# waczjoan/gaussian-mesh-splatting

Hardware: AMD Instinct MI355X
Metric: train iters/s (fwd+bwd raster) @800×800, 300k Gaussians; HBM GB/s vs roofline (higher is better)
Workload: dtype f32

## Files before the change

### gaussian-mesh-splatting_amd/csrc/gms_common.h

```cpp
#pragma once
#include <hip/hip_runtime.h>
#include <stdint.h>

#include "../../include/gmsplat.h"

namespace gms {

constexpr int TILE = 16;
constexpr int TILE_PIX = TILE * TILE;
constexpr int WAVE = 64;
constexpr int BLOCK = 256;
constexpr float NEAR_Z = 0.2f;
constexpr float DILATE = 0.3f;
constexpr float ALPHA_MIN = 1.0f / 255.0f;
constexpr float ALPHA_MAX = 0.99f;
constexpr float T_MIN = 0.0001f;

__device__ constexpr float SH_C0 = 0.28209479177387814f;
__device__ constexpr float SH_C1 = 0.4886025119029199f;
__device__ constexpr float SH_C2[5] = {1.0925484305920792f, -1.0925484305920792f, 0.31539156525252005f,
                                       -1.0925484305920792f, 0.5462742152960396f};
__device__ constexpr float SH_C3[7] = {-0.5900435899266435f, 2.890611442640554f, -0.4570457994644658f,
                                       0.3731763325901154f, -0.4570457994644658f, 1.445305721320277f,
                                       -0.5900435899266435f};

struct __attribute__((aligned(16))) SplatRec {
    float4 q0, q1, q2;
};

__host__ __device__ inline size_t align_up(size_t v, size_t a) { return (v + a - 1) / a * a; }

struct GeomState {
    SplatRec *rec;
    float *depth;
    uint8_t *clamped;
    ushort4 *rect;
    static __host__ __device__ size_t bytes(size_t P)
    {
        return align_up(P * sizeof(SplatRec), 256) + align_up(P * 4, 256) + align_up(P, 256) + align_up(P * sizeof(ushort4), 256);
    }
    static __host__ __device__ GeomState carve(void *base, size_t P)
    {
        GeomState g;
        char *p = (char *)base;
        g.rec = (SplatRec *)p; p += align_up(P * sizeof(SplatRec), 256);
        g.depth = (float *)p;  p += align_up(P * 4, 256);
        g.clamped = (uint8_t *)p; p += align_up(P, 256);
        g.rect = (ushort4 *)p;
        return g;
    }
};

struct ImageState {
    float *final_T;
    uint32_t *n_contrib;
    uint32_t *tile_count;
    uint32_t *tile_cursor;
    uint32_t *tile_offset;
    uint32_t *unit_first;
    uint32_t *mseg_first;
    uint32_t *class_first;
    uint32_t *tile_dead;
    uint32_t *tile_cmax;
    uint32_t *scan_out;
    static __host__ __device__ size_t bytes(size_t W, size_t H)
    {
        size_t T = ((W + TILE - 1) / TILE) * ((H + TILE - 1) / TILE);
        return 2 * align_up(W * H * 4, 256) + 2 * align_up(T * 4, 256) + 3 * align_up((T + 1) * 4, 256) +
               align_up(8 * (T + 1) * 4, 256) + 2 * align_up(T * 4, 256) + 256;
    }
    static __host__ __device__ ImageState carve(void *base, size_t W, size_t H)
    {
        size_t T = ((W + TILE - 1) / TILE) * ((H + TILE - 1) / TILE);
        ImageState s;
        char *p = (char *)base;
        s.final_T = (float *)p;        p += align_up(W * H * 4, 256);
        s.n_contrib = (uint32_t *)p;   p += align_up(W * H * 4, 256);
        s.tile_count = (uint32_t *)p;  p += align_up(T * 4, 256);
        s.tile_cursor = (uint32_t *)p; p += align_up(T * 4, 256);
        s.tile_offset = (uint32_t *)p; p += align_up((T + 1) * 4, 256);
        s.unit_first = (uint32_t *)p;  p += align_up((T + 1) * 4, 256);
        s.mseg_first = (uint32_t *)p;  p += align_up((T + 1) * 4, 256);
        s.class_first = (uint32_t *)p; p += align_up(8 * (T + 1) * 4, 256);
        s.tile_dead = (uint32_t *)p;   p += align_up(T * 4, 256);
        s.tile_cmax = (uint32_t *)p;   p += align_up(T * 4, 256);
        s.scan_out = (uint32_t *)p;
        return s;
    }
};

struct BinningState {
    uint64_t *keys;
    uint4 *unit_tile;
    float *seg_state;
    uint2 *deep_tab;
    uint32_t *multi_tab;
    uint16_t *mmask;
    static __host__ __device__ size_t n_units(size_t N, size_t T, size_t L) { return T + N / L + 1; }
    static __host__ __device__ size_t n_slots(size_t N, size_t L) { return 2 * (N / L) + 2; }
    static __host__ __device__ size_t n_deep(size_t N, size_t T) { return N / 1024 + T + 2; }
    static __host__ __device__ size_t n_multi(size_t N) { return N / 1024 + 2; }
    static __host__ __device__ size_t bytes(size_t N, size_t T, size_t L, bool micro)
    {
        return align_up((N > 0 ? N : 1) * 8, 256) + align_up(n_units(N, T, L) * 32, 256) +
               align_up(n_slots(N, L) * 7 * TILE_PIX * 4, 256) + align_up(n_deep(N, T) * 8, 256) + align_up(n_multi(N) * 4, 256) +
               (micro ? align_up((N > 0 ? N : 1) * 2, 256) : 0);
    }
    static __host__ __device__ BinningState carve(void *base, size_t N, size_t T, size_t L)
    {
        BinningState b;
        char *p = (char *)base;
        b.keys = (uint64_t *)p;      p += align_up((N > 0 ? N : 1) * 8, 256);
        b.unit_tile = (uint4 *)p;    p += align_up(n_units(N, T, L) * 32, 256);
        b.seg_state = (float *)p;    p += align_up(n_slots(N, L) * 7 * TILE_PIX * 4, 256);
        b.deep_tab = (uint2 *)p;     p += align_up(n_deep(N, T) * 8, 256);
        b.multi_tab = (uint32_t *)p; p += align_up(n_multi(N) * 4, 256);
        b.mmask = (uint16_t *)p;
        return b;
    }
};

template <int CTRL, int ROW_MASK = 0xf>
__device__ __forceinline__ float dpp_add(float v)
{
    int moved = __builtin_amdgcn_update_dpp(0, __builtin_bit_cast(int, v), CTRL, ROW_MASK, 0xf, false);
    return v + __builtin_bit_cast(float, moved);
}

__device__ __forceinline__ float wave_sum_to_lane63(float v)
{
    v = dpp_add<0xB1>(v);
    v = dpp_add<0x4E>(v);
    v = dpp_add<0x141>(v);
    v = dpp_add<0x140>(v);
    v = dpp_add<0x142, 0xa>(v);
    v = dpp_add<0x143, 0xc>(v);
    return v;
}

__device__ __forceinline__ void swap32x5(float &a0, float &a1, float &b0, float &b1, float &c0, float &c1, float &d0,
                                         float &d1, float &e0, float &e1)
{
    asm volatile("s_nop 1\n\tv_permlane32_swap_b32 %0, %1\n\tv_permlane32_swap_b32 %2, %3\n\t"
                 "v_permlane32_swap_b32 %4, %5\n\tv_permlane32_swap_b32 %6, %7\n\tv_permlane32_swap_b32 %8, %9"
                 : "+v"(a0), "+v"(a1), "+v"(b0), "+v"(b1), "+v"(c0), "+v"(c1), "+v"(d0), "+v"(d1), "+v"(e0), "+v"(e1));
}
__device__ __forceinline__ void swap16x3(float &a0, float &a1, float &b0, float &b1, float &c0, float &c1)
{
    asm volatile("s_nop 1\n\tv_permlane16_swap_b32 %0, %1\n\tv_permlane16_swap_b32 %2, %3\n\tv_permlane16_swap_b32 %4, %5"
                 : "+v"(a0), "+v"(a1), "+v"(b0), "+v"(b1), "+v"(c0), "+v"(c1));
}

__device__ __forceinline__ void wave_reduce10(float v0, float v1, float v2, float v3, float v4, float v5, float v6,
                                              float v7, float v8, float v9, float &y0, float &y1)
{
    swap32x5(v0, v1, v2, v3, v4, v5, v6, v7, v8, v9);
    float w0 = v0 + v1, w1 = v2 + v3, w2 = v4 + v5, w3 = v6 + v7, w4 = v8 + v9;
    float z = 0.f;
    swap16x3(w0, w1, w2, w3, w4, z);
    const float x0 = w0 + w1;
    const float x1 = w2 + w3;
    const float x2 = w4 + z;
    const float a = dpp_add<0x128>(x0);
    const float b = dpp_add<0x128>(x1);
    y0 = (threadIdx.x & 8) ? b : a;
    y1 = dpp_add<0x128>(x2);
    y0 = dpp_add<0x141>(y0); y0 = dpp_add<0xB1>(y0); y0 = dpp_add<0x4E>(y0);
    y1 = dpp_add<0x141>(y1); y1 = dpp_add<0xB1>(y1); y1 = dpp_add<0x4E>(y1);
}

__device__ __forceinline__ void wave_reduce10x2(float *a, float *b, float &y0a, float &y1a, float &y0b, float &y1b)
{
    swap32x5(a[0], a[1], a[2], a[3], a[4], a[5], a[6], a[7], a[8], a[9]);
    swap32x5(b[0], b[1], b[2], b[3], b[4], b[5], b[6], b[7], b[8], b[9]);
    float wa0 = a[0] + a[1], wb0 = b[0] + b[1], wa1 = a[2] + a[3], wb1 = b[2] + b[3], wa2 = a[4] + a[5];
    float wb2 = b[4] + b[5], wa3 = a[6] + a[7], wb3 = b[6] + b[7], wa4 = a[8] + a[9], wb4 = b[8] + b[9];
    float za = 0.f, zb = 0.f;
    swap16x3(wa0, wa1, wa2, wa3, wa4, za);
    swap16x3(wb0, wb1, wb2, wb3, wb4, zb);
    const float xa0 = wa0 + wa1, xb0 = wb0 + wb1, xa1 = wa2 + wa3, xb1 = wb2 + wb3, xa2 = wa4 + za, xb2 = wb4 + zb;
    const bool hi8 = (threadIdx.x & 8) != 0;
    const float pa = dpp_add<0x128>(xa0), pb = dpp_add<0x128>(xb0), qa = dpp_add<0x128>(xa1), qb = dpp_add<0x128>(xb1);
    y0a = hi8 ? qa : pa; y0b = hi8 ? qb : pb;
    y1a = dpp_add<0x128>(xa2); y1b = dpp_add<0x128>(xb2);
    y0a = dpp_add<0x141>(y0a); y0b = dpp_add<0x141>(y0b); y1a = dpp_add<0x141>(y1a); y1b = dpp_add<0x141>(y1b);
    y0a = dpp_add<0xB1>(y0a); y0b = dpp_add<0xB1>(y0b); y1a = dpp_add<0xB1>(y1a); y1b = dpp_add<0xB1>(y1b);
    y0a = dpp_add<0x4E>(y0a); y0b = dpp_add<0x4E>(y0b); y1a = dpp_add<0x4E>(y1a); y1b = dpp_add<0x4E>(y1b);
}

__device__ __forceinline__ void wave_sync()
{
    __builtin_amdgcn_fence(__ATOMIC_RELEASE, "wavefront");
    __builtin_amdgcn_wave_barrier();
    __builtin_amdgcn_fence(__ATOMIC_ACQUIRE, "wavefront");
}

__device__ __forceinline__ int lane_id() { return (int)(threadIdx.x & 63); }

__device__ __forceinline__ void tile_rect(float px, float py, float radius, int gx, int gy, int &minx, int &miny,
                                          int &maxx, int &maxy)
{
    const float big = 1048576.0f;
    float q0 = (px - radius) / TILE, q1 = (py - radius) / TILE;
    float q2 = (px + radius + (TILE - 1)) / TILE, q3 = (py + radius + (TILE - 1)) / TILE;
    minx = (int)fminf(big, fmaxf(-big, q0));
    miny = (int)fminf(big, fmaxf(-big, q1));
    maxx = (int)fminf(big, fmaxf(-big, q2));
    maxy = (int)fminf(big, fmaxf(-big, q3));
    minx = min(gx, max(0, minx)); maxx = min(gx, max(0, maxx));
    miny = min(gy, max(0, miny)); maxy = min(gy, max(0, maxy));
}

template <bool RETURNING>
__device__ __forceinline__ uint32_t wave_aggregated_inc(uint32_t *counters, int key, bool active)
{
    const int lane = (int)(threadIdx.x & 63);
    uint32_t rank = 0, cnt = 0;
    int my_leader = lane;
    bool is_leader = false;
    uint64_t todo = __ballot(active);
    while (todo) {
        const int leader = __builtin_ctzll(todo);
        const int k = __builtin_amdgcn_readlane(key, leader);
        const bool mine = active && key == k;
        const uint64_t same = __ballot(mine);
        if (mine) { rank = (uint32_t)__builtin_popcountll(same & ((1ull << lane) - 1ull)); my_leader = leader; }
        if (lane == leader) { is_leader = true; cnt = (uint32_t)__builtin_popcountll(same); }
        todo &= ~same;
    }
    uint32_t base = 0;
    if (is_leader) {
        if (RETURNING) base = atomicAdd(&counters[key], cnt);
        else atomicAdd(&counters[key], cnt);
    }
    if (!RETURNING) return 0;
    base = (uint32_t)__shfl((int)base, my_leader);
    return base + rank;
}

constexpr int TT_SLOTS = 1024;
__device__ __forceinline__ uint32_t tt_hash(int tile) { return ((uint32_t)tile * 2654435761u) >> 22; }
__device__ __forceinline__ int tt_insert(int *key, int tile)
{
    uint32_t h = tt_hash(tile);
    for (int probe = 0; probe < 16; probe++) {
        const int old = atomicCAS(&key[h], -1, tile);
        if (old == -1 || old == tile) return (int)h;
        h = (h + 1) & (TT_SLOTS - 1);
    }
    return -1;
}
__device__ __forceinline__ int tt_find(const int *key, int tile)
{
    uint32_t h = tt_hash(tile);
    for (int probe = 0; probe < 16; probe++) {
        const int k = key[h];
        if (k == tile) return (int)h;
        if (k == -1) return -1;
        h = (h + 1) & (TT_SLOTS - 1);
    }
    return -1;
}

struct AggTicket { uint32_t rank; int leader; uint32_t base; };

__device__ __forceinline__ AggTicket wave_aggregated_issue(uint32_t *counters, int key, bool active)
{
    const int lane = (int)(threadIdx.x & 63);
    AggTicket t{0u, lane, 0u};
    uint32_t cnt = 0;
    bool is_leader = false;
    uint64_t todo = __ballot(active);
    while (todo) {
        const int leader = __builtin_ctzll(todo);
        const int k = __builtin_amdgcn_readlane(key, leader);
        const bool mine = active && key == k;
        const uint64_t same = __ballot(mine);
        if (mine) { t.rank = (uint32_t)__builtin_popcountll(same & ((1ull << lane) - 1ull)); t.leader = leader; }
        if (lane == leader) { is_leader = true; cnt = (uint32_t)__builtin_popcountll(same); }
        todo &= ~same;
    }
    if (is_leader) t.base = atomicAdd(&counters[key], cnt);
    return t;
}

__device__ __forceinline__ uint32_t wave_aggregated_finish(const AggTicket &t)
{
    return (uint32_t)__shfl((int)t.base, t.leader) + t.rank;
}

__device__ __forceinline__ float dot3p(float a, float b, float c, float d, float e, float f, float g)
{
    float t = a * b;
    t = __fmaf_rn(c, d, t);
    t = __fmaf_rn(e, f, t);
    return t + g;
}

int fault_mode();

int det_mode();
int upstream_scale_mod_grad();
void *det_scratch(int slot, size_t bytes, hipStream_t stream);

void set_error(const char *fmt, ...);

struct TraceRange { bool on; explicit TraceRange(const char *name); ~TraceRange(); };

extern bool g_profile_on;
void profile_begin(int kernel_id, hipStream_t stream);
void profile_end(int kernel_id, hipStream_t stream);

}

#define GMS_HIP_CHECK(expr)                                                                    \
    do {                                                                                       \
        hipError_t _e = (expr);                                                                \
        if (_e != hipSuccess) {                                                                \
            gms::set_error("%s failed: %s (%s:%d)", #expr, hipGetErrorString(_e), __FILE__, __LINE__); \
            return GMS_ERR_HIP;                                                                \
        }                                                                                      \
    } while (0)

#define GMS_LAUNCH(kid, stream, ...)                                  \
    do {                                                              \
        if (gms::g_profile_on) gms::profile_begin(kid, stream);       \
        __VA_ARGS__;                                                  \
        if (gms::g_profile_on) gms::profile_end(kid, stream);         \
    } while (0)

#define GMS_KERNEL_CHECK(dbg, stream, name)                                                    \
    do {                                                                                       \
        hipError_t _e = hipGetLastError();                                                     \
        if (_e == hipSuccess && (dbg)) _e = hipStreamSynchronize(stream);                      \
        if (_e != hipSuccess) {                                                                \
            gms::set_error("kernel %s failed: %s", name, hipGetErrorString(_e));               \
            return GMS_ERR_HIP;                                                                \
        }                                                                                      \
    } while (0)
```

### gaussian-mesh-splatting_amd/csrc/gms_project.h

```cpp
#pragma once
#include "gms_common.h"

namespace gms {

struct Cov3 {
    float c[6];
};

__device__ __forceinline__ void cov3d_from_scale_rot(const float s_in[3], float mod, const float q[4], Cov3 &out)
{
#pragma clang fp contract(off)
    float s0 = mod * s_in[0], s1 = mod * s_in[1], s2 = mod * s_in[2];
    float r = q[0], x = q[1], y = q[2], z = q[3];
    float R00 = 1.f - 2.f * (y * y + z * z), R01 = 2.f * (x * y - r * z), R02 = 2.f * (x * z + r * y);
    float R10 = 2.f * (x * y + r * z), R11 = 1.f - 2.f * (x * x + z * z), R12 = 2.f * (y * z - r * x);
    float R20 = 2.f * (x * z - r * y), R21 = 2.f * (y * z + r * x), R22 = 1.f - 2.f * (x * x + y * y);
    float L00 = R00 * s0, L01 = R01 * s1, L02 = R02 * s2;
    float L10 = R10 * s0, L11 = R11 * s1, L12 = R12 * s2;
    float L20 = R20 * s0, L21 = R21 * s1, L22 = R22 * s2;
    out.c[0] = L00 * L00 + L01 * L01 + L02 * L02;
    out.c[1] = L00 * L10 + L01 * L11 + L02 * L12;
    out.c[2] = L00 * L20 + L01 * L21 + L02 * L22;
    out.c[3] = L10 * L10 + L11 * L11 + L12 * L12;
    out.c[4] = L10 * L20 + L11 * L21 + L12 * L22;
    out.c[5] = L20 * L20 + L21 * L21 + L22 * L22;
}

struct Ewa {
    float tx, ty, tz;
    float xmul, ymul;
    float T0[3], T1[3];
    float ST0[3], ST1[3];
    float a0, b, c0;
};

__device__ __forceinline__ void view_transform(const float *V, float px, float py, float pz, float &vx, float &vy,
                                               float &vz)
{
    vx = dot3p(V[0], px, V[4], py, V[8], pz, V[12]);
    vy = dot3p(V[1], px, V[5], py, V[9], pz, V[13]);
    vz = dot3p(V[2], px, V[6], py, V[10], pz, V[14]);
}

__device__ __forceinline__ void ewa_project(const float *V, float vx, float vy, float vz, const Cov3 &cv, float fx,
                                            float fy, float limx, float limy, Ewa &e)
{
#pragma clang fp contract(off)
    float txtz = vx / vz, tytz = vy / vz;
    e.tx = fminf(limx, fmaxf(-limx, txtz)) * vz;
    e.ty = fminf(limy, fmaxf(-limy, tytz)) * vz;
    e.tz = vz;
    e.xmul = (txtz < -limx || txtz > limx) ? 0.f : 1.f;
    e.ymul = (tytz < -limy || tytz > limy) ? 0.f : 1.f;
    float J00 = fx / e.tz, J02 = -(fx * e.tx) / (e.tz * e.tz);
    float J11 = fy / e.tz, J12 = -(fy * e.ty) / (e.tz * e.tz);
#pragma unroll
    for (int c = 0; c < 3; c++) {
        e.T0[c] = J00 * V[4 * c + 0] + J02 * V[4 * c + 2];
        e.T1[c] = J11 * V[4 * c + 1] + J12 * V[4 * c + 2];
    }
    const float S[3][3] = {{cv.c[0], cv.c[1], cv.c[2]}, {cv.c[1], cv.c[3], cv.c[4]}, {cv.c[2], cv.c[4], cv.c[5]}};
#pragma unroll
    for (int r = 0; r < 3; r++) {
        e.ST0[r] = S[r][0] * e.T0[0] + S[r][1] * e.T0[1] + S[r][2] * e.T0[2];
        e.ST1[r] = S[r][0] * e.T1[0] + S[r][1] * e.T1[1] + S[r][2] * e.T1[2];
    }
    e.a0 = e.T0[0] * e.ST0[0] + e.T0[1] * e.ST0[1] + e.T0[2] * e.ST0[2];
    e.b = e.T0[0] * e.ST1[0] + e.T0[1] * e.ST1[1] + e.T0[2] * e.ST1[2];
    e.c0 = e.T1[0] * e.ST1[0] + e.T1[1] * e.ST1[1] + e.T1[2] * e.ST1[2];
}

}
```

### gaussian-mesh-splatting_amd/csrc/raster_backward.hip

```cpp
#include "gms_blend.h"
#include "gms_mesh.h"
#include "gms_common.h"
#include "gms_project.h"

namespace gms {

constexpr int SH_PITCH_B = 52;

struct PreBwdArgs {
    int P, D, M, W, H;
    const float *means3D, *shs, *shs_rest, *colors, *opac, *scales, *rots, *cov3Dp, *view, *proj, *campos;
    float mod, tanx, tany;
    float scale_grad_mod;
    int aa;
    const int *radii;
    const uint8_t *clamped;
    float *accum;
    int rezero;
    float *dL_dmean2D, *dL_dopacity, *dL_dcolors;
    float *dL_dmeans3D, *dL_dcov3D, *dL_dsh, *dL_dsh_rest, *dL_dscales, *dL_drots;
    float *dL_dcolor_sh;
    int campos_row;
    GmsMeshArgs mesh;
    float *mesh_dvertices, *mesh_dalpha, *mesh_dscale, *mesh_dopacity;
};

template <int DEG>
__device__ __forceinline__ void sh_backward_regs(float *r, float x, float y, float z, const float dRGB[3], float gdir[3])
{
#define GMS_SH_TERM(K, BV, BDX, BDY, BDZ)                                          \
    {                                                                              \
        const float bv = (BV), bx = (BDX), by = (BDY), bz = (BDZ);                 \
        _Pragma("unroll") for (int c = 0; c < 3; c++) {                            \
            const float w = r[(K) * 3 + c] * dRGB[c];                              \
            gdir[0] += bx * w; gdir[1] += by * w; gdir[2] += bz * w;               \
            r[(K) * 3 + c] = bv * dRGB[c];                                         \
        }                                                                          \
    }
    GMS_SH_TERM(0, SH_C0, 0.f, 0.f, 0.f)
    if (DEG > 0) {
        GMS_SH_TERM(1, -SH_C1 * y, 0.f, -SH_C1, 0.f)
        GMS_SH_TERM(2, SH_C1 * z, 0.f, 0.f, SH_C1)
        GMS_SH_TERM(3, -SH_C1 * x, -SH_C1, 0.f, 0.f)
    }
    if (DEG > 1) {
        const float xx = x * x, yy = y * y, zz = z * z;
        GMS_SH_TERM(4, SH_C2[0] * x * y, SH_C2[0] * y, SH_C2[0] * x, 0.f)
        GMS_SH_TERM(5, SH_C2[1] * y * z, 0.f, SH_C2[1] * z, SH_C2[1] * y)
        GMS_SH_TERM(6, SH_C2[2] * (2.f * zz - xx - yy), -2.f * SH_C2[2] * x, -2.f * SH_C2[2] * y, 4.f * SH_C2[2] * z)
        GMS_SH_TERM(7, SH_C2[3] * x * z, SH_C2[3] * z, 0.f, SH_C2[3] * x)
        GMS_SH_TERM(8, SH_C2[4] * (xx - yy), 2.f * SH_C2[4] * x, -2.f * SH_C2[4] * y, 0.f)
    }
    if (DEG > 2) {
        const float xx = x * x, yy = y * y, zz = z * z;
        GMS_SH_TERM(9, SH_C3[0] * y * (3.f * xx - yy), SH_C3[0] * 6.f * x * y, SH_C3[0] * (3.f * xx - 3.f * yy), 0.f)
        GMS_SH_TERM(10, SH_C3[1] * x * y * z, SH_C3[1] * y * z, SH_C3[1] * x * z, SH_C3[1] * x * y)
        GMS_SH_TERM(11, SH_C3[2] * y * (4.f * zz - xx - yy), SH_C3[2] * (-2.f * x * y), SH_C3[2] * (4.f * zz - xx - 3.f * yy), SH_C3[2] * 8.f * y * z)
        GMS_SH_TERM(12, SH_C3[3] * z * (2.f * zz - 3.f * xx - 3.f * yy), SH_C3[3] * (-6.f * x * z), SH_C3[3] * (-6.f * y * z), SH_C3[3] * (6.f * zz - 3.f * xx - 3.f * yy))
        GMS_SH_TERM(13, SH_C3[4] * x * (4.f * zz - xx - yy), SH_C3[4] * (4.f * zz - 3.f * xx - yy), SH_C3[4] * (-2.f * x * y), SH_C3[4] * 8.f * x * z)
        GMS_SH_TERM(14, SH_C3[5] * z * (xx - yy), SH_C3[5] * 2.f * x * z, SH_C3[5] * (-2.f * y * z), SH_C3[5] * (xx - yy))
        GMS_SH_TERM(15, SH_C3[6] * x * (xx - 3.f * yy), SH_C3[6] * (3.f * xx - 3.f * yy), SH_C3[6] * (-6.f * x * y), 0.f)
    }
#undef GMS_SH_TERM
}

template <int DEG>
__device__ __forceinline__ void sh_backward(float *row_lds, float x, float y, float z, const float dRGB[3], float gdir[3])
{
    constexpr int NQ = ((DEG + 1) * (DEG + 1) * 3 + 3) / 4;
    float r[NQ * 4];
#pragma unroll
    for (int q = 0; q < NQ; q++) {
        const float4 v = *reinterpret_cast<const float4 *>(row_lds + q * 4);
        r[4 * q] = v.x; r[4 * q + 1] = v.y; r[4 * q + 2] = v.z; r[4 * q + 3] = v.w;
    }
    sh_backward_regs<DEG>(r, x, y, z, dRGB, gdir);
#pragma unroll
    for (int k = (DEG + 1) * (DEG + 1) * 3; k < NQ * 4; k++) r[k] = 0.f;
#pragma unroll
    for (int q = 0; q < NQ; q++)
        *reinterpret_cast<float4 *>(row_lds + q * 4) = make_float4(r[4 * q], r[4 * q + 1], r[4 * q + 2], r[4 * q + 3]);
}

template <int NQ>
__device__ __forceinline__ void stage_sh_rows_b(const float *shs, int g0, int rows, int rowq, float *wl, int lane)
{
    const float4 *src = reinterpret_cast<const float4 *>(shs) + (size_t)g0 * rowq;
    for (int idx = lane; idx < rows * NQ; idx += WAVE) {
        const int r = idx / NQ, c = idx - r * NQ;
        *reinterpret_cast<float4 *>(wl + r * 52 + c * 4) = src[(size_t)r * rowq + c];
    }
}

template <bool MESH>
__global__ void __launch_bounds__(BLOCK) preprocess_bwd_kernel(PreBwdArgs a, int pre_bwd_linear)
{
    __shared__ __attribute__((aligned(16))) float sh_lds[4 * WAVE * SH_PITCH_B];
    const int tid = threadIdx.x, lane = tid & 63, wave = tid >> 6;
    const int i = blockIdx.x * BLOCK + tid;
    const bool valid = i < a.P;
    const bool vis = valid && a.radii[i] > 0;
    float *wl = sh_lds + wave * (WAVE * SH_PITCH_B);
    const int rowf = a.M * 3;
    const bool use_sh = a.shs != nullptr;
    const bool vec_ok = use_sh && (rowf % 4 == 0) && (rowf <= 48);
    const int nb = (a.D + 1) * (a.D + 1);
    const int g0 = blockIdx.x * BLOCK + wave * WAVE;
    const int rows = min(WAVE, a.P - g0);

    const bool split = a.shs_rest != nullptr;
    constexpr int RESTF = 45;
    const bool linear = use_sh && split && a.D == 3 && pre_bwd_linear;
    float *const lin_dc = wl + WAVE * RESTF;
    if (linear) {
        if (__any(vis)) {
            const int rr = max(rows, 0);
            const float *sp = a.shs_rest + (size_t)g0 * RESTF;
            const int nfl = rr * RESTF, nd = rr * 3;
#pragma unroll
            for (int j = 0; j < 12; j++) {
                const int e4 = (lane + WAVE * j) * 4;
                if (e4 + 3 < nfl)
                    __builtin_amdgcn_global_load_lds((const __attribute__((address_space(1))) void *)(sp + e4),
                                                     (__attribute__((address_space(3))) void *)(wl + WAVE * 4 * j), 16, 0, 0);
            }
            if (lane * 4 + 3 < nd)
                __builtin_amdgcn_global_load_lds((const __attribute__((address_space(1))) void *)(a.shs + (size_t)g0 * 3 + lane * 4),
                                                 (__attribute__((address_space(3))) void *)lin_dc, 16, 0, 0);
            if (rr < WAVE) {
                for (int e = (nfl & ~3) + lane; e < nfl; e += WAVE) wl[e] = sp[e];
                for (int e = (nd & ~3) + lane; e < nd; e += WAVE) lin_dc[e] = a.shs[(size_t)g0 * 3 + e];
            }
            __builtin_amdgcn_s_waitcnt(0x0f70);
        }
        wave_sync();
    } else if (use_sh && split) {
        if (__any(vis)) {
            for (int e = lane; e < rows * 3; e += WAVE) wl[(e / 3) * SH_PITCH_B + (e % 3)] = a.shs[(size_t)g0 * 3 + e];
            const int need = nb * 3 - 3;
            if (need == RESTF) {
                const float *sp = a.shs_rest + (size_t)g0 * RESTF;
                const int nfl = rows * RESTF;
                for (int e4 = lane * 4; e4 < nfl; e4 += WAVE * 4) {
                    float v4[4];
                    if (e4 + 3 < nfl) { const float4 v = *reinterpret_cast<const float4 *>(sp + e4); v4[0] = v.x; v4[1] = v.y; v4[2] = v.z; v4[3] = v.w; }
                    else { for (int t = 0; t < 4; t++) v4[t] = e4 + t < nfl ? sp[e4 + t] : 0.f; }
#pragma unroll
                    for (int t = 0; t < 4; t++) {
                        const int e = e4 + t;
                        if (e < nfl) wl[(e / RESTF) * SH_PITCH_B + 3 + (e % RESTF)] = v4[t];
                    }
                }
            } else {
                for (int e = lane; e < rows * need; e += WAVE) {
                    const int r = e / need, c = e - r * need;
                    wl[r * SH_PITCH_B + 3 + c] = a.shs_rest[((size_t)g0 + r) * RESTF + c];
                }
            }
        }
        wave_sync();
    } else if (use_sh) {
        if (vec_ok) {
            if (__any(vis)) {
                const int rowq = rowf / 4;
                switch (a.D) {
                case 0: stage_sh_rows_b<1>(a.shs, g0, rows, rowq, wl, lane); break;
                case 1: stage_sh_rows_b<3>(a.shs, g0, rows, rowq, wl, lane); break;
                case 2: stage_sh_rows_b<7>(a.shs, g0, rows, rowq, wl, lane); break;
                default: stage_sh_rows_b<12>(a.shs, g0, rows, rowq, wl, lane); break;
                }
            }
        } else if (vis) {
            for (int k = 0; k < nb * 3; k++) wl[lane * SH_PITCH_B + k] = a.shs[(size_t)i * rowf + k];
        }
        wave_sync();
    }

    float dmean[3] = {0.f, 0.f, 0.f};
    float dcov[6] = {0.f, 0.f, 0.f, 0.f, 0.f, 0.f};
    float dscale[3] = {0.f, 0.f, 0.f};
    float drot[4] = {0.f, 0.f, 0.f, 0.f};
    float dcol_sh[3] = {0.f, 0.f, 0.f};
    float4 ga = make_float4(0.f, 0.f, 0.f, 0.f), gb = ga, gc4 = ga;
    if (valid) {
        float4 *rec = reinterpret_cast<float4 *>(a.accum + (size_t)i * GRAD_STRIDE);
        ga = rec[0]; gb = rec[1]; gc4 = rec[2];
        if (a.rezero && vis) {
            const float4 z = make_float4(0.f, 0.f, 0.f, 0.f);
            rec[0] = z; rec[1] = z; rec[2] = z;
        }
    }
    const float mom_x = ga.x, mom_y = ga.y, mom_xx = ga.z, mom_xy = ga.w, mom_yy = gb.x, mom_0 = gb.y;
    float acc_mx = 0.f, acc_my = 0.f;
    const float acc_col[3] = {gb.z, gb.w, gc4.x};
    const float acc_id = gc4.y;
    float dop = 0.f;
    float *row = wl + lane * SH_PITCH_B;

    if (vis) {
        const float px = a.means3D[3 * (size_t)i], py = a.means3D[3 * (size_t)i + 1], pz = a.means3D[3 * (size_t)i + 2];
        const float *V = a.view, *Mx = a.proj;
        float vx, vy, vz;
        view_transform(V, px, py, pz, vx, vy, vz);
        Cov3 cv;
        float s_in[3] = {0.f, 0.f, 0.f}, q[4] = {1.f, 0.f, 0.f, 0.f};
        if (a.cov3Dp) {
#pragma unroll
            for (int k = 0; k < 6; k++) cv.c[k] = a.cov3Dp[6 * (size_t)i + k];
        } else {
            s_in[0] = a.scales[3 * (size_t)i]; s_in[1] = a.scales[3 * (size_t)i + 1]; s_in[2] = a.scales[3 * (size_t)i + 2];
            const float4 qv = *reinterpret_cast<const float4 *>(a.rots + 4 * (size_t)i);
            q[0] = qv.x; q[1] = qv.y; q[2] = qv.z; q[3] = qv.w;
            cov3d_from_scale_rot(s_in, a.mod, q, cv);
        }
        const float fx = (float)a.W / (2.f * a.tanx), fy = (float)a.H / (2.f * a.tany);
        Ewa e;
        ewa_project(V, vx, vy, vz, cv, fx, fy, 1.3f * a.tanx, 1.3f * a.tany, e);
        const float b = e.b, aD = e.a0 + DILATE, cD = e.c0 + DILATE;
        const float det = aD * cD - b * b;
        {
            const float dinv = 1.f / det;
            const float cA = cD * dinv, cB = -b * dinv, cC = aD * dinv;
            acc_mx = -(0.5f * (float)a.W) * (cA * mom_x + cB * mom_y);
            acc_my = -(0.5f * (float)a.H) * (cC * mom_y + cB * mom_x);
            float opp = a.opac[i];
            if (a.aa) opp *= sqrtf(fmaxf(0.000025f, (e.a0 * e.c0 - b * b) / det));
            dop = opp > 0.f ? mom_0 / opp : 0.f;
        }
        const float gA = -0.5f * mom_xx, gB = -0.5f * mom_xy, gC = -0.5f * mom_yy;
        const float d2inv = 1.f / (det * det + 0.0000001f);
        float dL_da = d2inv * (-cD * cD * gA + 2.f * b * cD * gB + (det - aD * cD) * gC);
        float dL_dc = d2inv * (-aD * aD * gC + 2.f * aD * b * gB + (det - aD * cD) * gA);
        float dL_db = d2inv * 2.f * (b * cD * gA - (det + 2.f * b * b) * gB + aD * b * gC);
        if (a.aa) {
            const float det0 = e.a0 * e.c0 - b * b;
            const float ratio = det0 / det;
            const float h = sqrtf(fmaxf(0.000025f, ratio));
            const float dL_dh = dop * a.opac[i];
            dop = dop * h;
            const float dL_dr = ratio <= 0.000025f ? 0.f : dL_dh / (2.f * h);
            dL_da += dL_dr * (e.c0 / det - det0 * cD / (det * det));
            dL_dc += dL_dr * (e.a0 / det - det0 * aD / (det * det));
            dL_db += dL_dr * (-2.f * b / det + det0 * 2.f * b / (det * det));
        }
        const float *T0 = e.T0, *T1 = e.T1;
        dcov[0] = T0[0] * T0[0] * dL_da + T0[0] * T1[0] * dL_db + T1[0] * T1[0] * dL_dc;
        dcov[3] = T0[1] * T0[1] * dL_da + T0[1] * T1[1] * dL_db + T1[1] * T1[1] * dL_dc;
        dcov[5] = T0[2] * T0[2] * dL_da + T0[2] * T1[2] * dL_db + T1[2] * T1[2] * dL_dc;
        dcov[1] = 2.f * T0[0] * T0[1] * dL_da + (T0[0] * T1[1] + T0[1] * T1[0]) * dL_db + 2.f * T1[0] * T1[1] * dL_dc;
        dcov[2] = 2.f * T0[0] * T0[2] * dL_da + (T0[0] * T1[2] + T0[2] * T1[0]) * dL_db + 2.f * T1[0] * T1[2] * dL_dc;
        dcov[4] = 2.f * T0[2] * T0[1] * dL_da + (T0[1] * T1[2] + T0[2] * T1[1]) * dL_db + 2.f * T1[1] * T1[2] * dL_dc;
        float dJ00 = 0.f, dJ02 = 0.f, dJ11 = 0.f, dJ12 = 0.f;
#pragma unroll
        for (int c = 0; c < 3; c++) {
            const float dT0 = 2.f * e.ST0[c] * dL_da + e.ST1[c] * dL_db;
            const float dT1 = 2.f * e.ST1[c] * dL_dc + e.ST0[c] * dL_db;
            dJ00 += dT0 * V[4 * c + 0]; dJ02 += dT0 * V[4 * c + 2];
            dJ11 += dT1 * V[4 * c + 1]; dJ12 += dT1 * V[4 * c + 2];
        }
        const float tzi = 1.f / e.tz, tz2 = tzi * tzi, tz3 = tz2 * tzi;
        const float dtx = e.xmul * -fx * tz2 * dJ02;
        const float dty = e.ymul * -fy * tz2 * dJ12;
        float dtz = -fx * tz2 * dJ00 - fy * tz2 * dJ11 + (2.f * fx * e.tx) * tz3 * dJ02 + (2.f * fy * e.ty) * tz3 * dJ12;
        dtz -= acc_id * tz2;
#pragma unroll
        for (int r = 0; r < 3; r++) dmean[r] += V[4 * r + 0] * dtx + V[4 * r + 1] * dty + V[4 * r + 2] * dtz;

        const float hx = dot3p(Mx[0], px, Mx[4], py, Mx[8], pz, Mx[12]);
        const float hy = dot3p(Mx[1], px, Mx[5], py, Mx[9], pz, Mx[13]);
        const float hw = dot3p(Mx[3], px, Mx[7], py, Mx[11], pz, Mx[15]);
        const float mw = 1.f / (hw + 0.0000001f);
        const float gmx = acc_mx, gmy = acc_my;
        const float mul1 = hx * mw * mw, mul2 = hy * mw * mw;
#pragma unroll
        for (int r = 0; r < 3; r++)
            dmean[r] += (Mx[4 * r + 0] * mw - Mx[4 * r + 3] * mul1) * gmx + (Mx[4 * r + 1] * mw - Mx[4 * r + 3] * mul2) * gmy;

        if (use_sh) {
            const float ddx = px - a.campos[0], ddy = py - a.campos[1], ddz = pz - a.campos[2];
            const float inv = 1.f / sqrtf(ddx * ddx + ddy * ddy + ddz * ddz);
            const float x = ddx * inv, y = ddy * inv, z = ddz * inv;
            const unsigned cl = a.clamped[i];
            float dRGB[3];
#pragma unroll
            for (int c = 0; c < 3; c++) { dRGB[c] = ((cl >> c) & 1u) ? 0.f : acc_col[c]; dcol_sh[c] = dRGB[c]; }
            float gdir[3] = {0.f, 0.f, 0.f};
            if (linear) {
                float r[48];
#pragma unroll
                for (int c = 0; c < 3; c++) r[c] = lin_dc[lane * 3 + c];
#pragma unroll
                for (int m = 0; m < RESTF; m++) r[3 + m] = wl[lane * RESTF + m];
                sh_backward_regs<3>(r, x, y, z, dRGB, gdir);
                if (!a.dL_dcolor_sh) {
#pragma unroll
                    for (int c = 0; c < 3; c++) lin_dc[lane * 3 + c] = r[c];
#pragma unroll
                    for (int m = 0; m < RESTF; m++) wl[lane * RESTF + m] = r[3 + m];
                }
            } else
            switch (a.D) {
            case 0: sh_backward<0>(row, x, y, z, dRGB, gdir); break;
            case 1: sh_backward<1>(row, x, y, z, dRGB, gdir); break;
            case 2: sh_backward<2>(row, x, y, z, dRGB, gdir); break;
            default: sh_backward<3>(row, x, y, z, dRGB, gdir); break;
            }
            const float dd = x * gdir[0] + y * gdir[1] + z * gdir[2];
            dmean[0] += (gdir[0] - x * dd) * inv;
            dmean[1] += (gdir[1] - y * dd) * inv;
            dmean[2] += (gdir[2] - z * dd) * inv;
        }

        if (!a.cov3Dp) {
            const float mod = a.mod;
            const float s[3] = {mod * s_in[0], mod * s_in[1], mod * s_in[2]};
            const float r = q[0], x = q[1], y = q[2], z = q[3];
            const float R[3][3] = {
                {1.f - 2.f * (y * y + z * z), 2.f * (x * y - r * z), 2.f * (x * z + r * y)},
                {2.f * (x * y + r * z), 1.f - 2.f * (x * x + z * z), 2.f * (y * z - r * x)},
                {2.f * (x * z - r * y), 2.f * (y * z + r * x), 1.f - 2.f * (x * x + y * y)}};
            const float Gs[3][3] = {{dcov[0], 0.5f * dcov[1], 0.5f * dcov[2]},
                                    {0.5f * dcov[1], dcov[3], 0.5f * dcov[4]},
                                    {0.5f * dcov[2], 0.5f * dcov[4], dcov[5]}};
            float dR[3][3];
#pragma unroll
            for (int j = 0; j < 3; j++) {
                float accs = 0.f;
#pragma unroll
                for (int a1 = 0; a1 < 3; a1++) {
                    float acc = 0.f;
#pragma unroll
                    for (int k2 = 0; k2 < 3; k2++) acc += Gs[a1][k2] * R[k2][j] * s[j];
                    const float dLm = 2.f * acc;
                    accs += R[a1][j] * dLm;
                    dR[a1][j] = dLm * s[j];
                }
                dscale[j] = accs * a.scale_grad_mod;
            }
            drot[0] = 2.f * (-z * dR[0][1] + y * dR[0][2] + z * dR[1][0] - x * dR[1][2] - y * dR[2][0] + x * dR[2][1]);
            drot[1] = 2.f * (y * dR[0][1] + z * dR[0][2] + y * dR[1][0] - 2.f * x * dR[1][1] - r * dR[1][2] + z * dR[2][0] + r * dR[2][1] - 2.f * x * dR[2][2]);
            drot[2] = 2.f * (-2.f * y * dR[0][0] + x * dR[0][1] + r * dR[0][2] + x * dR[1][0] + z * dR[1][2] - r * dR[2][0] + z * dR[2][1] - 2.f * y * dR[2][2]);
            drot[3] = 2.f * (-2.f * z * dR[0][0] - r * dR[0][1] + x * dR[0][2] + r * dR[1][0] - 2.f * z * dR[1][1] + y * dR[1][2] + x * dR[2][0] + y * dR[2][1]);
        }
    }

    if (use_sh && a.dL_dcolor_sh) {
    } else if (linear) {
        if (!vis) {
#pragma unroll
            for (int c = 0; c < 3; c++) lin_dc[lane * 3 + c] = 0.f;
#pragma unroll
            for (int m = 0; m < RESTF; m++) wl[lane * RESTF + m] = 0.f;
        }
        wave_sync();
        if (rows > 0) {
            const int nfl = rows * RESTF, nd = rows * 3;
            float *dp = a.dL_dsh_rest + (size_t)g0 * RESTF, *dd = a.dL_dsh + (size_t)g0 * 3;
#pragma unroll
            for (int j = 0; j < 12; j++) {
                const int e4 = (lane + WAVE * j) * 4;
                if (e4 + 3 < nfl) {
                    typedef float v4f __attribute__((ext_vector_type(4)));
                    __builtin_nontemporal_store(*reinterpret_cast<const v4f *>(wl + e4), reinterpret_cast<v4f *>(dp + e4));
                }
                else for (int t = 0; t < 4; t++) if (e4 + t < nfl) dp[e4 + t] = wl[e4 + t];
            }
            if (lane * 4 + 3 < nd) *reinterpret_cast<float4 *>(dd + lane * 4) = *reinterpret_cast<const float4 *>(lin_dc + lane * 4);
            else for (int t = 0; t < 4; t++) if (lane * 4 + t < nd) dd[lane * 4 + t] = lin_dc[lane * 4 + t];
        }
    } else if (use_sh && split) {
        for (int q = vis ? (nb * 3 + 3) / 4 : 0; q < 12; q++)
            *reinterpret_cast<float4 *>(row + q * 4) = make_float4(0.f, 0.f, 0.f, 0.f);
        wave_sync();
        if (rows > 0) {
            for (int e = lane; e < rows * 3; e += WAVE) a.dL_dsh[(size_t)g0 * 3 + e] = wl[(e / 3) * SH_PITCH_B + (e % 3)];
            float *dp = a.dL_dsh_rest + (size_t)g0 * RESTF;
            const int nfl = rows * RESTF;
            for (int e4 = lane * 4; e4 < nfl; e4 += WAVE * 4) {
                float v4[4];
#pragma unroll
                for (int t = 0; t < 4; t++) {
                    const int e = e4 + t;
                    v4[t] = e < nfl ? wl[(e / RESTF) * SH_PITCH_B + 3 + (e % RESTF)] : 0.f;
                }
                if (e4 + 3 < nfl) *reinterpret_cast<float4 *>(dp + e4) = make_float4(v4[0], v4[1], v4[2], v4[3]);
                else for (int t = 0; t < 4; t++) if (e4 + t < nfl) dp[e4 + t] = v4[t];
            }
        }
    } else if (use_sh) {
        const int used = vis ? nb * 3 : 0;
        if (vec_ok) {
            const int rowq = rowf / 4;
            for (int q = vis ? (nb * 3 + 3) / 4 : 0; q < rowq; q++)
                *reinterpret_cast<float4 *>(row + q * 4) = make_float4(0.f, 0.f, 0.f, 0.f);
            wave_sync();
            if (rows > 0) {
                float4 *dst = reinterpret_cast<float4 *>(a.dL_dsh + (size_t)g0 * rowf);
                for (int idx = lane; idx < rows * rowq; idx += WAVE) {
                    int r = idx / rowq, c = idx - r * rowq;
                    dst[(size_t)r * rowq + c] = *reinterpret_cast<const float4 *>(wl + r * SH_PITCH_B + c * 4);
                }
            }
        } else if (valid) {
            for (int k = 0; k < rowf; k++) a.dL_dsh[(size_t)i * rowf + k] = k < used ? row[k] : 0.f;
        }
    }
    if (!valid) return;
    if (MESH) {
        const float gs[3] = {dscale[0], dscale[1], dscale[2]}, gq[4] = {drot[0], drot[1], drot[2], drot[3]};
        splat_backward_from_registers(a.mesh, (int64_t)i, dmean, gs, gq, dop, a.mesh_dvertices, a.mesh_dalpha, a.mesh_dscale, a.mesh_dopacity);
    } else {
        a.dL_dopacity[i] = dop;
    }
    a.dL_dmean2D[3 * (size_t)i] = acc_mx; a.dL_dmean2D[3 * (size_t)i + 1] = acc_my; a.dL_dmean2D[3 * (size_t)i + 2] = 0.f;
    if (a.dL_dcolors) { a.dL_dcolors[3 * (size_t)i] = acc_col[0]; a.dL_dcolors[3 * (size_t)i + 1] = acc_col[1]; a.dL_dcolors[3 * (size_t)i + 2] = acc_col[2]; }
    if (a.dL_dcolor_sh && a.campos_row && i == 0) {
        a.dL_dcolor_sh[3 * (size_t)a.P] = a.campos[0]; a.dL_dcolor_sh[3 * (size_t)a.P + 1] = a.campos[1]; a.dL_dcolor_sh[3 * (size_t)a.P + 2] = a.campos[2];
    }
    if (a.dL_dcolor_sh) { a.dL_dcolor_sh[3 * (size_t)i] = dcol_sh[0]; a.dL_dcolor_sh[3 * (size_t)i + 1] = dcol_sh[1]; a.dL_dcolor_sh[3 * (size_t)i + 2] = dcol_sh[2]; }
    if (MESH) return;
    a.dL_dmeans3D[3 * (size_t)i] = dmean[0]; a.dL_dmeans3D[3 * (size_t)i + 1] = dmean[1]; a.dL_dmeans3D[3 * (size_t)i + 2] = dmean[2];
    if (a.cov3Dp) {
        if (a.dL_dcov3D)
#pragma unroll
            for (int k = 0; k < 6; k++) a.dL_dcov3D[6 * (size_t)i + k] = dcov[k];
    } else {
        a.dL_dscales[3 * (size_t)i] = dscale[0]; a.dL_dscales[3 * (size_t)i + 1] = dscale[1]; a.dL_dscales[3 * (size_t)i + 2] = dscale[2];
        *reinterpret_cast<float4 *>(a.dL_drots + 4 * (size_t)i) = make_float4(drot[0], drot[1], drot[2], drot[3]);
    }
}


__global__ void fault_scale_kernel(float *base, int rows, int stride, int field, int every, float factor)
{
    const int i = (blockIdx.x * blockDim.x + threadIdx.x) * every;
    if (i < rows) base[(size_t)i * stride + field] *= factor;
}

template <int NSUB>
__global__ void __launch_bounds__(BLOCK) det_reduce_kernel(int P, int gx, int gy, const int *radii, const SplatRec *rec, const float *depth,
                                                           const uint32_t *tile_offset, const uint64_t *keys, uint64_t capacity,
                                                           const float *part, float *accum)
{
    const int i = (int)((blockIdx.x * (unsigned)BLOCK + threadIdx.x) >> 4), f = (int)(threadIdx.x & 15u);
    if (i >= P) return;
    const int r = radii[i];
    if (r <= 0) return;
    const float4 q0 = rec[i].q0;
    int minx, miny, maxx, maxy;
    tile_rect(q0.x, q0.y, (float)r, gx, gy, minx, miny, maxx, maxy);
    const uint64_t key = ((uint64_t)__float_as_uint(depth[i]) << 32) | (uint32_t)i;
    float acc = 0.f;
    for (int ty = miny; ty < maxy; ty++)
        for (int tx = minx; tx < maxx; tx++) {
            const int t = ty * gx + tx;
            uint32_t lo = tile_offset[t], hi = tile_offset[t + 1];
            if ((uint64_t)hi > capacity) return;
            while (lo < hi) {
                const uint32_t mid = lo + ((hi - lo) >> 1);
                if (keys[mid] < key) lo = mid + 1; else hi = mid;
            }
#pragma unroll
            for (int sub = 0; sub < NSUB; sub++) acc += part[((size_t)lo * NSUB + sub) * GRAD_STRIDE + f];
        }
    if (f < 10) accum[(size_t)i * GRAD_STRIDE + f] = acc;
}

struct ShExpandArgs {
    int P, D, M, V;
    const float *means3D;
    const float *campos;
    const float *factors;
    size_t stride;
    float *dL_dsh;
    float *dL_dsh_rest;
    int accumulate;
};

template <int DEG>
__device__ __forceinline__ void sh_basis(float x, float y, float z, float *Y)
{
    Y[0] = SH_C0;
    if (DEG > 0) { Y[1] = -SH_C1 * y; Y[2] = SH_C1 * z; Y[3] = -SH_C1 * x; }
    if (DEG > 1) {
        const float xx = x * x, yy = y * y, zz = z * z;
        Y[4] = SH_C2[0] * x * y; Y[5] = SH_C2[1] * y * z; Y[6] = SH_C2[2] * (2.f * zz - xx - yy);
        Y[7] = SH_C2[3] * x * z; Y[8] = SH_C2[4] * (xx - yy);
    }
    if (DEG > 2) {
        const float xx = x * x, yy = y * y, zz = z * z;
        Y[9] = SH_C3[0] * y * (3.f * xx - yy); Y[10] = SH_C3[1] * x * y * z; Y[11] = SH_C3[2] * y * (4.f * zz - xx - yy);
        Y[12] = SH_C3[3] * z * (2.f * zz - 3.f * xx - 3.f * yy); Y[13] = SH_C3[4] * x * (4.f * zz - xx - yy);
        Y[14] = SH_C3[5] * z * (xx - yy); Y[15] = SH_C3[6] * x * (xx - 3.f * yy);
    }
}

template <int DEG>
__global__ void __launch_bounds__(BLOCK) sh_grad_expand_kernel(ShExpandArgs a)
{
    constexpr int NB = (DEG + 1) * (DEG + 1);
    const int i = blockIdx.x * BLOCK + threadIdx.x;
    if (i >= a.P) return;
    const float px = a.means3D[3 * (size_t)i], py = a.means3D[3 * (size_t)i + 1], pz = a.means3D[3 * (size_t)i + 2];
    float acc[NB * 3];
#pragma unroll
    for (int k = 0; k < NB * 3; k++) acc[k] = 0.f;
    for (int v = 0; v < a.V; v++) {
        const float *gp = a.factors + (size_t)v * a.stride + (size_t)i * 3;
        const float g[3] = {gp[0], gp[1], gp[2]};
        if (g[0] == 0.f && g[1] == 0.f && g[2] == 0.f) continue;
        const float ddx = px - a.campos[3 * v], ddy = py - a.campos[3 * v + 1], ddz = pz - a.campos[3 * v + 2];
        const float inv = 1.f / sqrtf(ddx * ddx + ddy * ddy + ddz * ddz);
        float Y[16];
        sh_basis<DEG>(ddx * inv, ddy * inv, ddz * inv, Y);
#pragma unroll
        for (int k = 0; k < NB; k++)
#pragma unroll
            for (int c = 0; c < 3; c++) acc[k * 3 + c] += Y[k] * g[c];
    }
    float *d0 = a.dL_dsh + (size_t)i * (a.dL_dsh_rest ? 3 : a.M * 3);
    float *d1 = a.dL_dsh_rest ? a.dL_dsh_rest + (size_t)i * ((a.M - 1) * 3) : d0 + 3;
    if (a.accumulate) {
#pragma unroll
        for (int c = 0; c < 3; c++) d0[c] += acc[c];
#pragma unroll
        for (int k = 3; k < NB * 3; k++) d1[k - 3] += acc[k];
    } else {
#pragma unroll
        for (int c = 0; c < 3; c++) d0[c] = acc[c];
#pragma unroll
        for (int k = 3; k < NB * 3; k++) d1[k - 3] = acc[k];
        for (int k = NB * 3; k < a.M * 3; k++) d1[k - 3] = 0.f;
    }
}

}

using namespace gms;

extern "C" int32_t gms_rasterize_backward(const GmsRasterBackwardArgs *A, void *stream_)
{
    gms::TraceRange trace_range("gms_rasterize_backward");
    hipStream_t stream = (hipStream_t)stream_;
    set_error("%s", "");
    if (!A || A->P < 0 || A->width <= 0 || A->height <= 0) {
        set_error("gms_rasterize_backward: invalid sizes");
        return GMS_ERR_INVALID_ARGUMENT;
    }
    const int P = A->P, W = A->width, H = A->height;
    if (P == 0) return GMS_OK;
    const bool sr = A->scales && A->rotations;
    const GmsMeshArgs *mesh = A->mesh;
    if (mesh) {
        const int32_t mrc = check_mesh_args(mesh, false);
        if (mrc != GMS_OK) return mrc;
        if (mesh->P != (int64_t)P || mesh->splats_per_face <= 0 || mesh->splats_per_face > 4 || !mesh->_opacity || !sr || A->cov3D_precomp ||
            !A->mesh_dL_dvertices || !A->mesh_dL_dalpha || !A->mesh_dL_dscale || !A->mesh_dL_d_opacity || det_mode()) {
            set_error("gms_rasterize_backward: the mesh backward inside preprocess_bwd needs a complete GmsMeshArgs (P equal, 1-4 splats per face, "
                      "_opacity), the scales + rotations path, all four mesh_dL_* outputs, and is not available in deterministic mode");
            return GMS_ERR_INVALID_ARGUMENT;
        }
    }
    if (!A->means3D || !A->opacities || !A->radii || !A->geom_buffer || !A->binning_buffer || !A->image_buffer ||
        !A->dL_dout_color || !A->dL_dmeans2D || !A->grad_accum || (!mesh && !A->dL_dopacity) || (A->colors_precomp && !A->dL_dcolors) ||
        (!mesh && !A->dL_dmeans3D) || (A->sh_factor_mode != 0 && A->sh_factor_mode != 1) || (A->sh_factor_mode && (!A->shs || !A->dL_dcolors)) ||
        (A->factor_campos_row && !A->sh_factor_mode) ||
        (A->shs && !A->sh_factor_mode && !A->dL_dsh) || (A->shs_rest && ((!A->sh_factor_mode && !A->dL_dsh_rest) || A->M != 16)) ||
        ((A->shs == nullptr) == (A->colors_precomp == nullptr)) ||
        (sr == (A->cov3D_precomp != nullptr)) || (sr && !mesh && (!A->dL_dscales || !A->dL_drotations)) ||
        (A->cov3D_precomp && !A->dL_dcov3D)) {
        set_error("gms_rasterize_backward: null or inconsistent pointer arguments");
        return GMS_ERR_INVALID_ARGUMENT;
    }
    const int gx = (W + TILE - 1) / TILE, gy = (H + TILE - 1) / TILE;
    GeomState geom = GeomState::carve(const_cast<void *>(A->geom_buffer), (size_t)P);
    ImageState img = ImageState::carve(const_cast<void *>(A->image_buffer), (size_t)W, (size_t)H);
    const int T = gx * gy;
    const uint32_t L = seg_len_min();
    const uint64_t cap = (uint64_t)(A->binning_capacity > 0 ? A->binning_capacity : (A->num_rendered > 0 ? A->num_rendered : 1));
    BinningState bin = BinningState::carve(const_cast<void *>(A->binning_buffer), (size_t)cap, (size_t)T, L);

    if (A->num_rendered > 0) {
        BlendGrid g;
        g.W = W; g.H = H; g.gx = gx; g.gy = gy; g.T = T; g.scan_out = img.scan_out; g.tile_offset = img.tile_offset;
        g.unit_first = img.unit_first; g.mseg_first = img.mseg_first; g.unit_tile = bin.unit_tile; g.keys = bin.keys;
        g.seg_state = bin.seg_state; g.capacity = cap;
        g.max_units = (uint32_t)BinningState::n_units((size_t)cap, (size_t)T, L); g.dbg = 0; g.unit_run = unit_run(); g.dbg_buf = nullptr; g.tile_dead = img.tile_dead; g.tile_cmax = img.tile_cmax;
        g.mmask = bin.mmask;
        BlendBwdArgs b;
        b.rec = geom.rec; b.bg = A->background; b.final_T = img.final_T; b.n_contrib = img.n_contrib;
        b.dL_dpix = A->dL_dout_color; b.dL_dinvd = A->dL_dout_invdepth; b.accum = A->grad_accum;
        b.has_invd = A->dL_dout_invdepth != nullptr;
        b.part = nullptr;
        uint32_t mu = (uint32_t)BinningState::n_units((size_t)cap, (size_t)T, L);
        if (A->num_units > 0 && (uint64_t)A->num_units < mu) mu = (uint32_t)A->num_units;
        const bool micro = use_micro(cap, T);
        const bool det = det_mode() != 0 && fault_mode() == 0;
        if (det) {
            const size_t nsub = micro ? 1 : 4, bytes = (size_t)A->num_rendered * nsub * GRAD_STRIDE * sizeof(float);
            b.part = static_cast<float *>(det_scratch(0, bytes, stream));
            if (!b.part) { set_error("deterministic mode: scratch allocation of %zu bytes failed", bytes); return GMS_ERR_ALLOC; }
            if (!micro) GMS_HIP_CHECK(hipMemsetAsync(b.part, 0, bytes, stream));
        }
        int32_t rc = micro ? launch_micro_backward(g, b, mu, A->debug != 0, stream) : launch_blend_backward(g, b, mu, A->debug != 0, stream);
        if (rc != GMS_OK) return rc;
        if (det) {
            const unsigned rblocks = (unsigned)(((size_t)P * 16 + BLOCK - 1) / BLOCK);
            if (micro) det_reduce_kernel<1><<<rblocks, BLOCK, 0, stream>>>(P, gx, gy, A->radii, geom.rec, geom.depth, img.tile_offset, bin.keys, cap, b.part, A->grad_accum);
            else det_reduce_kernel<4><<<rblocks, BLOCK, 0, stream>>>(P, gx, gy, A->radii, geom.rec, geom.depth, img.tile_offset, bin.keys, cap, b.part, A->grad_accum);
            GMS_KERNEL_CHECK(A->debug, stream, "det_reduce");
        }
        if (fault_mode() == 1)
            fault_scale_kernel<<<(unsigned)((P / 1000 + 256) / 256), 256, 0, stream>>>(A->grad_accum, P, GRAD_STRIDE, GRAD_CA, 1000, 1.002f);
    }
    PreBwdArgs p{};
    p.P = P; p.D = A->D; p.M = A->M; p.W = W; p.H = H;
    p.means3D = A->means3D; p.shs = A->shs; p.shs_rest = A->shs_rest; p.colors = A->colors_precomp; p.opac = A->opacities; p.scales = A->scales;
    p.rots = A->rotations; p.cov3Dp = A->cov3D_precomp; p.view = A->viewmatrix; p.proj = A->projmatrix; p.campos = A->campos;
    p.mod = A->scale_modifier; p.scale_grad_mod = upstream_scale_mod_grad() ? 1.f : A->scale_modifier; p.tanx = A->tan_fovx; p.tany = A->tan_fovy; p.aa = A->antialiasing; p.radii = A->radii;
    p.clamped = geom.clamped; p.accum = A->grad_accum; p.rezero = fault_mode() == 3 ? 0 : A->grad_accum_rezero; p.dL_dmean2D = A->dL_dmeans2D;
    p.dL_dcolors = A->colors_precomp ? A->dL_dcolors : nullptr; p.dL_dcolor_sh = (A->shs && A->sh_factor_mode) ? A->dL_dcolors : nullptr; p.campos_row = A->factor_campos_row; p.dL_dopacity = A->dL_dopacity; p.dL_dmeans3D = A->dL_dmeans3D;
    p.dL_dcov3D = A->dL_dcov3D; p.dL_dsh = A->dL_dsh; p.dL_dsh_rest = A->dL_dsh_rest; p.dL_dscales = A->dL_dscales; p.dL_drots = A->dL_drotations;
    const int lin_ok = A->shs && A->shs_rest && A->D == 3 && (((uintptr_t)A->shs) & 15u) == 0 && (((uintptr_t)A->shs_rest) & 15u) == 0 &&
                       (A->sh_factor_mode || ((((uintptr_t)A->dL_dsh) & 15u) == 0 && (((uintptr_t)A->dL_dsh_rest) & 15u) == 0));
    if (mesh) {
        p.mesh = *mesh; p.mesh_dvertices = A->mesh_dL_dvertices; p.mesh_dalpha = A->mesh_dL_dalpha; p.mesh_dscale = A->mesh_dL_dscale; p.mesh_dopacity = A->mesh_dL_d_opacity;
        GMS_LAUNCH(GMS_K_PREPROCESS_BWD, stream, preprocess_bwd_kernel<true><<<(unsigned)((P + BLOCK - 1) / BLOCK), BLOCK, 0, stream>>>(p, lin_ok));
    } else {
        GMS_LAUNCH(GMS_K_PREPROCESS_BWD, stream, preprocess_bwd_kernel<false><<<(unsigned)((P + BLOCK - 1) / BLOCK), BLOCK, 0, stream>>>(p, lin_ok));
    }
    GMS_KERNEL_CHECK(A->debug, stream, "preprocess_bwd");
    if (fault_mode() == 4 && A->dL_dscales)
        fault_scale_kernel<<<(unsigned)((P / 1000 + 256) / 256), 256, 0, stream>>>(A->dL_dscales, P, 3, 0, 1000, 1.002f);
    if (fault_mode() == 5 && A->dL_dscales)
        for (int f = 0; f < 3; f++)
            fault_scale_kernel<<<(unsigned)((P / 100 + 256) / 256), 256, 0, stream>>>(A->dL_dscales, P, 3, f, 100, 1.0013f);
    return GMS_OK;
}

extern "C" int32_t gms_sh_grad_expand(const GmsShGradExpandArgs *A, void *stream_)
{
    gms::TraceRange trace_range("gms_sh_grad_expand");
    hipStream_t stream = (hipStream_t)stream_;
    set_error("%s", "");
    if (!A || A->P < 0 || A->V < 1 || A->D < 0 || A->D > 3 || A->M < (A->D + 1) * (A->D + 1) || !A->means3D || !A->campos || !A->factors || (A->factor_stride != 0 && A->factor_stride < (int64_t)A->P * 3) ||
        !A->dL_dsh || (A->dL_dsh_rest && A->M < 2)) {
        set_error("gms_sh_grad_expand: invalid sizes or null pointer arguments");
        return GMS_ERR_INVALID_ARGUMENT;
    }
    if (A->P == 0) return GMS_OK;
    ShExpandArgs e;
    e.P = A->P; e.D = A->D; e.M = A->M; e.V = A->V; e.means3D = A->means3D; e.campos = A->campos; e.factors = A->factors;
    e.stride = A->factor_stride > 0 ? (size_t)A->factor_stride : (size_t)A->P * 3;
    e.dL_dsh = A->dL_dsh; e.dL_dsh_rest = A->dL_dsh_rest; e.accumulate = A->accumulate;
    const unsigned blocks = (unsigned)((A->P + BLOCK - 1) / BLOCK);
    switch (A->D) {
    case 0: GMS_LAUNCH(GMS_K_SH_EXPAND, stream, sh_grad_expand_kernel<0><<<blocks, BLOCK, 0, stream>>>(e)); break;
    case 1: GMS_LAUNCH(GMS_K_SH_EXPAND, stream, sh_grad_expand_kernel<1><<<blocks, BLOCK, 0, stream>>>(e)); break;
    case 2: GMS_LAUNCH(GMS_K_SH_EXPAND, stream, sh_grad_expand_kernel<2><<<blocks, BLOCK, 0, stream>>>(e)); break;
    default: GMS_LAUNCH(GMS_K_SH_EXPAND, stream, sh_grad_expand_kernel<3><<<blocks, BLOCK, 0, stream>>>(e)); break;
    }
    GMS_KERNEL_CHECK(A->debug, stream, "sh_grad_expand");
    return GMS_OK;
}
```

### gaussian-mesh-splatting_amd/csrc/raster_forward.hip

```cpp
#include <stdarg.h>
#include <stdio.h>

#include <stdlib.h>
#include <mutex>

#include "gms_blend.h"
#include "gms_mesh.h"
#include "gms_points.h"
#include <atomic>
#include <vector>
#include <chrono>

#include "gms_common.h"
#include "gms_project.h"

namespace gms {

static thread_local char g_err[512] = "";
void set_error(const char *fmt, ...)
{
    va_list ap;
    va_start(ap, fmt);
    vsnprintf(g_err, sizeof(g_err), fmt, ap);
    va_end(ap);
}

constexpr int SMALL_AREA = 64;
constexpr int SH_PITCH = 52;

struct PreArgs {
    int P, D, M, W, H, gx, gy;
    const float *means3D, *shs, *shs_rest, *colors, *opac, *scales, *rots, *cov3Dp, *view, *proj, *campos;
    float mod, tanx, tany;
    int aa;
    int *radii;
    uint8_t *visible;
    GeomState geom;
    uint32_t *tile_count;
    uint32_t *zero_cursor;
    uint32_t *zero_cmax;
    int T;
    GmsMeshArgs mesh;
    float *k0_xyz, *k0_scale, *k0_rot, *k0_opac;
};

template <int DEG>
__device__ __forceinline__ float sh_eval_channel(const float *row, int c, float x, float y, float z)
{
#pragma clang fp contract(off)
    float res = SH_C0 * row[0 * 3 + c];
    if (DEG > 0) {
        res = res - SH_C1 * y * row[1 * 3 + c] + SH_C1 * z * row[2 * 3 + c] - SH_C1 * x * row[3 * 3 + c];
        if (DEG > 1) {
            float xx = x * x, yy = y * y, zz = z * z, xy = x * y, yz = y * z, xz = x * z;
            res = res + SH_C2[0] * xy * row[4 * 3 + c] + SH_C2[1] * yz * row[5 * 3 + c] +
                  SH_C2[2] * (2.f * zz - xx - yy) * row[6 * 3 + c] + SH_C2[3] * xz * row[7 * 3 + c] +
                  SH_C2[4] * (xx - yy) * row[8 * 3 + c];
            if (DEG > 2) {
                res = res + SH_C3[0] * y * (3.f * xx - yy) * row[9 * 3 + c] + SH_C3[1] * xy * z * row[10 * 3 + c] +
                      SH_C3[2] * y * (4.f * zz - xx - yy) * row[11 * 3 + c] +
                      SH_C3[3] * z * (2.f * zz - 3.f * xx - 3.f * yy) * row[12 * 3 + c] +
                      SH_C3[4] * x * (4.f * zz - xx - yy) * row[13 * 3 + c] + SH_C3[5] * z * (xx - yy) * row[14 * 3 + c] +
                      SH_C3[6] * x * (xx - 3.f * yy) * row[15 * 3 + c];
            }
        }
    }
    return res;
}

template <int NQ>
__device__ __forceinline__ void stage_sh_rows(const float *shs, int g0, int rows, int rowq, float *wl, int lane)
{
    const float4 *src = reinterpret_cast<const float4 *>(shs) + (size_t)g0 * rowq;
    for (int idx = lane; idx < rows * NQ; idx += WAVE) {
        const int r = idx / NQ, c = idx - r * NQ;
        *reinterpret_cast<float4 *>(wl + r * SH_PITCH + c * 4) = src[(size_t)r * rowq + c];
    }
}

template <int DEG>
__device__ __forceinline__ void sh_colour(const float *row_lds, float x, float y, float z, float rgb[3], unsigned &clampbits)
{
    constexpr int NQ = ((DEG + 1) * (DEG + 1) * 3 + 3) / 4;
    float r[NQ * 4];
#pragma unroll
    for (int q = 0; q < NQ; q++) {
        const float4 v = *reinterpret_cast<const float4 *>(row_lds + q * 4);
        r[4 * q] = v.x; r[4 * q + 1] = v.y; r[4 * q + 2] = v.z; r[4 * q + 3] = v.w;
    }
#pragma unroll
    for (int c = 0; c < 3; c++) {
        float v = sh_eval_channel<DEG>(r, c, x, y, z) + 0.5f;
        if (v < 0.f) { clampbits |= 1u << c; v = 0.f; }
        rgb[c] = v;
    }
}

template <int SHDEG, bool SPLIT, bool DMA = false, bool K0 = false, bool PTS = false>
__device__ __forceinline__ void preprocess_fwd_body(const PreArgs &a, const GmsPointsArgs &pts = GmsPointsArgs{})
{
#pragma clang fp contract(off)
    static_assert(!DMA || (SHDEG >= 0 && SHDEG <= 3 && SPLIT), "the LDS-DMA staging exists for split degree-3 STORAGE (any active degree: the rows come in whole)");
    static_assert(!K0 || DMA, "the fused mesh input rides on the LDS-DMA instantiation");
    static_assert(!PTS || (DMA && !K0), "the fused points input rides on the LDS-DMA instantiation, without the mesh input");
    static_assert(DMA || !SPLIT || SHDEG != 3, "split degree-3 storage is staged by LDS-DMA (the register-staged rows were measured and removed)");
    constexpr int DMA_HALF_ROWS = WAVE / 2, DMA_HALF_Q = 6;
    constexpr int DMA_REST_FLOATS = DMA_HALF_Q * WAVE * 4;
    constexpr int DMA_WAVE_FLOATS = DMA_REST_FLOATS + WAVE * 3;
    __shared__ __attribute__((aligned(16))) float sh_lds[DMA ? 4 * DMA_WAVE_FLOATS : 4 * WAVE * SH_PITCH];
    const int tid = threadIdx.x, lane = tid & 63, wave = tid >> 6;
    const int i = blockIdx.x * BLOCK + tid;
    const bool valid = i < a.P;
    if (a.zero_cursor)
        for (int q = i; q < a.T; q += (int)gridDim.x * BLOCK) a.zero_cursor[q] = 0u;
    if (a.zero_cmax)
        for (int q = i; q < a.T; q += (int)gridDim.x * BLOCK) a.zero_cmax[q] = 0u;
    if (K0 && a.mesh.prezero)
        for (int64_t q = i; q < a.mesh.prezero_count; q += (int64_t)gridDim.x * BLOCK) a.mesh.prezero[q] = 0.f;

    constexpr int NQ = SHDEG >= 0 ? ((SHDEG + 1) * (SHDEG + 1) * 3 + 3) / 4 : 1;
    constexpr int NB3 = SHDEG >= 0 ? (SHDEG + 1) * (SHDEG + 1) * 3 : 3;
    constexpr int RESTF = 45;
    float4 stg[NQ];
    float dcv[3] = {0.f, 0.f, 0.f};
    float s_in[3] = {0.f, 0.f, 0.f};
    float4 q_in = make_float4(1.f, 0.f, 0.f, 0.f);
    float op_in = 0.f;
    SplatInputs k0in = {};
    if (K0 && valid) splat_inputs_load(a.mesh, (int64_t)i, k0in);
    PointsInputs ptin = {};
    if (PTS && valid) points_inputs_load(pts, (int64_t)i, ptin);
    if (SHDEG >= 0) {
        const int g0 = blockIdx.x * BLOCK + wave * WAVE;
        const int rows = min(WAVE, a.P - g0);
        if (DMA) {
            float *wl = sh_lds + wave * DMA_WAVE_FLOATS;
            const float *sp = a.shs_rest + (size_t)g0 * RESTF;
            const int nfl = max(0, min(rows, DMA_HALF_ROWS)) * RESTF;
#pragma unroll
            for (int j = 0; j < DMA_HALF_Q; j++) {
                const int e4 = (lane + WAVE * j) * 4;
                if (e4 + 3 < nfl)
                    __builtin_amdgcn_global_load_lds((const __attribute__((address_space(1))) void *)(sp + e4),
                                                     (__attribute__((address_space(3))) void *)(wl + WAVE * 4 * j), 16, 0, 0);
            }
            const float *dp = a.shs + (size_t)g0 * 3;
            if (lane * 4 + 3 < rows * 3)
                __builtin_amdgcn_global_load_lds((const __attribute__((address_space(1))) void *)(dp + lane * 4),
                                                 (__attribute__((address_space(3))) void *)(wl + DMA_REST_FLOATS), 16, 0, 0);
        } else if (!SPLIT) {
            const float4 *src = reinterpret_cast<const float4 *>(a.shs) + (size_t)g0 * 12;
#pragma unroll
            for (int j = 0; j < NQ; j++) {
                const int idx = lane + WAVE * j;
                const int r = idx / NQ, c = idx - r * NQ;
                stg[j] = idx < rows * NQ ? src[(size_t)r * 12 + c] : make_float4(0.f, 0.f, 0.f, 0.f);
            }
        } else {
#pragma unroll
            for (int j = 0; j < 3; j++) {
                const int e = lane + WAVE * j;
                dcv[j] = e < rows * 3 ? a.shs[(size_t)g0 * 3 + e] : 0.f;
            }
        }
        if (valid && !K0 && !PTS) {
            op_in = a.opac[i];
            if (!a.cov3Dp) {
                s_in[0] = a.scales[3 * (size_t)i]; s_in[1] = a.scales[3 * (size_t)i + 1]; s_in[2] = a.scales[3 * (size_t)i + 2];
                q_in = *reinterpret_cast<const float4 *>(a.rots + 4 * (size_t)i);
            }
        }
    }

    float px = 0, py = 0, pz = 0, vx = 0, vy = 0, vz = 0;
    bool vis = false;
    float pix = 0, piy = 0, cA = 0, cB = 0, cC = 0, opp = 0, a_d = 0, c_d = 0, rad = 0;
    int minx = 0, miny = 0, maxx = 0, maxy = 0;
    if (K0) {
        if (valid) {
            SplatParams sp;
            splat_from_inputs(a.mesh, k0in, sp);
            px = sp.xyz[0]; py = sp.xyz[1]; pz = sp.xyz[2];
            s_in[0] = sp.scale[0]; s_in[1] = sp.scale[1]; s_in[2] = sp.scale[2];
            q_in = make_float4(sp.q[0], sp.q[1], sp.q[2], sp.q[3]);
            op_in = sp.opacity;
            if (a.k0_xyz) {
                a.k0_xyz[3 * (size_t)i] = px; a.k0_xyz[3 * (size_t)i + 1] = py; a.k0_xyz[3 * (size_t)i + 2] = pz;
                a.k0_scale[3 * (size_t)i] = s_in[0]; a.k0_scale[3 * (size_t)i + 1] = s_in[1]; a.k0_scale[3 * (size_t)i + 2] = s_in[2];
                *reinterpret_cast<float4 *>(a.k0_rot + 4 * (size_t)i) = q_in;
                a.k0_opac[i] = op_in;
            }
            view_transform(a.view, px, py, pz, vx, vy, vz); vis = vz > NEAR_Z;
        }
    } else if (PTS) {
        if (valid) {
            SplatParams sp;
            points_from_inputs(pts, ptin, sp, nullptr);
            px = sp.xyz[0]; py = sp.xyz[1]; pz = sp.xyz[2];
            s_in[0] = sp.scale[0]; s_in[1] = sp.scale[1]; s_in[2] = sp.scale[2];
            q_in = make_float4(sp.q[0], sp.q[1], sp.q[2], sp.q[3]);
            op_in = sp.opacity;
            view_transform(a.view, px, py, pz, vx, vy, vz); vis = vz > NEAR_Z;
        }
    } else if (valid) {
        px = a.means3D[3 * (size_t)i]; py = a.means3D[3 * (size_t)i + 1]; pz = a.means3D[3 * (size_t)i + 2];
        view_transform(a.view, px, py, pz, vx, vy, vz); vis = vz > NEAR_Z;
    }
    if (vis) {
        const float *Mx = a.proj;
        float hx = dot3p(Mx[0], px, Mx[4], py, Mx[8], pz, Mx[12]);
        float hy = dot3p(Mx[1], px, Mx[5], py, Mx[9], pz, Mx[13]);
        float hw = dot3p(Mx[3], px, Mx[7], py, Mx[11], pz, Mx[15]);
        float pw = 1.f / (hw + 0.0000001f);
        float ndcx = hx * pw, ndcy = hy * pw;
        Cov3 cv;
        if (a.cov3Dp) {
#pragma unroll
            for (int k = 0; k < 6; k++) cv.c[k] = a.cov3Dp[6 * (size_t)i + k];
        } else {
            if (SHDEG < 0) {
                s_in[0] = a.scales[3 * (size_t)i]; s_in[1] = a.scales[3 * (size_t)i + 1]; s_in[2] = a.scales[3 * (size_t)i + 2];
                q_in = *reinterpret_cast<const float4 *>(a.rots + 4 * (size_t)i);
            }
            float q[4] = {q_in.x, q_in.y, q_in.z, q_in.w};
            cov3d_from_scale_rot(s_in, a.mod, q, cv);
        }
        const float fx = (float)a.W / (2.f * a.tanx), fy = (float)a.H / (2.f * a.tany);
        Ewa e;
        ewa_project(a.view, vx, vy, vz, cv, fx, fy, 1.3f * a.tanx, 1.3f * a.tany, e);
        float det0 = e.a0 * e.c0 - e.b * e.b;
        a_d = e.a0 + DILATE; c_d = e.c0 + DILATE;
        float det = a_d * c_d - e.b * e.b;
        float hconv = 1.f;
        if (a.aa) hconv = sqrtf(fmaxf(0.000025f, det0 / det));
        if (det == 0.f) vis = false;
        float dinv = 1.f / det;
        cA = c_d * dinv; cB = -e.b * dinv; cC = a_d * dinv;
        float mid = 0.5f * (a_d + c_d);
        float disc = sqrtf(fmaxf(0.1f, mid * mid - det));
        float l1 = mid + disc, l2 = mid - disc;
        rad = ceilf(3.f * sqrtf(fmaxf(l1, l2)));
        pix = ((ndcx + 1.f) * a.W - 1.f) * 0.5f;
        piy = ((ndcy + 1.f) * a.H - 1.f) * 0.5f;
        tile_rect(pix, piy, rad, a.gx, a.gy, minx, miny, maxx, maxy);
        if ((maxx - minx) * (maxy - miny) == 0) vis = false;
        opp = (SHDEG >= 0 ? op_in : a.opac[i]) * hconv;
    }

    float rgb[3] = {0, 0, 0};
    unsigned clampbits = 0;
    if (DMA) {
        float *wl = sh_lds + wave * DMA_WAVE_FLOATS;
        const int g0 = blockIdx.x * BLOCK + wave * WAVE;
        const int rows = max(0, min(WAVE, a.P - g0));
        const float *sp = a.shs_rest + (size_t)g0 * RESTF;
        float dxc = 0.f, dyc = 0.f, dzc = 0.f;
        if (vis) {
            const float dx = px - a.campos[0], dy = py - a.campos[1], dz = pz - a.campos[2];
            const float inv = 1.f / sqrtf(dx * dx + dy * dy + dz * dz);
            dxc = dx * inv; dyc = dy * inv; dzc = dz * inv;
        }
#pragma unroll
        for (int half = 0; half < 2; half++) {
            const int r0 = half * DMA_HALF_ROWS;
            const int hrows = max(0, min(rows - r0, DMA_HALF_ROWS));
            if (half == 1) {
                wave_sync();
                const int nfl = hrows * RESTF;
#pragma unroll
                for (int j = 0; j < DMA_HALF_Q; j++) {
                    const int e4 = (lane + WAVE * j) * 4;
                    if (e4 + 3 < nfl)
                        __builtin_amdgcn_global_load_lds((const __attribute__((address_space(1))) void *)(sp + r0 * RESTF + e4),
                                                         (__attribute__((address_space(3))) void *)(wl + WAVE * 4 * j), 16, 0, 0);
                }
            }
            if (hrows < DMA_HALF_ROWS) {
                const int nfl = hrows * RESTF;
                for (int e = (nfl & ~3) + lane; e < nfl; e += WAVE) wl[e] = sp[r0 * RESTF + e];
            }
            if (half == 0 && rows < WAVE) {
                const int nd = rows * 3;
                for (int e = (nd & ~3) + lane; e < nd; e += WAVE) wl[DMA_REST_FLOATS + e] = a.shs[(size_t)g0 * 3 + e];
            }
            __builtin_amdgcn_s_waitcnt(0x0f70);
            wave_sync();
            if (vis && (lane >> 5) == half) {
                float r[48];
#pragma unroll
                for (int c = 0; c < 3; c++) r[c] = wl[DMA_REST_FLOATS + lane * 3 + c];
#pragma unroll
                for (int m = 0; m < RESTF; m++) r[3 + m] = wl[(lane - r0) * RESTF + m];
#pragma unroll
                for (int c = 0; c < 3; c++) {
                    float v = sh_eval_channel<SHDEG>(r, c, dxc, dyc, dzc) + 0.5f;
                    if (v < 0.f) { clampbits |= 1u << c; v = 0.f; }
                    rgb[c] = v;
                }
            }
        }
    } else if (SHDEG >= 0) {
        float *wl = sh_lds + wave * (WAVE * SH_PITCH);
        if (!SPLIT) {
#pragma unroll
            for (int j = 0; j < NQ; j++) {
                const int idx = lane + WAVE * j;
                const int r = idx / NQ, c = idx - r * NQ;
                *reinterpret_cast<float4 *>(wl + r * SH_PITCH + c * 4) = stg[j];
            }
        } else {
#pragma unroll
            for (int j = 0; j < 3; j++) {
                const int e = lane + WAVE * j;
                wl[(e / 3) * SH_PITCH + (e % 3)] = dcv[j];
            }
            if (SHDEG > 0) {
                const int g0 = blockIdx.x * BLOCK + wave * WAVE;
                const int rows = min(WAVE, a.P - g0);
                constexpr int need = NB3 > 3 ? NB3 - 3 : 1;
                for (int e = lane; e < rows * need; e += WAVE) {
                    const int r = e / need, c = e - r * need;
                    wl[r * SH_PITCH + 3 + c] = a.shs_rest[((size_t)g0 + r) * RESTF + c];
                }
            }
        }
        wave_sync();
        if (vis) {
            float dx = px - a.campos[0], dy = py - a.campos[1], dz = pz - a.campos[2];
            float inv = 1.f / sqrtf(dx * dx + dy * dy + dz * dz);
            sh_colour<(SHDEG >= 0 ? SHDEG : 0)>(wl + lane * SH_PITCH, dx * inv, dy * inv, dz * inv, rgb, clampbits);
        }
    } else if (a.shs) {
        const int nb = (a.D + 1) * (a.D + 1);
        const int rowf = a.M * 3;
        float *wl = sh_lds + wave * (WAVE * SH_PITCH);
        const bool any_vis = __any(vis);
        const bool vec_ok = (rowf % 4 == 0) && (rowf <= 48);
        if (any_vis && vec_ok) {
            const int g0 = blockIdx.x * BLOCK + wave * WAVE;
            const int rows = min(WAVE, a.P - g0);
            const int rowq = rowf / 4;
            switch (a.D) {
            case 0: stage_sh_rows<1>(a.shs, g0, rows, rowq, wl, lane); break;
            case 1: stage_sh_rows<3>(a.shs, g0, rows, rowq, wl, lane); break;
            case 2: stage_sh_rows<7>(a.shs, g0, rows, rowq, wl, lane); break;
            default: stage_sh_rows<12>(a.shs, g0, rows, rowq, wl, lane); break;
            }
        } else if (vis) {
            for (int k = 0; k < nb * 3; k++) wl[lane * SH_PITCH + k] = a.shs[(size_t)i * rowf + k];
        }
        wave_sync();
        if (vis) {
            float dx = px - a.campos[0], dy = py - a.campos[1], dz = pz - a.campos[2];
            float inv = 1.f / sqrtf(dx * dx + dy * dy + dz * dz);
            float x = dx * inv, y = dy * inv, z = dz * inv;
            const float *row = wl + lane * SH_PITCH;
            switch (a.D) {
            case 0: sh_colour<0>(row, x, y, z, rgb, clampbits); break;
            case 1: sh_colour<1>(row, x, y, z, rgb, clampbits); break;
            case 2: sh_colour<2>(row, x, y, z, rgb, clampbits); break;
            default: sh_colour<3>(row, x, y, z, rgb, clampbits); break;
            }
        }
    } else if (vis) {
        rgb[0] = a.colors[3 * (size_t)i]; rgb[1] = a.colors[3 * (size_t)i + 1]; rgb[2] = a.colors[3 * (size_t)i + 2];
    }

    if (valid && !vis) a.radii[i] = 0;
    if (valid) a.geom.rect[i] = vis ? make_ushort4((unsigned short)minx, (unsigned short)miny, (unsigned short)maxx, (unsigned short)maxy)
                                    : make_ushort4(0, 0, 0, 0);
    if (valid && a.visible) a.visible[i] = vis ? 1 : 0;
    if (vis) {
        float ex, ey;
        cull_extents(a_d, c_d, cA, cB, cC, opp, ex, ey);
        SplatRec rec;
        rec.q0 = make_float4(pix, piy, cA, cB);
        rec.q1 = make_float4(cC, opp, rgb[0], rgb[1]);
        rec.q2 = make_float4(rgb[2], 1.f / vz, ex, ey);
        a.geom.rec[i] = rec;
        a.geom.depth[i] = vz;
        a.geom.clamped[i] = (uint8_t)clampbits;
        a.radii[i] = (int)rad;
    }
    const int rw = maxx - minx;
    const int area = vis ? rw * (maxy - miny) : 0;
    const bool small = area <= SMALL_AREA;
    __syncthreads();
    int *tt_key = reinterpret_cast<int *>(sh_lds);
    uint32_t *tt_cnt = reinterpret_cast<uint32_t *>(sh_lds) + TT_SLOTS;
    for (int q = tid; q < TT_SLOTS; q += BLOCK) { tt_key[q] = -1; tt_cnt[q] = 0; }
    __syncthreads();
    if (small) {
        int cx = minx, cy = miny;
        for (int k = 0; k < area; k++) {
            const int t = cy * a.gx + cx;
            const int sl = tt_insert(tt_key, t);
            if (sl >= 0) atomicAdd(&tt_cnt[sl], 1u);
            else atomicAdd(&a.tile_count[t], 1u);
            if (++cx == maxx) { cx = minx; cy++; }
        }
    }
    __syncthreads();
    for (int q = tid; q < TT_SLOTS; q += BLOCK)
        if (tt_key[q] >= 0) atomicAdd(&a.tile_count[tt_key[q]], tt_cnt[q]);
    uint64_t big = __ballot(!small);
    while (big) {
        const int src = __builtin_ctzll(big);
        big &= big - 1;
        const int bminx = __builtin_amdgcn_readlane(minx, src), bminy = __builtin_amdgcn_readlane(miny, src);
        const int brw = __builtin_amdgcn_readlane(rw, src), barea = __builtin_amdgcn_readlane(area, src);
        for (int k = lane; k < barea; k += WAVE) {
            const int ty = k / brw, tx = k - ty * brw;
            atomicAdd(&a.tile_count[(bminy + ty) * a.gx + bminx + tx], 1u);
        }
    }
}

template <int SHDEG, bool SPLIT>
__global__ void __launch_bounds__(BLOCK) preprocess_fwd_kernel(PreArgs a) { preprocess_fwd_body<SHDEG, SPLIT, false, false>(a); }
template <bool K0, int DEG = 3>
__global__ void __launch_bounds__(BLOCK) __attribute__((amdgpu_waves_per_eu(5, 5))) preprocess_fwd_dma_kernel(PreArgs a)
{
    preprocess_fwd_body<DEG, true, true, K0>(a);
}
template <int DEG>
__global__ void __launch_bounds__(BLOCK) __attribute__((amdgpu_waves_per_eu(5, 5))) preprocess_fwd_points_kernel(PreArgs a, GmsPointsArgs pts)
{
    preprocess_fwd_body<DEG, true, true, false, true>(a, pts);
}

constexpr int SORT_RUN = 1024;
constexpr int SORT_RUNS_PER_TILE = 8;
constexpr int SORT_BIG_CHUNK = SORT_RUN * SORT_RUNS_PER_TILE;
constexpr int MP_CHUNK = 1024;

constexpr int NSCAN = 11;
constexpr int NCLASS = 6;
constexpr int SCAN_THREADS = 1024;

__device__ __forceinline__ void tile_terms(uint32_t c, uint32_t L, uint32_t t[NSCAN], int sort_np = 0)
{
    const uint32_t ns = max(1u, (c + L - 1) / L);
    t[0] = c; t[1] = ns; t[2] = ns > 1 ? ns : 0;
    const uint32_t r = c % L;
    t[3] = c / L;
    t[4] = r * 4 >= 3 * L ? 1u : 0u;
    t[5] = (r * 4 < 3 * L && r * 2 >= L) ? 1u : 0u;
    t[6] = (r * 2 < L && r * 4 >= L) ? 1u : 0u;
    t[7] = (r * 4 < L && r != 0) ? 1u : 0u;
    t[8] = c == 0 ? 1u : 0u;
    t[9] = c > 1 ? (c + MP_CHUNK - 1) / MP_CHUNK : 0u;
    t[10] = c > (uint32_t)SORT_RUN ? 1u : 0u;
    (void)sort_np;
}

__device__ __forceinline__ void publish_counts(int32_t *host_slot, int32_t seq, uint32_t n, uint32_t deepest, uint32_t units)
{
    unsigned long long *hs = reinterpret_cast<unsigned long long *>(host_slot);
    const unsigned long long tag = (unsigned long long)(uint32_t)seq << 32;
    __hip_atomic_store(&hs[2], tag | units, __ATOMIC_RELAXED, __HIP_MEMORY_SCOPE_SYSTEM);
    __hip_atomic_store(&hs[1], tag | deepest, __ATOMIC_RELAXED, __HIP_MEMORY_SCOPE_SYSTEM);
    __hip_atomic_store(&hs[0], tag | n, __ATOMIC_RELAXED, __HIP_MEMORY_SCOPE_SYSTEM);
}

__global__ void __launch_bounds__(SCAN_THREADS) tile_scan_kernel(uint32_t *count, uint32_t *offset, uint32_t *cursor,
                                                                 uint32_t *unit_first, uint32_t *mseg_first,
                                                                 uint32_t *class_first, int T, uint32_t L_forced, int32_t *host_slot,
                                                                 int32_t seq, int sort_np, uint32_t *scan_out)
{
    __shared__ uint32_t wave_tot[NSCAN][SCAN_THREADS / WAVE];
    const int tid = threadIdx.x, lane = tid & 63, wave = tid >> 6;
    const int per = (T + SCAN_THREADS - 1) / SCAN_THREADS;
    const int b = tid * per, e = min(T, b + per);
    uint32_t L = L_forced;
    if (L == 0) {
        __shared__ uint32_t wave_n[SCAN_THREADS / WAVE];
        uint32_t n = 0;
        for (int t = b; t < e; t++) n += count[t];
        for (int d = 32; d >= 1; d >>= 1) n += (uint32_t)__shfl_xor((int)n, d);
        if (lane == 0) wave_n[wave] = n;
        __syncthreads();
        uint64_t total = 0;
        for (int w = 0; w < SCAN_THREADS / WAVE; w++) total += wave_n[w];
        L = total > (uint64_t)SEG_VERY_DEEP_PER_TILE * (uint64_t)T ? SEG_LEN_VERY_DEEP
          : total > (uint64_t)SEG_DEEP_PER_TILE * (uint64_t)T ? SEG_LEN_DEEP : SEG_LEN_SHALLOW;
    }
    uint32_t run[NSCAN], own[NSCAN];
    uint32_t deepest = 0;
#pragma unroll
    for (int k = 0; k < NSCAN; k++) run[k] = 0;
    for (int t = b; t < e; t++) {
        uint32_t q[NSCAN];
        tile_terms(count[t], L, q, sort_np);
        deepest = max(deepest, q[0]);
#pragma unroll
        for (int k = 0; k < NSCAN; k++) run[k] += q[k];
    }
    for (int d = 32; d >= 1; d >>= 1) deepest = max(deepest, (uint32_t)__shfl_xor((int)deepest, d));
    __shared__ uint32_t wave_deep[SCAN_THREADS / WAVE];
    if (lane == 0) wave_deep[wave] = deepest;
#pragma unroll
    for (int k = 0; k < NSCAN; k++) {
        own[k] = run[k];
        for (int d = 1; d < WAVE; d <<= 1) {
            const uint32_t x = (uint32_t)__shfl_up((int)run[k], d);
            if (lane >= d) run[k] += x;
        }
        if (lane == WAVE - 1) wave_tot[k][wave] = run[k];
    }
    __syncthreads();
    if (wave == 0) {
#pragma unroll
        for (int k = 0; k < NSCAN; k++) {
            uint32_t v = lane < SCAN_THREADS / WAVE ? wave_tot[k][lane] : 0u;
            for (int d = 1; d < SCAN_THREADS / WAVE; d <<= 1) {
                const uint32_t x = (uint32_t)__shfl_up((int)v, d);
                if (lane >= d) v += x;
            }
            if (lane < SCAN_THREADS / WAVE) wave_tot[k][lane] = v;
        }
    }
    __syncthreads();
    uint32_t tot[NSCAN];
#pragma unroll
    for (int k = 0; k < NSCAN; k++) {
        tot[k] = wave_tot[k][SCAN_THREADS / WAVE - 1];
        run[k] = run[k] - own[k] + (wave > 0 ? wave_tot[k][wave - 1] : 0u);
    }
    if (tid == 0) {
        uint32_t dm = 0;
        for (int w = 0; w < SCAN_THREADS / WAVE; w++) dm = max(dm, wave_deep[w]);
        scan_out[0] = tot[0]; scan_out[1] = dm; scan_out[2] = tot[1]; scan_out[3] = L;
        if (host_slot) publish_counts(host_slot, seq, tot[0], dm, tot[1]);
    }
    for (int t = b; t < e; t++) {
        uint32_t q[NSCAN];
        tile_terms(count[t], L, q, sort_np);
        offset[t] = run[0]; unit_first[t] = run[1]; mseg_first[t] = run[2];
#pragma unroll
        for (int k = 0; k < NCLASS; k++) class_first[k * (T + 1) + t] = run[3 + k];
        class_first[NCLASS * (T + 1) + t] = run[9];
        class_first[(NCLASS + 1) * (T + 1) + t] = run[10];
        cursor[t] = 0;
        count[t] = 0;
#pragma unroll
        for (int k = 0; k < NSCAN; k++) run[k] += q[k];
    }
    if (tid == 0) {
        offset[T] = tot[0]; unit_first[T] = tot[1]; mseg_first[T] = tot[2];
#pragma unroll
        for (int k = 0; k < NCLASS; k++) class_first[k * (T + 1) + T] = tot[3 + k];
        class_first[NCLASS * (T + 1) + T] = tot[9];
        class_first[(NCLASS + 1) * (T + 1) + T] = tot[10];
    }
}

struct FillUnitsArgs {
    const uint32_t *class_first, *offset, *mseg_first;
    uint4 *unit_tile;
    uint2 *deep_tab;
    uint32_t *multi_tab;
    int T, sort_np;
    const uint32_t *scan_out;
    uint32_t max_units, max_deep, max_multi;
};

__device__ __forceinline__ void fill_units_tile(const FillUnitsArgs &f, int t, uint32_t c, uint32_t L, const uint32_t pre[NSCAN], const uint32_t tot[NSCAN])
{
    const uint32_t nfull = c / L;
    uint32_t q[NSCAN];
    tile_terms(c, L, q, f.sort_np);
    const uint32_t nseg = q[1];
    const uint4 tail = make_uint4(pre[0], pre[0] + c, 0u, 0u);
    const uint32_t slot0 = pre[2];
    auto put = [&](uint32_t u, uint32_t seg) {
        if (u < f.max_units) {
            f.unit_tile[2 * (size_t)u] = make_uint4((uint32_t)t, seg, nseg, slot0);
            f.unit_tile[2 * (size_t)u + 1] = tail;
        }
    };
    for (uint32_t j = 0, d = pre[9]; j < q[9]; j++, d++)
        if (d < f.max_deep) f.deep_tab[d] = make_uint2((uint32_t)t, j);
    if (q[10]) { const uint32_t d = pre[10]; if (d < f.max_multi) f.multi_tab[d] = (uint32_t)t; }
    uint32_t u = pre[3];
    for (uint32_t s = 0; s < nfull; s++, u++) put(u, s);
    uint32_t base = tot[3];
    for (int k = 1; k < NCLASS; k++) {
        if (q[3 + k]) put(base + pre[3 + k], k == NCLASS - 1 ? 0u : nfull);
        base += tot[3 + k];
    }
}

__device__ __forceinline__ void fill_units(const FillUnitsArgs &f, int block)
{
    const int T = f.T;
    const int t = block * BLOCK + threadIdx.x;
    if (t >= T) return;
    const uint32_t c = f.offset[t + 1] - f.offset[t];
    uint32_t pre[NSCAN], tot[NSCAN];
    pre[0] = f.offset[t]; pre[1] = 0u; pre[2] = f.mseg_first[t]; tot[0] = tot[1] = tot[2] = 0u;
#pragma unroll
    for (int k = 0; k < NCLASS + 2; k++) { pre[3 + k] = f.class_first[k * (T + 1) + t]; tot[3 + k] = f.class_first[k * (T + 1) + T]; }
    fill_units_tile(f, t, c, f.scan_out[3], pre, tot);
}

constexpr int INLINE_SCAN_MAX_T = 4096;

__device__ __forceinline__ uint32_t wave_incl_scan_u32(uint32_t v, int lane)
{
    for (int d = 1; d < WAVE; d <<= 1) {
        const uint32_t x = (uint32_t)__shfl_up((int)v, d);
        if (lane >= d) v += x;
    }
    return v;
}

__device__ __forceinline__ void inline_offsets(const uint32_t *count, int T, uint32_t *s_off, uint32_t *s_wave )
{
    const int tid = threadIdx.x, lane = tid & 63, wave = tid >> 6;
    const int per = (T + BLOCK - 1) / BLOCK;
    const int b = min(T, tid * per), e = min(T, b + per);
    uint32_t c[16];
    uint32_t sum = 0;
#pragma unroll
    for (int k = 0; k < 16; k++) { c[k] = (k < per && b + k < e) ? count[b + k] : 0u; sum += c[k]; }
    const uint32_t incl = wave_incl_scan_u32(sum, lane);
    if (lane == WAVE - 1) s_wave[wave] = incl;
    __syncthreads();
    uint32_t pre = incl - sum;
    for (int w = 0; w < wave; w++) pre += s_wave[w];
#pragma unroll
    for (int k = 0; k < 16; k++)
        if (k < per && b + k < e) { s_off[b + k] = pre; pre += c[k]; }
    if (tid == BLOCK - 1) s_off[T] = pre;
    __syncthreads();
}

struct InlineScanLds {
    uint32_t chunk[NSCAN][BLOCK];
    uint32_t wave_tot[NSCAN][BLOCK / WAVE];
    uint32_t total[NSCAN];
    uint32_t wave_deep[BLOCK / WAVE];
    uint32_t deepest;
};

__device__ __forceinline__ void inline_scan_build(const uint32_t *count, int T, uint32_t L, int sort_np, InlineScanLds &S)
{
    const int tid = threadIdx.x, lane = tid & 63, wave = tid >> 6;
    const int per = (T + BLOCK - 1) / BLOCK;
    const int b = min(T, tid * per), e = min(T, b + per);
    uint32_t run[NSCAN];
    uint32_t deepest = 0;
#pragma unroll
    for (int k = 0; k < NSCAN; k++) run[k] = 0;
    for (int t = b; t < e; t++) {
        uint32_t q[NSCAN];
        tile_terms(count[t], L, q, sort_np);
        deepest = max(deepest, q[0]);
#pragma unroll
        for (int k = 0; k < NSCAN; k++) run[k] += q[k];
    }
    for (int d = 32; d >= 1; d >>= 1) deepest = max(deepest, (uint32_t)__shfl_xor((int)deepest, d));
    if (lane == 0) S.wave_deep[wave] = deepest;
    uint32_t incl[NSCAN];
#pragma unroll
// ... 988 lines not shown
```

### gaussian-mesh-splatting_amd/csrc/torch_binding.cpp

```cpp
#include <torch/extension.h>

#include <ATen/hip/impl/HIPGuardImplMasqueradingAsCUDA.h>
#include <ATen/hip/impl/HIPStreamMasqueradingAsCUDA.h>

#include <atomic>
#include <map>
#include <mutex>
#include <optional>
#include <tuple>
#include <vector>

#include "../../include/gmsplat.h"

namespace {

using torch::Tensor;
using torch::autograd::AutogradContext;
using torch::autograd::variable_list;

inline void *stream_of(c10::Device d) { return (void *)c10::hip::getCurrentHIPStreamMasqueradingAsCUDA(d.index()).stream(); }
inline void *stream_of(const Tensor &t) { return stream_of(t.device()); }
inline const float *cf(const Tensor &t) { return (t.defined() && t.numel()) ? t.data_ptr<float>() : nullptr; }
inline float *mf(const Tensor &t) { return (t.defined() && t.numel()) ? t.data_ptr<float>() : nullptr; }

inline Tensor f32c(const Tensor &t)
{
    if (!t.defined() || t.numel() == 0) return t;
    Tensor r = t.scalar_type() == torch::kFloat ? t : t.to(torch::kFloat);
    return r.is_contiguous() ? r : r.contiguous();
}

inline void require_gpu(const Tensor &t)
{
    TORCH_CHECK(!t.defined() || t.numel() == 0 || t.is_cuda(),
                "diff_gaussian_rasterization (MI355X/HIP build): tensors must live on a GPU; there is no CPU path in the "
                "product (the CPU oracle lives under oracle/ for tests only)");
}

inline void check_rc(int64_t rc, const char *what)
{
    TORCH_CHECK(rc >= 0, what, " failed (", rc, "): ", gms_last_error());
}

struct Slot { Tensor t; c10::Device dev; bool failed; };
void *alloc_cb(void *ctx, size_t bytes)
{
    Slot *s = static_cast<Slot *>(ctx);
    try {
        s->t = torch::empty({(int64_t)(bytes > 0 ? bytes : 1)}, torch::TensorOptions().dtype(torch::kUInt8).device(s->dev));
        return s->t.data_ptr();
    } catch (...) {
        s->failed = true;
        return nullptr;
    }
}

std::mutex g_mu;
std::map<std::tuple<int, int, int, int64_t>, int64_t> g_capacity;
std::map<std::tuple<int, void *, int64_t>, Tensor> g_accum;

static int64_t quantize_capacity(int64_t x)
{
    if (x < 16) return x;
    const int s = 63 - __builtin_clzll((unsigned long long)x) - 3;
    return ((x + ((int64_t)1 << s) - 1) >> s) << s;
}

struct LastCall { int64_t num_rendered = 0, num_units = 0, hint = 0, P = 0; int W = 0, H = 0; Tensor radii, image, binning, geom; } g_last;
std::atomic<bool> g_keep_buffers{false};

struct Forward {
    int64_t num_rendered = 0, num_units = 0, capacity = 0;
    int64_t ticket[2] = {0, 0}, launched_units = 0;
    Tensor color, radii, invdepth, geom, binning, image;
};
static std::atomic<int> g_defer_counts{-1};
bool deferred_counts()
{
    int v = g_defer_counts.load();
    if (v < 0) { const char *e = getenv("GMS_DEFER_COUNTS"); int expected = -1; g_defer_counts.compare_exchange_strong(expected, (e && atoi(e) != 0) ? 1 : 0); v = g_defer_counts.load(); }
    return v != 0;
}
void set_deferred_counts(bool on) { g_defer_counts.store(on ? 1 : 0); }
static std::atomic<int> g_fused_mesh_bwd{-1};
bool fused_mesh_backward()
{
    int v = g_fused_mesh_bwd.load();
    if (v < 0) { const char *e = getenv("GMS_TRAIN_FUSED_BWD"); int expected = -1; g_fused_mesh_bwd.compare_exchange_strong(expected, (e && atoi(e) == 0) ? 0 : 1); v = g_fused_mesh_bwd.load(); }
    return v != 0;
}
void set_fused_mesh_backward(bool on) { g_fused_mesh_bwd.store(on ? 1 : 0); }
struct MeshOut { Tensor xyz, scaling_act, rotation_unit, opacity_act; };

struct FrameSettings { Tensor bg, view, proj, campos; int64_t H, W; double tanx, tany, mod; int64_t D; bool prefiltered, aa, debug; };
FrameSettings frame_settings(c10::Device dev, const Tensor &bg, const Tensor &view, const Tensor &proj, const Tensor &campos, int64_t H,
                             int64_t W, double tanx, double tany, double mod, int64_t D, bool prefiltered, bool aa, bool debug)
{
    require_gpu(bg); require_gpu(view); require_gpu(proj); require_gpu(campos);
    return {f32c(bg.to(dev)), f32c(view.to(dev)), f32c(proj.to(dev)), f32c(campos.to(dev)), H, W, tanx, tany, mod, D, prefiltered, aa, debug};
}
struct Gaussians { Tensor sh, sh_rest, means3D, colors, opac, scales, rots, cov; };
Gaussians tensor_gaussians(const Tensor &means3D, const Tensor &sh, const Tensor &sh_rest, const Tensor &colors, const Tensor &opac,
                           const Tensor &scales, const Tensor &rots, const Tensor &cov)
{
    require_gpu(means3D);
    TORCH_CHECK(means3D.dim() == 2 && means3D.size(1) == 3, "means3D must have dimensions (num_points, 3)");
    return {f32c(sh), f32c(sh_rest), f32c(means3D), f32c(colors), f32c(opac), f32c(scales), f32c(rots), f32c(cov)};
}

Forward forward_core(const FrameSettings &s, int64_t P, c10::Device dev, const Gaussians &g, const Tensor &visible, bool use_hint,
                     const GmsMeshArgs *mesh = nullptr, const MeshOut *mesh_out = nullptr, bool may_defer = false, const GmsPointsArgs *points = nullptr)
{
    c10::hip::OptionalHIPGuardMasqueradingAsCUDA guard(dev);
    const bool has_sh = g.sh.defined() && g.sh.numel() > 0;
    if (has_sh) TORCH_CHECK(g.sh.dim() == 3 && g.sh.size(0) == P && g.sh.size(2) == 3, "sh must have dimensions (num_points, num_coeffs, 3)");
    int64_t M = has_sh ? g.sh.size(1) : 0;
    const bool split = g.sh_rest.defined() && g.sh_rest.numel() > 0;
    if (split) M = g.sh.size(1) + g.sh_rest.size(1);

    auto fopt = torch::TensorOptions().dtype(torch::kFloat).device(dev);
    Forward f;
    f.color = torch::empty({3, s.H, s.W}, fopt);
    f.invdepth = torch::empty({1, s.H, s.W}, fopt);
    f.radii = torch::empty({P}, fopt.dtype(torch::kInt));

    int64_t hint = 0;
    const auto key = std::make_tuple((int)dev.index(), (int)s.W, (int)s.H, P);
    if (use_hint && !gms_get_deterministic()) {
        std::lock_guard<std::mutex> lk(g_mu);
        auto it = g_capacity.find(key);
        if (it != g_capacity.end()) hint = quantize_capacity(it->second + it->second / 4 + 4096);
    }
    void *stream = stream_of(dev);
    hipStreamCaptureStatus cap_status = hipStreamCaptureStatusNone;
    const bool capturing = hipStreamIsCapturing((hipStream_t)stream, &cap_status) == hipSuccess && cap_status != hipStreamCaptureStatusNone;
    if (capturing)
        TORCH_CHECK(hint > 0 && P > 0, "rasterizing inside a stream capture needs the capacity hint of this shape: render it at least once on the "
                                        "same stream before the capture (not in deterministic mode)");
    Slot geom{Tensor(), dev, false}, binning{Tensor(), dev, false}, image{Tensor(), dev, false};
    int64_t num_units = 0;
    GmsRasterForwardArgs a{};
    a.P = (int32_t)P; a.D = (int32_t)s.D; a.M = (int32_t)M; a.width = (int32_t)s.W; a.height = (int32_t)s.H;
    a.background = cf(s.bg); a.means3D = cf(g.means3D); a.shs = cf(g.sh); a.shs_rest = split ? cf(g.sh_rest) : nullptr;
    a.colors_precomp = cf(g.colors); a.opacities = cf(g.opac); a.scales = cf(g.scales); a.rotations = cf(g.rots);
    a.cov3D_precomp = cf(g.cov); a.viewmatrix = cf(s.view); a.projmatrix = cf(s.proj); a.campos = cf(s.campos);
    a.scale_modifier = (float)s.mod; a.tan_fovx = (float)s.tanx; a.tan_fovy = (float)s.tany;
    a.prefiltered = s.prefiltered; a.antialiasing = s.aa; a.debug = s.debug;
    a.out_color = mf(f.color); a.out_invdepth = mf(f.invdepth); a.radii = P ? f.radii.data_ptr<int32_t>() : nullptr;
    a.geom_alloc = alloc_cb; a.geom_ctx = &geom; a.binning_alloc = alloc_cb; a.binning_ctx = &binning;
    a.image_alloc = alloc_cb; a.image_ctx = &image;
    a.binning_capacity_hint = hint;
    a.visible = (visible.defined() && visible.numel()) ? static_cast<uint8_t *>(visible.data_ptr()) : nullptr;
    a.num_units_out = &num_units;
    a.no_host_wait = capturing ? 1 : 0;
    a.mesh = mesh;
    a.points = points;
    if (mesh && mesh_out) {
        a.mesh_out_xyz = mf(mesh_out->xyz); a.mesh_out_scaling_act = mf(mesh_out->scaling_act);
        a.mesh_out_rotation_unit = mf(mesh_out->rotation_unit); a.mesh_out_opacity_act = mf(mesh_out->opacity_act);
    }
    int64_t ticket[2] = {0, 0};
    const bool defer = may_defer && hint > 0 && !capturing && P > 0 && deferred_counts();
    if (defer) a.count_ticket_out = ticket;
    const int64_t n = gms_rasterize_forward(&a, stream);
    TORCH_CHECK(!(geom.failed || binning.failed || image.failed), "scratch allocation failed (out of device memory?)");
    check_rc(n, "gms_rasterize_forward");
    f.num_rendered = n; f.num_units = num_units;
    f.capacity = (hint > 0 && n <= hint) ? hint : (n > 0 ? n : 1);
    f.geom = geom.t; f.binning = binning.t; f.image = image.t;
    if (defer) { f.ticket[0] = ticket[0]; f.ticket[1] = ticket[1]; f.launched_units = gms_last_launched_units(); f.num_rendered = -1; f.capacity = hint; }
    {
        std::lock_guard<std::mutex> lk(g_mu);
        int64_t &c = g_capacity[key];
        if (!capturing && !defer) c = std::max(n, (int64_t)(0.97 * (double)c));
        g_last.num_rendered = n; g_last.num_units = num_units; g_last.hint = hint; g_last.P = P; g_last.W = (int)s.W; g_last.H = (int)s.H;
        if (g_keep_buffers.load()) { g_last.radii = f.radii; g_last.image = f.image; g_last.binning = f.binning; g_last.geom = f.geom; }
    }
    return f;
}

struct Backward { Tensor dmeans2D, dcolors, dopacity, dmeans3D, dcov3D, dsh, dsh_rest, dscales, drots; };
struct MeshGrads { Tensor d_vertices, d_alpha, d_scale, d_opacity; };

static std::atomic<bool> g_sh_factor{false};
static std::map<int, std::vector<Tensor>> g_factors;
constexpr size_t MAX_QUEUED_FACTORS = 256;

Backward alloc_backward(const Gaussians &g)
{
    const int64_t P = g.means3D.size(0);
    auto fopt = torch::TensorOptions().dtype(torch::kFloat).device(g.means3D.device());
    const bool has_sh = g.sh.defined() && g.sh.numel() > 0, split = g.sh_rest.defined() && g.sh_rest.numel() > 0;
    const bool has_cov = g.cov.defined() && g.cov.numel() > 0;
    Backward b;
    b.dmeans2D = torch::empty({P, 3}, fopt);
    b.dopacity = torch::empty(g.opac.sizes(), fopt);
    b.dmeans3D = torch::empty({P, 3}, fopt);
    const bool factor = has_sh && g_sh_factor.load();
    if (!has_sh) b.dcolors = torch::empty({P, 3}, fopt);
    if (factor) b.dcolors = torch::empty({P + 1, 3}, fopt);
    if (has_sh && !factor) b.dsh = torch::empty(g.sh.sizes(), fopt);
    if (split && !factor) b.dsh_rest = torch::empty(g.sh_rest.sizes(), fopt);
    if (has_cov) b.dcov3D = torch::empty({P, 6}, fopt);
    else { b.dscales = torch::empty({P, 3}, fopt); b.drots = torch::empty({P, 4}, fopt); }
    return b;
}

Backward backward_core(const FrameSettings &s, const Gaussians &g, const Forward &f, const Tensor &dL_dcolor_, const Tensor &dL_dinvd_,
                       const Backward *prealloc = nullptr, const GmsMeshArgs *mesh = nullptr, const MeshGrads *mesh_grads = nullptr)
{
    const auto dev = g.means3D.device();
    c10::hip::OptionalHIPGuardMasqueradingAsCUDA guard(dev);
    const int64_t P = g.means3D.size(0);
    const bool has_sh = g.sh.defined() && g.sh.numel() > 0, split = g.sh_rest.defined() && g.sh_rest.numel() > 0;
    int64_t M = has_sh ? g.sh.size(1) : 0;
    if (split) M = g.sh.size(1) + g.sh_rest.size(1);
    auto fopt = torch::TensorOptions().dtype(torch::kFloat).device(dev);
    Tensor gcol = f32c(dL_dcolor_), ginv = f32c(dL_dinvd_);
    void *stream = stream_of(dev);
    Tensor accum;
    const auto akey = std::make_tuple((int)dev.index(), stream, P);
    {
        std::lock_guard<std::mutex> lk(g_mu);
        auto it = g_accum.find(akey);
        if (it != g_accum.end()) { accum = it->second; g_accum.erase(it); }
    }
    if (!accum.defined()) accum = torch::zeros({std::max<int64_t>(P, 1), 16}, fopt);
    Backward b = prealloc ? *prealloc : alloc_backward(g);
    GmsRasterBackwardArgs a{};
    a.P = (int32_t)P; a.D = (int32_t)s.D; a.M = (int32_t)M; a.width = (int32_t)s.W; a.height = (int32_t)s.H;
    a.num_rendered = f.num_rendered; a.binning_capacity = f.capacity;
    a.background = cf(s.bg); a.means3D = cf(g.means3D); a.shs = cf(g.sh); a.shs_rest = split ? cf(g.sh_rest) : nullptr;
    a.colors_precomp = cf(g.colors); a.opacities = cf(g.opac); a.scales = cf(g.scales); a.rotations = cf(g.rots); a.cov3D_precomp = cf(g.cov);
    a.viewmatrix = cf(s.view); a.projmatrix = cf(s.proj); a.campos = cf(s.campos);
    a.scale_modifier = (float)s.mod; a.tan_fovx = (float)s.tanx; a.tan_fovy = (float)s.tany; a.antialiasing = s.aa; a.debug = s.debug;
    a.radii = P ? f.radii.data_ptr<int32_t>() : nullptr;
    a.geom_buffer = f.geom.numel() ? f.geom.data_ptr() : nullptr;
    a.binning_buffer = f.binning.numel() ? f.binning.data_ptr() : nullptr;
    a.image_buffer = f.image.numel() ? f.image.data_ptr() : nullptr;
    a.dL_dout_color = cf(gcol); a.dL_dout_invdepth = cf(ginv);
    a.grad_accum = mf(accum); a.dL_dmeans2D = mf(b.dmeans2D); a.dL_dopacity = mf(b.dopacity); a.dL_dcolors = mf(b.dcolors);
    a.dL_dmeans3D = mf(b.dmeans3D); a.dL_dcov3D = mf(b.dcov3D); a.dL_dsh = mf(b.dsh); a.dL_dsh_rest = mf(b.dsh_rest);
    a.dL_dscales = mf(b.dscales); a.dL_drotations = mf(b.drots);
    a.grad_accum_rezero = 1; a.num_units = f.num_units;
    if (mesh && mesh_grads) {
        a.mesh = mesh; a.mesh_dL_dvertices = mf(mesh_grads->d_vertices); a.mesh_dL_dalpha = mf(mesh_grads->d_alpha);
        a.mesh_dL_dscale = mf(mesh_grads->d_scale); a.mesh_dL_d_opacity = mf(mesh_grads->d_opacity);
    }
    a.sh_factor_mode = (has_sh && b.dcolors.defined()) ? 1 : 0;
    a.factor_campos_row = (a.sh_factor_mode && b.dcolors.size(0) == P + 1) ? 1 : 0;
    if (a.sh_factor_mode) {
        std::lock_guard<std::mutex> lk(g_mu);
        TORCH_CHECK(g_factors[(int)dev.index()].size() < MAX_QUEUED_FACTORS, "factorised SH mode: ", MAX_QUEUED_FACTORS,
                    " factors queued on this device and never taken (call take_sh_factors() every step, or set_sh_factor_mode(False))");
    }
    if (P > 0) check_rc(gms_rasterize_backward(&a, stream), "gms_rasterize_backward");
    if (a.sh_factor_mode) {
        std::lock_guard<std::mutex> lk(g_mu);
        g_factors[(int)dev.index()].push_back(b.dcolors);
    }
    {
        std::lock_guard<std::mutex> lk(g_mu);
        if (g_accum.size() >= 8) g_accum.clear();
        g_accum[akey] = accum;
    }
    return b;
}

std::tuple<int64_t, Tensor, Tensor, Tensor, Tensor, Tensor, Tensor>
rasterize_gaussians(const Tensor &background, const Tensor &means3D, const Tensor &colors, const Tensor &opacity, const Tensor &scales,
                    const Tensor &rotations, double scale_modifier, const Tensor &cov3D_precomp, const Tensor &viewmatrix,
                    const Tensor &projmatrix, double tan_fovx, double tan_fovy, int64_t image_height, int64_t image_width,
                    const Tensor &sh, int64_t degree, const Tensor &campos, bool prefiltered, bool antialiasing, bool debug)
{
    const Gaussians g = tensor_gaussians(means3D, sh, Tensor(), colors, opacity, scales, rotations, cov3D_precomp);
    const FrameSettings s = frame_settings(means3D.device(), background, viewmatrix, projmatrix, campos, image_height, image_width, tan_fovx,
                                           tan_fovy, scale_modifier, degree, prefiltered, antialiasing, debug);
    Forward f = forward_core(s, means3D.size(0), means3D.device(), g, Tensor(), false);
    return std::make_tuple(f.num_rendered, f.color, f.radii, f.geom, f.binning, f.image, f.invdepth);
}

std::tuple<Tensor, Tensor, Tensor, Tensor, Tensor, Tensor, Tensor, Tensor>
rasterize_gaussians_backward(const Tensor &background, const Tensor &means3D, const Tensor &radii, const Tensor &colors,
                             const Tensor &opacities, const Tensor &scales, const Tensor &rotations, double scale_modifier,
                             const Tensor &cov3D_precomp, const Tensor &viewmatrix, const Tensor &projmatrix, double tan_fovx,
                             double tan_fovy, const Tensor &dL_dout_color, const Tensor &dL_dout_invdepth, const Tensor &sh,
                             int64_t degree, const Tensor &campos, const Tensor &geomBuffer, int64_t R, const Tensor &binningBuffer,
                             const Tensor &imageBuffer, bool antialiasing, bool debug)
{
    const Gaussians g = tensor_gaussians(means3D, sh, Tensor(), colors, opacities, scales, rotations, cov3D_precomp);
    const int64_t H = dL_dout_color.defined() ? dL_dout_color.size(-2) : 0, W = dL_dout_color.defined() ? dL_dout_color.size(-1) : 0;
    const FrameSettings s = frame_settings(means3D.device(), background, viewmatrix, projmatrix, campos, H, W, tan_fovx, tan_fovy,
                                           scale_modifier, degree, false, antialiasing, debug);
    Forward f;
    f.radii = radii; f.geom = geomBuffer; f.binning = binningBuffer; f.image = imageBuffer; f.num_rendered = R; f.capacity = R > 0 ? R : 1;
    Backward b = backward_core(s, g, f, dL_dout_color, dL_dout_invdepth);
    return std::make_tuple(b.dmeans2D, b.dcolors, b.dopacity, b.dmeans3D, b.dcov3D, b.dsh, b.dscales, b.drots);
}

Tensor mark_visible(const Tensor &means3D, const Tensor &viewmatrix, const Tensor &projmatrix)
{
    require_gpu(means3D);
    c10::hip::OptionalHIPGuardMasqueradingAsCUDA guard(means3D.device());
    Tensor pos = f32c(means3D.detach()), view = f32c(viewmatrix.to(means3D.device())), proj = f32c(projmatrix.to(means3D.device()));
    Tensor present = torch::empty({pos.size(0)}, torch::TensorOptions().dtype(torch::kUInt8).device(pos.device()));
    check_rc(gms_mark_visible((int32_t)pos.size(0), cf(pos), cf(view), cf(proj), pos.size(0) ? present.data_ptr<uint8_t>() : nullptr,
                              stream_of(pos)), "gms_mark_visible");
    return present.to(torch::kBool);
}

void save_frame(AutogradContext *ctx, std::vector<Tensor> tensors, const FrameSettings &s, const Forward &f)
{
    tensors.insert(tensors.end(), {f.radii, f.geom, f.binning, f.image, s.bg, s.view, s.proj, s.campos});
    ctx->save_for_backward(tensors);
    auto &d = ctx->saved_data;
    d["H"] = s.H; d["W"] = s.W; d["tanx"] = s.tanx; d["tany"] = s.tany; d["mod"] = s.mod; d["D"] = s.D; d["aa"] = s.aa; d["debug"] = s.debug;
    d["R"] = f.num_rendered; d["units"] = f.num_units; d["cap"] = f.capacity;
    d["ticket0"] = f.ticket[0]; d["ticket1"] = f.ticket[1]; d["launched"] = f.launched_units;
}
std::pair<FrameSettings, Forward> load_frame(AutogradContext *ctx, const variable_list &saved)
{
    auto &d = ctx->saved_data;
    const size_t k = saved.size() - 8;
    FrameSettings s{saved[k + 4], saved[k + 5], saved[k + 6], saved[k + 7], d["H"].toInt(), d["W"].toInt(), d["tanx"].toDouble(),
                    d["tany"].toDouble(), d["mod"].toDouble(), d["D"].toInt(), false, d["aa"].toBool(), d["debug"].toBool()};
    Forward f;
    f.radii = saved[k]; f.geom = saved[k + 1]; f.binning = saved[k + 2]; f.image = saved[k + 3];
    f.num_rendered = d["R"].toInt(); f.num_units = d["units"].toInt(); f.capacity = d["cap"].toInt();
    f.ticket[0] = d["ticket0"].toInt(); f.ticket[1] = d["ticket1"].toInt(); f.launched_units = d["launched"].toInt();
    return {s, f};
}

void redeem_counts(AutogradContext *ctx, const FrameSettings &s, Forward &f, const Tensor &means3D)
{
    if (f.ticket[0] == 0) return;
    const auto dev = means3D.device();
    const int64_t P = means3D.size(0);
    c10::hip::OptionalHIPGuardMasqueradingAsCUDA guard(dev);
    int64_t units = 0, deepest = 0;
    const int64_t n = gms_rasterize_forward_counts(f.ticket, (int32_t)s.W, (int32_t)s.H, (int32_t)P, &units, &deepest, stream_of(dev));
    check_rc(n, "gms_rasterize_forward_counts");
    {
        std::lock_guard<std::mutex> lk(g_mu);
        int64_t &c = g_capacity[std::make_tuple((int)dev.index(), (int)s.W, (int)s.H, P)];
        c = std::max(n, (int64_t)(0.97 * (double)c));
        g_last.num_rendered = n; g_last.num_units = units;
    }
    TORCH_CHECK(n <= f.capacity && units <= f.launched_units,
                "GMS_DEFERRED_OVERFLOW: the frame held ", n, " instances / ", units, " work units but was launched for ", f.capacity, " / ", f.launched_units,
                " (deferred read-back of the instance count: diff_gaussian_rasterization.set_deferred_counts): its image is incomplete -- "
                "redo this step (the capacity hint has been raised; or render it with set_deferred_counts(False))");
    f.ticket[0] = 0; f.num_rendered = n; f.num_units = units;
// ... 575 lines not shown
    const auto dev = in.tables[0].device();
    const int64_t V = in.tables[0].size(0), J = (int64_t)in.parents.size(), L = in.tables[1].size(0);
    TORCH_CHECK(J >= 2 && J <= GMS_FLAME_MAX_JOINTS, "flame: ", J, " joints (2 .. ", GMS_FLAME_MAX_JOINTS, " are supported)");
    TORCH_CHECK(V <= INT32_MAX / 3 && in.tables[0].numel() == V * 3 && in.tables[1].numel() == L * V * 3 && in.tables[2].numel() == (J - 1) * 9 * V * 3 &&
                in.tables[3].numel() == V * J && in.tables[4].numel() == J * 3 && in.tables[5].numel() == L * J * 3, "flame: model table sizes do not fit together");
    m = GmsFlameModel{};
    m.V = (int32_t)V; m.J = (int32_t)J; m.L = (int32_t)L;
    for (int64_t j = 0; j < J; j++) m.parents[j] = (int32_t)in.parents[j];
    m.v_template = cf(in.tables[0]); m.shapedirs = cf(in.tables[1]); m.posedirs = cf(in.tables[2]);
    m.lbs_weights = cf(in.tables[3]); m.joints_template = cf(in.tables[4]); m.joints_shapedirs = cf(in.tables[5]);
    auto param = [&](Tensor &t, int64_t n, const char *name) {
        if (!t.defined()) return;
        require_gpu(t);
        TORCH_CHECK(t.scalar_type() == torch::kFloat, "flame: ", name, " must be a float32 tensor (the kernels and their gradients are float32), got ",
                    t.scalar_type());
        t = f32c(t);
        TORCH_CHECK(t.numel() == n && (n == 0 || t.device() == dev), "flame: ", name, " must hold ", n, " values on the model's device (batch 1 only)");
    };
    TORCH_CHECK(in.shape.defined() && in.expression.defined(), "flame: shape and expression parameters are required");
    TORCH_CHECK(in.shape.numel() + in.expression.numel() == L, "flame: the model is packed for ", L, " shape + expression columns, got ",
                in.shape.numel(), " + ", in.expression.numel(), " (batch 1 only)");
    param(in.shape, in.shape.numel(), "shape_params");
    param(in.expression, in.expression.numel(), "expression_params");
    param(in.transl, 3, "transl");
    param(in.enlargement, V * 3, "enlargement");
    p = GmsFlameParams{};
    p.shape = cf(in.shape); p.expression = cf(in.expression);
    p.n_shape = (int32_t)in.shape.numel(); p.n_expression = (int32_t)in.expression.numel();
    size_t k = 0;
    for (Tensor &r : in.rots) {
        TORCH_CHECK(r.defined() && r.numel() % 3 == 0, "flame: a rotation tensor holds 3 values per joint");
        param(r, r.numel(), "pose");
        for (int64_t q = 0; q < r.numel() / 3; q++, k++) {
            TORCH_CHECK(k < in.rot_joints.size() && in.rot_joints[k] >= 0 && in.rot_joints[k] < J && !p.joint_rot[in.rot_joints[k]],
                        "flame: every rotation triple needs one joint of its own in [0, J)");
            p.joint_rot[in.rot_joints[k]] = cf(r) + 3 * q;
        }
    }
    TORCH_CHECK(k == in.rot_joints.size(), "flame: ", in.rot_joints.size(), " joints named for ", k, " rotation triples");
    p.transl = cf(in.transl);
    p.enlargement = cf(in.enlargement);
    p.enlargement_scalar = (float)in.enlargement_scalar;
    p.swap = in.swap ? 1 : 0;
}

Tensor flame_run_forward(FlameInputs &in, Tensor *saved)
{
    GmsFlameModel m;
    GmsFlameParams p;
    flame_fill(in, m, p);
    const auto dev = in.tables[0].device();
    c10::hip::OptionalHIPGuardMasqueradingAsCUDA guard(dev);
    auto fopt = torch::TensorOptions().dtype(torch::kFloat).device(dev);
    Tensor out = torch::empty({(int64_t)m.V, 3}, fopt);
    if (saved) *saved = torch::empty({(int64_t)GMS_FLAME_SAVED_FLOATS(m.V)}, fopt);
    check_rc(gms_flame_forward(&m, &p, mf(out), saved ? mf(*saved) : nullptr, stream_of(dev)), "gms_flame_forward");
    return out;
}

class FlameFn : public torch::autograd::Function<FlameFn> {
public:
    static Tensor forward(AutogradContext *ctx, at::TensorList rots, Tensor shape, Tensor expression, std::optional<Tensor> transl,
                          std::optional<Tensor> enlargement, const FlameInputs *st)
    {
        ctx->set_materialize_grads(false);
        FlameInputs in = *st;
        in.rots.assign(rots.begin(), rots.end());
        in.shape = shape; in.expression = expression;
        in.transl = transl ? *transl : Tensor(); in.enlargement = enlargement ? *enlargement : Tensor();
        Tensor saved;
        Tensor out = flame_run_forward(in, &saved);
        variable_list keep(in.rots.begin(), in.rots.end());
        auto fopt = out.options();
        keep.push_back(in.shape); keep.push_back(in.expression);
        keep.push_back(in.transl.defined() ? in.transl : torch::empty({0}, fopt));
        keep.push_back(in.enlargement.defined() ? in.enlargement : torch::empty({0}, fopt));
        keep.push_back(saved);
        for (const Tensor &t : in.tables) keep.push_back(t);
        ctx->save_for_backward(keep);
        ctx->saved_data["n_rots"] = (int64_t)in.rots.size();
        ctx->saved_data["parents"] = in.parents;
        ctx->saved_data["rot_joints"] = in.rot_joints;
        ctx->saved_data["enlargement_scalar"] = in.enlargement_scalar;
        ctx->saved_data["swap"] = in.swap;
        return out;
    }

    static variable_list backward(AutogradContext *ctx, variable_list g)
    {
        auto s = ctx->get_saved_variables();
        const size_t nr = (size_t)ctx->saved_data["n_rots"].toInt();
        variable_list grads(nr + 5);
        if (!g[0].defined()) return grads;
        FlameInputs in;
        in.rots.assign(s.begin(), s.begin() + nr);
        in.shape = s[nr]; in.expression = s[nr + 1];
        if (s[nr + 2].numel()) in.transl = s[nr + 2];
        if (s[nr + 3].numel()) in.enlargement = s[nr + 3];
        const Tensor &saved = s[nr + 4];
        in.tables.assign(s.begin() + nr + 5, s.end());
        in.parents = ctx->saved_data["parents"].toIntVector();
        in.rot_joints = ctx->saved_data["rot_joints"].toIntVector();
        in.enlargement_scalar = ctx->saved_data["enlargement_scalar"].toDouble();
        in.swap = ctx->saved_data["swap"].toBool();
        GmsFlameModel m;
        GmsFlameParams p;
        flame_fill(in, m, p);
        const auto dev = in.tables[0].device();
        c10::hip::OptionalHIPGuardMasqueradingAsCUDA guard(dev);
        Tensor gv = f32c(g[0]);
        TORCH_CHECK(gv.numel() == (int64_t)m.V * 3 && gv.device() == dev, "flame backward: gradient of the vertices must be [V,3] on the model's device");
        GmsFlameGrads gr{};
        size_t k = 0;
        for (size_t i = 0; i < nr; i++) {
            const int64_t n = in.rots[i].numel() / 3;
            if (ctx->needs_input_grad(i)) {
                grads[i] = torch::empty_like(in.rots[i]);
                for (int64_t q = 0; q < n; q++) gr.d_joint_rot[in.rot_joints[k + q]] = mf(grads[i]) + 3 * q;
            }
            k += (size_t)n;
        }
        if (ctx->needs_input_grad(nr) && in.shape.numel()) { grads[nr] = torch::empty_like(in.shape); gr.d_shape = mf(grads[nr]); }
        if (ctx->needs_input_grad(nr + 1) && in.expression.numel()) { grads[nr + 1] = torch::empty_like(in.expression); gr.d_expression = mf(grads[nr + 1]); }
        size_t edge = nr + 2;
        if (in.transl.defined() && ctx->needs_input_grad(edge++)) { grads[nr + 2] = torch::empty_like(in.transl); gr.d_transl = mf(grads[nr + 2]); }
        if (in.enlargement.defined() && ctx->needs_input_grad(edge++)) { grads[nr + 3] = torch::empty_like(in.enlargement); gr.d_enlargement = mf(grads[nr + 3]); }
        const size_t bytes = gms_flame_workspace_bytes(m.V, m.J, m.L);
        Tensor work = torch::empty({(int64_t)bytes}, torch::TensorOptions().dtype(torch::kUInt8).device(dev));
        check_rc(gms_flame_backward(&m, &p, cf(saved), cf(gv), &gr, work.data_ptr(), bytes, stream_of(dev)), "gms_flame_backward");
        return grads;
    }
};

FlameInputs flame_inputs(const std::vector<Tensor> &tables, const std::vector<int64_t> &parents, const std::vector<Tensor> &rots,
                         const std::vector<std::vector<int64_t>> &rot_joints, const Tensor &shape, const Tensor &expression,
                         const std::optional<Tensor> &transl, const std::optional<Tensor> &enlargement, double enlargement_scalar, bool swap)
{
    TORCH_CHECK(rots.size() == rot_joints.size(), "flame: one list of joints per rotation tensor");
    FlameInputs in;
    in.tables = tables; in.parents = parents; in.rots = rots;
    for (size_t i = 0; i < rots.size(); i++) {
        TORCH_CHECK(rots[i].defined() && (int64_t)rot_joints[i].size() * 3 == rots[i].numel(), "flame: a rotation tensor holds 3 values for each of its joints (batch 1 only)");
        in.rot_joints.insert(in.rot_joints.end(), rot_joints[i].begin(), rot_joints[i].end());
    }
    in.shape = shape; in.expression = expression;
    if (transl) in.transl = *transl;
    if (enlargement) in.enlargement = *enlargement;
    in.enlargement_scalar = enlargement_scalar; in.swap = swap;
    return in;
}

Tensor flame_vertices(const std::vector<Tensor> &tables, const std::vector<int64_t> &parents, const std::vector<Tensor> &rots,
                      const std::vector<std::vector<int64_t>> &rot_joints, const Tensor &shape, const Tensor &expression,
                      const std::optional<Tensor> &transl, const std::optional<Tensor> &enlargement, double enlargement_scalar, bool swap)
{
    FlameInputs in = flame_inputs(tables, parents, rots, rot_joints, shape, expression, transl, enlargement, enlargement_scalar, swap);
    auto opt = [](const Tensor &t) { return t.defined() ? std::optional<Tensor>(t) : std::nullopt; };
    return FlameFn::apply(at::TensorList(in.rots), in.shape, in.expression, opt(in.transl), opt(in.enlargement), (const FlameInputs *)&in);
}

Tensor flame_forward(const std::vector<Tensor> &tables, const std::vector<int64_t> &parents, const std::vector<Tensor> &rots,
                     const std::vector<std::vector<int64_t>> &rot_joints, const Tensor &shape, const Tensor &expression,
                     const std::optional<Tensor> &transl, const std::optional<Tensor> &enlargement, double enlargement_scalar, bool swap)
{
    FlameInputs in = flame_inputs(tables, parents, rots, rot_joints, shape, expression, transl, enlargement, enlargement_scalar, swap);
    return flame_run_forward(in, nullptr);
}

const float *densify_f32(const Tensor &t, int64_t numel, c10::Device dev, const char *what)
{
    TORCH_CHECK(t.defined() && t.scalar_type() == torch::kFloat && t.is_contiguous() && t.numel() == numel && (numel == 0 || t.device() == dev),
                "densify: ", what, " must be a contiguous float32 tensor of ", numel, " values on the model's device");
    return numel ? t.data_ptr<float>() : nullptr;
}

void densify_stats(const Tensor &radii, const Tensor &viewspace_grad, const std::optional<Tensor> &max_radii2D, Tensor xyz_gradient_accum, Tensor denom)
{
    require_gpu(radii);
    const int64_t P = radii.numel();
    const c10::Device dev = radii.device();
    TORCH_CHECK(radii.scalar_type() == torch::kInt && radii.is_contiguous(), "densify_stats: radii must be a contiguous int32 tensor");
    TORCH_CHECK(viewspace_grad.dim() == 2 && viewspace_grad.size(1) == 3, "densify_stats: the screen-space gradient must have dimensions (P, 3)");
    const float *g = densify_f32(viewspace_grad, 3 * P, dev, "viewspace_grad");
    float *mr = max_radii2D.has_value() && max_radii2D->defined() ? const_cast<float *>(densify_f32(*max_radii2D, P, dev, "max_radii2D")) : nullptr;
    float *ac = const_cast<float *>(densify_f32(xyz_gradient_accum, P, dev, "xyz_gradient_accum"));
    float *dn = const_cast<float *>(densify_f32(denom, P, dev, "denom"));
    if (P == 0) return;
    c10::hip::OptionalHIPGuardMasqueradingAsCUDA guard(dev);
    check_rc(gms_densify_stats(P, radii.data_ptr<int32_t>(), g, mr, ac, dn, stream_of(dev)), "gms_densify_stats");
}

std::tuple<Tensor, Tensor, std::vector<int64_t>> densify_plan(const Tensor &xyz_gradient_accum, const Tensor &denom, const Tensor &opacity,
                                                              const Tensor &scaling, double grad_threshold, double dense_threshold,
                                                              double min_opacity, bool prune_world, double world_threshold, double eps_s0)
{
    require_gpu(scaling);
    TORCH_CHECK(scaling.dim() == 2, "densify_plan: scaling must have dimensions (P, 2) or (P, 3)");
    const int64_t P = scaling.size(0), S = scaling.size(1);
    const c10::Device dev = scaling.device();
    const float *sc = densify_f32(scaling, P * S, dev, "scaling"), *ac = densify_f32(xyz_gradient_accum, P, dev, "xyz_gradient_accum");
    const float *dn = densify_f32(denom, P, dev, "denom"), *op = densify_f32(opacity, P, dev, "opacity");
    c10::hip::OptionalHIPGuardMasqueradingAsCUDA guard(dev);
    auto iopt = torch::TensorOptions().dtype(torch::kInt).device(dev);
    Tensor src = torch::empty({2 * P}, iopt), kind = torch::empty({2 * P}, iopt);
    const size_t bytes = gms_densify_plan_workspace_bytes(P);
    Tensor work = torch::empty({(int64_t)bytes}, torch::TensorOptions().dtype(torch::kUInt8).device(dev));
    std::vector<int64_t> counts(5, 0);
    check_rc(gms_densify_plan(P, (int32_t)S, ac, dn, op, sc, (float)grad_threshold, (float)dense_threshold, (float)min_opacity, prune_world ? 1 : 0,
                              (float)world_threshold, (float)eps_s0, P ? src.data_ptr<int32_t>() : nullptr, P ? kind.data_ptr<int32_t>() : nullptr,
                              counts.data(), work.data_ptr(), bytes, P ? stream_of(dev) : nullptr),
             "gms_densify_plan");
    return {src.narrow(0, 0, counts[0]), kind.narrow(0, 0, counts[0]), counts};
}

std::tuple<std::vector<Tensor>, std::vector<Tensor>, std::vector<Tensor>> densify_apply(const Tensor &src, const Tensor &kind, const std::vector<Tensor> &params,
                                                                                        const std::vector<Tensor> &exp_avg, const std::vector<Tensor> &exp_avg_sq,
                                                                                        const Tensor &noise, double eps_s0)
{
    TORCH_CHECK(params.size() == 6, "densify_apply: six parameter tensors expected (xyz, f_dc, f_rest, opacity, scaling, rotation)");
    const bool moments = !exp_avg.empty() || !exp_avg_sq.empty();
    TORCH_CHECK(!moments || (exp_avg.size() == 6 && exp_avg_sq.size() == 6), "densify_apply: six tensors of each Adam moment, or none");
    require_gpu(params[0]); require_gpu(src);
    const int64_t P = params[0].size(0), P_new = src.numel();
    const c10::Device dev = params[0].device();
    TORCH_CHECK(src.scalar_type() == torch::kInt && kind.scalar_type() == torch::kInt && src.is_contiguous() && kind.is_contiguous() && kind.numel() == P_new &&
                (P_new == 0 || (src.device() == dev && kind.device() == dev)), "densify_apply: src and kind must be contiguous int32 [P'] on the model's device");
    const float *z = densify_f32(noise, 6 * P, dev, "noise [2,P,3]");
    c10::hip::OptionalHIPGuardMasqueradingAsCUDA guard(dev);
    GmsDensifyTensor t[6];
    std::vector<Tensor> po(6), mo, vo;
    for (int g = 0; g < 6; g++) {
        const Tensor &p = params[g];
        TORCH_CHECK(p.defined() && p.dim() >= 1 && p.size(0) == P, "densify_apply: parameter ", g, " does not have P rows");
        const int64_t width = P ? p.numel() / P : 0;
        std::vector<int64_t> shape = p.sizes().vec();
        shape[0] = P_new;
        po[g] = torch::empty(shape, p.options());
        t[g] = GmsDensifyTensor{densify_f32(p, P * width, dev, "a parameter"), nullptr, nullptr, P_new * width ? po[g].data_ptr<float>() : nullptr,
                                nullptr, nullptr, (int32_t)width};
        if (moments) {
            mo.push_back(torch::empty(shape, p.options())); vo.push_back(torch::empty(shape, p.options()));
            t[g].exp_avg = densify_f32(exp_avg[g], P * width, dev, "exp_avg");
            t[g].exp_avg_sq = densify_f32(exp_avg_sq[g], P * width, dev, "exp_avg_sq");
            if (P_new * width) { t[g].exp_avg_out = mo[g].data_ptr<float>(); t[g].exp_avg_sq_out = vo[g].data_ptr<float>(); }
        }
    }
    if (P_new == 0 || P == 0) return {po, mo, vo};
    check_rc(gms_densify_apply(P, P_new, src.data_ptr<int32_t>(), kind.data_ptr<int32_t>(), t, z, (float)eps_s0, stream_of(dev)), "gms_densify_apply");
    return {po, mo, vo};
}

void adam_step(const std::vector<Tensor> &params, const std::vector<Tensor> &grads, const std::vector<Tensor> &exp_avg,
               const std::vector<Tensor> &exp_avg_sq, const std::vector<double> &lrs, const std::vector<int64_t> &steps, double beta1,
               double beta2, double eps)
{
    const size_t n = params.size();
    TORCH_CHECK(grads.size() == n && exp_avg.size() == n && exp_avg_sq.size() == n && lrs.size() == n && steps.size() == n, "adam_step: list sizes differ");
    if (n == 0) return;
    std::vector<GmsAdamTensor> t(n);
    std::vector<Tensor> keep;
    for (size_t i = 0; i < n; i++) {
        require_gpu(params[i]);
        TORCH_CHECK(params[i].scalar_type() == torch::kFloat && params[i].is_contiguous(), "FusedAdam needs contiguous float32 parameters");
        TORCH_CHECK(exp_avg[i].is_contiguous() && exp_avg_sq[i].is_contiguous(), "FusedAdam needs contiguous optimizer state");
        Tensor g = f32c(grads[i]);
        keep.push_back(g);
        t[i] = GmsAdamTensor{params[i].data_ptr<float>(), g.data_ptr<float>(), exp_avg[i].data_ptr<float>(), exp_avg_sq[i].data_ptr<float>(),
                             params[i].numel(), (float)lrs[i], (int32_t)steps[i]};
    }
    c10::hip::OptionalHIPGuardMasqueradingAsCUDA guard(params[0].device());
    check_rc(gms_adam_step(t.data(), (int32_t)n, beta1, beta2, eps, stream_of(params[0])), "gms_adam_step");
}

}

PYBIND11_MODULE(TORCH_EXTENSION_NAME, m)
{
    m.doc() = "MI355X-native diff_gaussian_rasterization._C (PyTorch-ROCm binding of libgmsplat.so)";
    using nogil = py::call_guard<py::gil_scoped_release>;
    m.def("rasterize_gaussians", &rasterize_gaussians, nogil());
    m.def("rasterize_gaussians_backward", &rasterize_gaussians_backward, nogil());
    m.def("mark_visible", &mark_visible, nogil());
    m.def("rasterize", &rasterize, "differentiable rasterization (autograd node in C++)", nogil());
    m.def("mesh_to_gaussians", &mesh_to_gaussians, "differentiable mesh-face -> Gaussian parameterization", nogil());
    m.def("render_mesh_forward", &render_mesh_forward, "forward-only frame straight from a mesh (K0 inside the preprocess thread)", nogil());
    m.def("points_to_gaussians", &points_to_gaussians, "differentiable pseudo-triangle -> Gaussian: [xyz, scaling_raw, rotation_raw, scaling_act, rotation_unit(, opacity_act)]", nogil());
    m.def("points_prepare_vertices", &points_prepare_vertices, "Gaussian -> pseudo-triangle [P,3,3] (prepare_vertices)", nogil());
    m.def("render_points_forward", &render_points_forward, "forward-only frame straight from pseudo-triangles (the points op inside the preprocess thread)", nogil());
    m.def("bind_pseudomesh", &bind_pseudomesh, "bind pseudo-triangles [P,3,3] to the nearest faces of a guide mesh: (face_idx int32 [P], alpha [P,3,3], n_degenerate)", nogil());
    m.def("bind_apply", &bind_apply, "pseudo-triangles [P,3,3] of a binding on (edited) guide vertices; launches only", py::arg("face_idx"), py::arg("alpha"),
          py::arg("guide_vertices"), py::arg("guide_faces"), py::arg("out") = py::none(), nogil());
    m.def("densify_stats", &densify_stats, "per-iteration densification statistics, in place on (max_radii2D, xyz_gradient_accum, denom); one launch", nogil());
    m.def("densify_plan", &densify_plan, "clone / split / prune decisions as a source map: (src int32 [P'], kind int32 [P'], counts)", nogil());
    m.def("densify_apply", &densify_apply, "gather the six parameters and their Adam moments through a plan: (params, exp_avg, exp_avg_sq)", nogil());
    m.def("flame_vertices", &flame_vertices, "differentiable FLAME layer (+ axis swap and enlargement): vertices [V,3], one autograd node", py::arg("tables"),
          py::arg("parents"), py::arg("rots"), py::arg("rot_joints"), py::arg("shape"), py::arg("expression"), py::arg("transl") = py::none(),
          py::arg("enlargement") = py::none(), py::arg("enlargement_scalar") = 1.0, py::arg("swap") = false, nogil());
    m.def("flame_forward", &flame_forward, "the FLAME layer without a graph: one launch", py::arg("tables"), py::arg("parents"), py::arg("rots"),
          py::arg("rot_joints"), py::arg("shape"), py::arg("expression"), py::arg("transl") = py::none(), py::arg("enlargement") = py::none(),
          py::arg("enlargement_scalar") = 1.0, py::arg("swap") = false, nogil());
    m.def("render_mesh", &render_mesh, "differentiable frame straight from a mesh: [image, radii, invdepth, xyz, scaling_act, rotation_unit, opacity_act]", nogil());
    m.def("l1_ssim", &l1_ssim, "differentiable w_l1 * L1 + w_ssim * SSIM + bias; returns (value [0-dim], [l1, ssim])", nogil());
    m.def("adam_step", &adam_step, nogil());
    m.def("set_keep_buffers", &set_keep_buffers, "keep references to the last forward's scratch tensors (diagnostics only)");
    m.def("clear_accum", &clear_accum);
    m.def("set_sh_factor_mode", &set_sh_factor_mode, "factorised SH gradient: backward calls queue [P+1,3] factors instead of writing dL/dsh");
    m.def("sh_factor_mode", &sh_factor_mode);
    m.def("take_sh_factors", &take_sh_factors, py::arg("device") = -1);
    m.def("sh_grad_expand", &sh_grad_expand, "dsh (+)= sum_v Y(dir_v) (x) factor_v over the [V,P+1,3] factors", nogil());
    m.def("last_stats", &last_stats);
    m.def("set_deferred_counts", &set_deferred_counts, "read the frame's instance count back at the start of the backward instead of inside the forward (opt-in)");
    m.def("deferred_counts", &deferred_counts);
    m.def("set_fused_mesh_backward", &set_fused_mesh_backward, "frames rendered straight from a mesh: run the mesh backward inside preprocess_bwd (default on)");
    m.def("fused_mesh_backward", &fused_mesh_backward);
    m.def("set_capacity", &set_capacity);
    m.def("clear_capacity", &clear_capacity);
    m.def("abi_version", []() { return (int64_t)gms_abi_version(); });
    m.def("image_counts_offset", [](int64_t w, int64_t h) { return (int64_t)gms_image_counts_offset((int32_t)w, (int32_t)h); });
    m.def("last_launched_units", []() { return (int64_t)gms_last_launched_units(); });
}
```

### gaussian-mesh-splatting_amd/diff_gaussian_rasterization/__init__.py

```python
from __future__ import annotations

import ctypes as C
import os
from typing import NamedTuple, Optional

import torch
import torch.nn as nn

from . import _lib

_BINDING = os.environ.get("GMS_BINDING", "auto")
try:
    if _BINDING == "ctypes":
        raise ImportError("GMS_BINDING=ctypes")
    from . import _C
except ImportError as _e:
    if _BINDING == "torch":
        raise
    _C = None

__all__ = ["GaussianRasterizationSettings", "GaussianRasterizer", "rasterize_gaussians", "last_stats", "SplitSH", "keep_buffers",
           "set_capacity_hint", "clear_capacity_hints"]


class SplitSH:

    def __init__(self, dc: torch.Tensor, rest: torch.Tensor):
        self.dc, self.rest = dc, rest
        self._full = None

    def full(self) -> torch.Tensor:
        if self._full is None:
            self._full = torch.cat((self.dc, self.rest), dim=1)
        return self._full

    @property
    def shape(self):
        return torch.Size((self.dc.shape[0], self.dc.shape[1] + self.rest.shape[1], self.dc.shape[2]))

    def __getattr__(self, name):
        return getattr(self.full(), name)


class GaussianRasterizationSettings(NamedTuple):
    image_height: int
    image_width: int
    tanfovx: float
    tanfovy: float
    bg: torch.Tensor
    scale_modifier: float
    viewmatrix: torch.Tensor
    projmatrix: torch.Tensor
    sh_degree: int
    campos: torch.Tensor
    prefiltered: bool
    debug: bool
    antialiasing: bool


_capacity_cache = {}
_last_stats = {}


def _quantize_capacity(x: int) -> int:
    if x < 16:
        return x
    s = x.bit_length() - 1 - 3
    return ((x + (1 << s) - 1) >> s) << s


def set_capacity_hint(device_index: int, width: int, height: int, P: int, value: int) -> None:
    if _C is not None:
        _C.set_capacity(int(device_index), int(width), int(height), int(P), int(value))
    elif value < 0:
        _capacity_cache.pop((device_index, width, height, P), None)
    else:
        _capacity_cache[(device_index, width, height, P)] = int(value)


def clear_capacity_hints() -> None:
    if _C is not None:
        _C.clear_capacity()
    _capacity_cache.clear()


def set_upstream_scale_mod_grad(on: bool) -> None:
    _lib.load().gms_set_upstream_scale_mod_grad(1 if on else 0)


def set_deterministic(on: bool) -> None:
    _lib.load().gms_set_deterministic(1 if on else 0)


def deterministic() -> bool:
    return bool(_lib.load().gms_get_deterministic())


DEFERRED_OVERFLOW = "GMS_DEFERRED_OVERFLOW"


def set_deferred_counts(on: bool) -> None:
    if _C is None:
        raise NotImplementedError("the deferred read-back needs the _C extension module (GMS_BINDING=ctypes drives the blocking form)")
    _C.set_deferred_counts(bool(on))


def deferred_counts() -> bool:
    return bool(_C is not None and _C.deferred_counts())


def set_sh_factor_mode(on: bool) -> None:
    if _C is None:
        raise NotImplementedError("the factorised SH gradient needs the _C extension module (GMS_BINDING=ctypes has no such path)")
    _C.set_sh_factor_mode(bool(on))


def sh_factor_mode() -> bool:
    return _C is not None and bool(_C.sh_factor_mode())


def take_sh_factors(device=None) -> list:
    if _C is None:
        return []
    idx = -1 if device is None else (device if isinstance(device, int) else (torch.device(device).index if torch.device(device).index is not None else -1))
    return list(_C.take_sh_factors(int(idx)))


def sh_grad_expand(factors: torch.Tensor, means3D: torch.Tensor, sh_degree: int, dL_dsh: torch.Tensor,
                   dL_dsh_rest: Optional[torch.Tensor] = None, accumulate: bool = False) -> None:
    if _C is None:
        raise NotImplementedError("sh_grad_expand needs the _C extension module")
    _C.sh_grad_expand(factors, means3D, int(sh_degree), dL_dsh, dL_dsh_rest if dL_dsh_rest is not None else torch.Tensor(), bool(accumulate))


_keep_buffers = False


def keep_buffers(on: bool = True) -> None:
    global _keep_buffers
    _keep_buffers = bool(on)
    if _C is not None:
        _C.set_keep_buffers(bool(on))
    if not on:
        for k in ("radii", "image", "binning", "geom"):
            _last_stats.pop(k, None)


def raw_buffers() -> dict:
    d = _C.last_stats() if _C is not None else _last_stats
    return {k: d.get(k) for k in ("geom", "binning", "image")}


def last_stats() -> dict:
    d = dict(_C.last_stats()) if _C is not None else dict(_last_stats)
    radii = d.pop("radii", None)
    if radii is not None:
        d["visible"] = int((radii > 0).sum())
    d.pop("binning", None)
    d.pop("geom", None)
    image = d.pop("image", None)
    if image is not None and image.numel():
        off = int(_lib.load().gms_image_n_contrib_offset(d["width"], d["height"]))
        d["interactions"] = int(image[off:off + 4 * d["width"] * d["height"]].view(torch.int32).sum(dtype=torch.int64))
        micro = bool(d.get("used_micro", int(_lib.load().gms_last_used_micro())))
        d["interactions_kind"] = "micro_tile_block_list_positions" if micro else "tile_list_positions"
    return d


def _f32c(t: Optional[torch.Tensor]) -> Optional[torch.Tensor]:
    if t is None:
        return None
    if t.dtype != torch.float32:
        t = t.float()
    return t if t.is_contiguous() else t.contiguous()


class _Scratch:

    def __init__(self, device):
        self.device = device
        self.tensors = {}
        self.error = None

        def make(name):
            def cb(_ctx, nbytes):
                try:
                    t = torch.empty(max(int(nbytes), 1), dtype=torch.uint8, device=self.device)
                    self.tensors[name] = t
                    return t.data_ptr()
                except Exception as e:
                    self.error = e
                    return None
            return _lib.ALLOC_FN(cb)

        self.geom_cb, self.binning_cb, self.image_cb = make("geom"), make("binning"), make("image")


_empties = {}


def _empty(device):
    e = _empties.get(device)
    if e is None:
        e = _empties[device] = torch.empty(0, device=device)
    return e


def _cpu_copy(x):
    if torch.is_tensor(x):
        return x.detach().cpu().clone()
    if isinstance(x, SplitSH):
        return (_cpu_copy(x.dc), _cpu_copy(x.rest))
    if isinstance(x, tuple):
        return tuple(_cpu_copy(v) for v in x)
    return x


def rasterize_gaussians(means3D, means2D, sh, colors_precomp, opacities, scales, rotations, cov3Ds_precomp,
                        raster_settings, visible_out=None):
    if raster_settings.debug:
        snapshot = _cpu_copy((means3D, means2D, sh, colors_precomp, opacities, scales, rotations, cov3Ds_precomp,
                              tuple(raster_settings)))
        try:
            return _rasterize_gaussians(means3D, means2D, sh, colors_precomp, opacities, scales, rotations, cov3Ds_precomp,
                                        raster_settings, visible_out)
        except Exception:
            torch.save(snapshot, "snapshot_fw.dump")
            print("\nAn error occured in forward. Please forward snapshot_fw.dump for debugging.")
            raise
    return _rasterize_gaussians(means3D, means2D, sh, colors_precomp, opacities, scales, rotations, cov3Ds_precomp,
                                raster_settings, visible_out)


def _rasterize_gaussians(means3D, means2D, sh, colors_precomp, opacities, scales, rotations, cov3Ds_precomp,
                         raster_settings, visible_out=None):
    if _C is not None:
        rs = raster_settings
        e = _empty(means3D.device)
        rest = e
        if isinstance(sh, SplitSH):
            if sh.dc.shape[1] == 1 and sh.rest.shape[1] == 15 and sh.dc.is_cuda:
                sh, rest = sh.dc, sh.rest
            else:
                sh = sh.full()
        return _C.rasterize(means3D, means2D, sh, rest, colors_precomp, opacities, scales, rotations, cov3Ds_precomp, rs.bg,
                            rs.viewmatrix, rs.projmatrix, rs.campos, int(rs.image_height), int(rs.image_width), float(rs.tanfovx),
                            float(rs.tanfovy), float(rs.scale_modifier), int(rs.sh_degree), bool(rs.prefiltered),
                            bool(rs.antialiasing), bool(rs.debug), visible_out if visible_out is not None else e,
                            os.environ.get("GMS_SYNC_BINNING", "0") != "1")
    if isinstance(sh, SplitSH):
        if sh.dc.shape[1] == 1 and sh.rest.shape[1] == 15 and sh.dc.is_cuda:
            return _RasterizeGaussians.apply(means3D, means2D, sh.dc, colors_precomp, opacities, scales, rotations,
                                             cov3Ds_precomp, raster_settings, sh.rest, visible_out)
        sh = sh.full()
    return _RasterizeGaussians.apply(means3D, means2D, sh, colors_precomp, opacities, scales, rotations,
                                     cov3Ds_precomp, raster_settings, None, visible_out)


_accum_cache = {}


class _RasterizeGaussians(torch.autograd.Function):
    @staticmethod
    def forward(ctx, means3D, means2D, sh, colors_precomp, opacities, scales, rotations, cov3Ds_precomp,
                raster_settings, sh_rest=None, visible_out=None):
        rs = raster_settings
        lib = _lib.load()
        _lib.require_gpu(means3D, rs.bg, rs.viewmatrix, rs.projmatrix, rs.campos)
        device = means3D.device
        ctx.set_materialize_grads(False)
        if means3D.dim() != 2 or means3D.shape[1] != 3:
            raise RuntimeError("means3D must have dimensions (num_points, 3)")
        P = int(means3D.shape[0])
        H, W = int(rs.image_height), int(rs.image_width)

        means3D = _f32c(means3D)
        sh = _f32c(sh) if sh.numel() else sh
        colors_precomp = _f32c(colors_precomp) if colors_precomp.numel() else colors_precomp
        opacities = _f32c(opacities)
        scales = _f32c(scales) if scales.numel() else scales
        rotations = _f32c(rotations) if rotations.numel() else rotations
        cov3Ds_precomp = _f32c(cov3Ds_precomp) if cov3Ds_precomp.numel() else cov3Ds_precomp
        bg, view, proj, campos = (_f32c(t.to(device)) for t in (rs.bg, rs.viewmatrix, rs.projmatrix, rs.campos))
        if sh.numel() and (sh.dim() != 3 or sh.shape[0] != P or sh.shape[2] != 3):
            raise RuntimeError("sh must have dimensions (num_points, num_coeffs, 3)")
        M = int(sh.shape[1]) if sh.numel() else 0
        if sh_rest is not None:
            sh_rest = _f32c(sh_rest)
            M = int(sh.shape[1] + sh_rest.shape[1])

        color = torch.empty((3, H, W), dtype=torch.float32, device=device)
        invdepth = torch.empty((1, H, W), dtype=torch.float32, device=device)
        radii = torch.empty((P,), dtype=torch.int32, device=device)

        scratch = _Scratch(device)
        key = (device.index, W, H, P)
        hint = 0
        if os.environ.get("GMS_SYNC_BINNING", "0") != "1" and not lib.gms_get_deterministic():
            prev = _capacity_cache.get(key)
            if prev is not None:
                hint = _quantize_capacity(int(prev * 1.25) + 4096)
        num_units = C.c_int64(0)
        a = _lib.RasterForwardArgs(
            P=P, D=int(rs.sh_degree), M=M, width=W, height=H,
            background=_lib.ptr(bg), means3D=_lib.ptr(means3D), shs=_lib.ptr(sh), shs_rest=_lib.ptr(sh_rest),
            colors_precomp=_lib.ptr(colors_precomp), opacities=_lib.ptr(opacities), scales=_lib.ptr(scales),
            rotations=_lib.ptr(rotations), cov3D_precomp=_lib.ptr(cov3Ds_precomp), viewmatrix=_lib.ptr(view),
            projmatrix=_lib.ptr(proj), campos=_lib.ptr(campos), scale_modifier=float(rs.scale_modifier),
            tan_fovx=float(rs.tanfovx), tan_fovy=float(rs.tanfovy), prefiltered=int(bool(rs.prefiltered)),
            antialiasing=int(bool(rs.antialiasing)), debug=int(bool(rs.debug)),
            out_color=_lib.ptr(color), out_invdepth=_lib.ptr(invdepth), radii=_lib.ptr(radii),
            visible=_lib.ptr(visible_out) if visible_out is not None else None,
            num_units_out=C.addressof(num_units),
            geom_alloc=scratch.geom_cb, geom_ctx=None, binning_alloc=scratch.binning_cb, binning_ctx=None,
            image_alloc=scratch.image_cb, image_ctx=None, binning_capacity_hint=hint)
        with _lib.on_device(device):
            stream = _lib.stream_ptr(device)
            num_rendered = lib.gms_rasterize_forward(C.byref(a), C.c_void_p(stream))
        if num_rendered < 0:
            if scratch.error is not None:
                raise scratch.error
            _lib.check(num_rendered, "gms_rasterize_forward")
        _capacity_cache[key] = max(int(num_rendered), int(0.97 * _capacity_cache.get(key, 0)))
        _last_stats.update(num_rendered=int(num_rendered), num_units=int(num_units.value), capacity_hint=hint, P=P, width=W, height=H,
                           deepest_tile=int(lib.gms_last_deepest_tile()), used_micro=int(lib.gms_last_used_micro()))
        if _keep_buffers:
            _last_stats.update(radii=radii, image=scratch.tensors.get("image"), binning=scratch.tensors.get("binning"),
                               geom=scratch.tensors.get("geom"))

        ctx.raster_settings = rs
        ctx.num_rendered = int(num_rendered)
        ctx.num_units = int(num_units.value)
        ctx.binning_capacity = hint if (hint > 0 and num_rendered <= hint) else max(int(num_rendered), 1)
        ctx.M = M
        empty = torch.empty(0, device=device)
        ctx.split = sh_rest is not None
        ctx.save_for_backward(means3D, sh, sh_rest if sh_rest is not None else empty, colors_precomp, opacities, scales,
                              rotations, cov3Ds_precomp, radii,
                              scratch.tensors.get("geom", empty), scratch.tensors.get("binning", empty),
                              scratch.tensors.get("image", empty), bg, view, proj, campos)
        ctx.mark_non_differentiable(radii)
        return color, radii, invdepth

    @staticmethod
    def backward(ctx, grad_color, _grad_radii, grad_invdepth):
        lib = _lib.load()
        rs = ctx.raster_settings
        (means3D, sh, sh_rest, colors_precomp, opacities, scales, rotations, cov3Ds_precomp, radii, geom, binning, image,
         bg, view, proj, campos) = ctx.saved_tensors
        device = means3D.device
        P = int(means3D.shape[0])
        H, W = int(rs.image_height), int(rs.image_width)
        M = ctx.M
        use_sh, use_cov = sh.numel() > 0, cov3Ds_precomp.numel() > 0

        grad_color = _f32c(grad_color) if grad_color is not None else torch.zeros((3, H, W), device=device)
        grad_invdepth = _f32c(grad_invdepth) if grad_invdepth is not None else None

        stream = _lib.stream_ptr(device)
        accum_key = (device.index, stream, P)
        grad_accum = _accum_cache.pop(accum_key, None)
        if grad_accum is None:
            grad_accum = torch.zeros((max(P, 1), 16), dtype=torch.float32, device=device)
        dL_dmeans2D = torch.empty((P, 3), dtype=torch.float32, device=device)
        dL_dopacity = torch.empty(opacities.shape, dtype=torch.float32, device=device)
        dL_dcolors = torch.empty((P, 3), dtype=torch.float32, device=device) if not use_sh else None
        dL_dmeans3D = torch.empty((P, 3), dtype=torch.float32, device=device)
        dL_dsh = torch.empty(sh.shape, dtype=torch.float32, device=device) if use_sh else None
        dL_dsh_rest = torch.empty(sh_rest.shape, dtype=torch.float32, device=device) if ctx.split else None
        dL_dscales = torch.empty((P, 3), dtype=torch.float32, device=device) if not use_cov else None
        dL_drot = torch.empty((P, 4), dtype=torch.float32, device=device) if not use_cov else None
        dL_dcov3D = torch.empty((P, 6), dtype=torch.float32, device=device) if use_cov else None

        a = _lib.RasterBackwardArgs(
            P=P, D=int(rs.sh_degree), M=M, width=W, height=H, num_rendered=ctx.num_rendered,
            binning_capacity=ctx.binning_capacity,
            background=_lib.ptr(bg), means3D=_lib.ptr(means3D), shs=_lib.ptr(sh),
            shs_rest=_lib.ptr(sh_rest) if ctx.split else None, colors_precomp=_lib.ptr(colors_precomp),
            opacities=_lib.ptr(opacities), scales=_lib.ptr(scales), rotations=_lib.ptr(rotations),
            cov3D_precomp=_lib.ptr(cov3Ds_precomp), viewmatrix=_lib.ptr(view), projmatrix=_lib.ptr(proj),
            campos=_lib.ptr(campos), scale_modifier=float(rs.scale_modifier), tan_fovx=float(rs.tanfovx),
            tan_fovy=float(rs.tanfovy), antialiasing=int(bool(rs.antialiasing)), debug=int(bool(rs.debug)),
            radii=_lib.ptr(radii), geom_buffer=_lib.ptr(geom), binning_buffer=_lib.ptr(binning),
            image_buffer=_lib.ptr(image), dL_dout_color=_lib.ptr(grad_color), dL_dout_invdepth=_lib.ptr(grad_invdepth),
            grad_accum=_lib.ptr(grad_accum), dL_dmeans2D=_lib.ptr(dL_dmeans2D), dL_dopacity=_lib.ptr(dL_dopacity),
            dL_dcolors=_lib.ptr(dL_dcolors), dL_dmeans3D=_lib.ptr(dL_dmeans3D),
            dL_dcov3D=_lib.ptr(dL_dcov3D), dL_dsh=_lib.ptr(dL_dsh), dL_dsh_rest=_lib.ptr(dL_dsh_rest),
            dL_dscales=_lib.ptr(dL_dscales),
            dL_drotations=_lib.ptr(dL_drot), grad_accum_rezero=1, num_units=ctx.num_units)
        if P > 0:
            try:
                with _lib.on_device(device):
                    _lib.check(lib.gms_rasterize_backward(C.byref(a), C.c_void_p(stream)), "gms_rasterize_backward")
            except Exception:
                if rs.debug:
                    torch.save(_cpu_copy((means3D, sh, colors_precomp, opacities, scales, rotations, cov3Ds_precomp, radii,
                                          grad_color, tuple(rs))), "snapshot_bw.dump")
                    print("\nAn error occured in backward. Writing snapshot_bw.dump for debugging.\n")
                raise
        if len(_accum_cache) >= 8:
            _accum_cache.clear()
        _accum_cache[accum_key] = grad_accum
        return (dL_dmeans3D, dL_dmeans2D, dL_dsh, dL_dcolors, dL_dopacity, dL_dscales, dL_drot,
                dL_dcov3D, None, dL_dsh_rest, None)


class GaussianRasterizer(nn.Module):
    def __init__(self, raster_settings: GaussianRasterizationSettings):
        super().__init__()
        self.raster_settings = raster_settings

    def markVisible(self, positions: torch.Tensor) -> torch.Tensor:
        rs = self.raster_settings
        if _C is not None:
            with torch.no_grad():
                return _C.mark_visible(positions, rs.viewmatrix, rs.projmatrix)
        lib = _lib.load()
        _lib.require_gpu(positions)
        with torch.no_grad():
            pos = _f32c(positions)
            present = torch.empty((pos.shape[0],), dtype=torch.uint8, device=pos.device)
            view, proj = _f32c(rs.viewmatrix.to(pos.device)), _f32c(rs.projmatrix.to(pos.device))
            with _lib.on_device(pos.device):
                stream = _lib.stream_ptr(pos.device)
                _lib.check(lib.gms_mark_visible(int(pos.shape[0]), _lib.ptr(pos), _lib.ptr(view), _lib.ptr(proj),
                                                _lib.ptr(present), C.c_void_p(stream)), "gms_mark_visible")
        return present.bool()

    def forward(self, means3D, means2D, opacities, shs=None, colors_precomp=None, scales=None, rotations=None,
                cov3D_precomp=None):
        rs = self.raster_settings
        if (shs is None and colors_precomp is None) or (shs is not None and colors_precomp is not None):
            raise Exception("Please provide excatly one of either SHs or precomputed colors!")
        if ((scales is None or rotations is None) and cov3D_precomp is None) or \
                ((scales is not None or rotations is not None) and cov3D_precomp is not None):
            raise Exception("Please provide exactly one of either scale/rotation pair or precomputed 3D covariance!")
        e = torch.Tensor([]).to(means3D.device)
        shs = e if shs is None else shs
        colors_precomp = e if colors_precomp is None else colors_precomp
        scales = e if scales is None else scales
        rotations = e if rotations is None else rotations
        cov3D_precomp = e if cov3D_precomp is None else cov3D_precomp
        vis = torch.empty((means3D.shape[0],), dtype=torch.bool, device=means3D.device) if means3D.is_cuda and means3D.shape[0] else None
        out = rasterize_gaussians(means3D, means2D, shs, colors_precomp, opacities, scales, rotations, cov3D_precomp, rs, vis)
        self.visibility_filter = vis
        return out
```

Baseline: 3000.

## Cache SH direction Jacobian in forward pass and drop SH staging in backward

The forward preprocess now computes the 3x3 Jacobian of the SH colour with respect to view direction while evaluating colour, and stores 9 floats per Gaussian in geometry scratch. The backward preprocess no longer stages the full SH coefficient rows (up to 48 floats per Gaussian) into LDS. It reads the cached Jacobian to get the direction gradient, and writes dL/dsh from the SH basis times dRGB. This trades a large SH read in backward for a small extra write in forward and a small read in backward, with more scratch memory per Gaussian. A diagnostic scratch-fill option is also added.

```diff
diff --git a/gaussian-mesh-splatting_amd/csrc/gms_common.h b/gaussian-mesh-splatting_amd/csrc/gms_common.h
--- a/gaussian-mesh-splatting_amd/csrc/gms_common.h
+++ b/gaussian-mesh-splatting_amd/csrc/gms_common.h
@@ -35,9 +35,12 @@
     float *depth;
     uint8_t *clamped;
     ushort4 *rect;
+    float *sh_ddir;
+    static constexpr size_t SH_DDIR = 9;
     static __host__ __device__ size_t bytes(size_t P)
     {
-        return align_up(P * sizeof(SplatRec), 256) + align_up(P * 4, 256) + align_up(P, 256) + align_up(P * sizeof(ushort4), 256);
+        return align_up(P * sizeof(SplatRec), 256) + align_up(P * 4, 256) + align_up(P, 256) + align_up(P * sizeof(ushort4), 256) +
+               align_up(P * SH_DDIR * 4, 256);
     }
     static __host__ __device__ GeomState carve(void *base, size_t P)
     {
@@ -46,7 +49,8 @@
         g.rec = (SplatRec *)p; p += align_up(P * sizeof(SplatRec), 256);
         g.depth = (float *)p;  p += align_up(P * 4, 256);
         g.clamped = (uint8_t *)p; p += align_up(P, 256);
-        g.rect = (ushort4 *)p;
+        g.rect = (ushort4 *)p; p += align_up(P * sizeof(ushort4), 256);
+        g.sh_ddir = (float *)p;
         return g;
     }
 };
diff --git a/gaussian-mesh-splatting_amd/csrc/gms_project.h b/gaussian-mesh-splatting_amd/csrc/gms_project.h
--- a/gaussian-mesh-splatting_amd/csrc/gms_project.h
+++ b/gaussian-mesh-splatting_amd/csrc/gms_project.h
@@ -70,4 +70,76 @@
     e.c0 = e.T1[0] * e.ST1[0] + e.T1[1] * e.ST1[1] + e.T1[2] * e.ST1[2];
 }
 
+template <int DEG, typename SH>
+__device__ __forceinline__ void sh_eval_with_dir_jacobian(SH sh, float x, float y, float z, float res[3], float D[9])
+{
+#pragma clang fp contract(off)
+#pragma unroll
+    for (int j = 0; j < 9; j++) D[j] = 0.f;
+#define GMS_SH_K(K, BV, AXES)                                                      \
+    {                                                                              \
+        const float s[3] = {sh((K), 0), sh((K), 1), sh((K), 2)};                   \
+        const float bv = (BV);                                                     \
+        _Pragma("unroll") for (int c = 0; c < 3; c++) res[c] = res[c] + bv * s[c]; \
+        AXES                                                                       \
+    }
+#define GMS_DDIR_AXIS(A, BD)                                                       \
+    {                                                                              \
+        const float bd = (BD);                                                     \
+        _Pragma("unroll") for (int c = 0; c < 3; c++) D[(A) * 3 + c] = __fmaf_rn(bd, s[c], D[(A) * 3 + c]); \
+    }
+#define GMS_SH_FENCE()                                                             \
+    __asm__ volatile("" : "+v"(x), "+v"(y), "+v"(z), "+v"(xx), "+v"(yy), "+v"(zz), "+v"(xy), "+v"(yz), "+v"(xz),       \
+                          "+v"(res[0]), "+v"(res[1]), "+v"(res[2]), "+v"(D[0]), "+v"(D[1]), "+v"(D[2]), "+v"(D[3]), "+v"(D[4]), \
+                          "+v"(D[5]), "+v"(D[6]), "+v"(D[7]), "+v"(D[8]));
+#define GMS_DDIR_X(BD) GMS_DDIR_AXIS(0, BD)
+#define GMS_DDIR_Y(BD) GMS_DDIR_AXIS(1, BD)
+#define GMS_DDIR_Z(BD) GMS_DDIR_AXIS(2, BD)
+#pragma unroll
+    for (int c = 0; c < 3; c++) res[c] = SH_C0 * sh(0, c);
+    if (DEG > 0) {
+        GMS_SH_K(1, -(SH_C1 * y), GMS_DDIR_Y(-SH_C1))
+        GMS_SH_K(2, SH_C1 * z, GMS_DDIR_Z(SH_C1))
+        GMS_SH_K(3, -(SH_C1 * x), GMS_DDIR_X(-SH_C1))
+    }
+    if (DEG > 1) {
+        float xx = x * x, yy = y * y, zz = z * z, xy = x * y, yz = y * z, xz = x * z;
+        GMS_SH_FENCE()
+        GMS_SH_K(4, SH_C2[0] * xy, GMS_DDIR_X(SH_C2[0] * y) GMS_DDIR_Y(SH_C2[0] * x))
+        GMS_SH_K(5, SH_C2[1] * yz, GMS_DDIR_Y(SH_C2[1] * z) GMS_DDIR_Z(SH_C2[1] * y))
+        GMS_SH_K(6, SH_C2[2] * (2.f * zz - xx - yy), GMS_DDIR_X(-2.f * SH_C2[2] * x) GMS_DDIR_Y(-2.f * SH_C2[2] * y) GMS_DDIR_Z(4.f * SH_C2[2] * z))
+        GMS_SH_FENCE()
+        GMS_SH_K(7, SH_C2[3] * xz, GMS_DDIR_X(SH_C2[3] * z) GMS_DDIR_Z(SH_C2[3] * x))
+        GMS_SH_K(8, SH_C2[4] * (xx - yy), GMS_DDIR_X(2.f * SH_C2[4] * x) GMS_DDIR_Y(-2.f * SH_C2[4] * y))
+        if (DEG > 2) {
+            GMS_SH_FENCE()
+            GMS_SH_K(9, SH_C3[0] * y * (3.f * xx - yy), GMS_DDIR_X(SH_C3[0] * 6.f * xy) GMS_DDIR_Y(SH_C3[0] * (3.f * xx - 3.f * yy)))
+            GMS_SH_K(10, SH_C3[1] * xy * z, GMS_DDIR_X(SH_C3[1] * yz) GMS_DDIR_Y(SH_C3[1] * xz) GMS_DDIR_Z(SH_C3[1] * xy))
+            GMS_SH_K(11, SH_C3[2] * y * (4.f * zz - xx - yy),
+                     GMS_DDIR_X(SH_C3[2] * (-2.f * xy)) GMS_DDIR_Y(SH_C3[2] * (4.f * zz - xx - 3.f * yy)) GMS_DDIR_Z(SH_C3[2] * 8.f * yz))
+            GMS_SH_FENCE()
+            GMS_SH_K(12, SH_C3[3] * z * (2.f * zz - 3.f * xx - 3.f * yy),
+                     GMS_DDIR_X(SH_C3[3] * (-6.f * xz)) GMS_DDIR_Y(SH_C3[3] * (-6.f * yz)) GMS_DDIR_Z(SH_C3[3] * (6.f * zz - 3.f * xx - 3.f * yy)))
+            GMS_SH_K(13, SH_C3[4] * x * (4.f * zz - xx - yy),
+                     GMS_DDIR_X(SH_C3[4] * (4.f * zz - 3.f * xx - yy)) GMS_DDIR_Y(SH_C3[4] * (-2.f * xy)) GMS_DDIR_Z(SH_C3[4] * 8.f * xz))
+            GMS_SH_FENCE()
+            GMS_SH_K(14, SH_C3[5] * z * (xx - yy), GMS_DDIR_X(SH_C3[5] * 2.f * xz) GMS_DDIR_Y(SH_C3[5] * (-2.f * yz)) GMS_DDIR_Z(SH_C3[5] * (xx - yy)))
+            GMS_SH_K(15, SH_C3[6] * x * (xx - 3.f * yy), GMS_DDIR_X(SH_C3[6] * (3.f * xx - 3.f * yy)) GMS_DDIR_Y(SH_C3[6] * (-6.f * xy)))
+        }
+    }
+#undef GMS_SH_K
+#undef GMS_SH_FENCE
+#undef GMS_DDIR_X
+#undef GMS_DDIR_Y
+#undef GMS_DDIR_Z
+#undef GMS_DDIR_AXIS
 }
+
+__device__ __forceinline__ void sh_dir_grad(const float D[9], const float dRGB[3], float gdir[3])
+{
+#pragma clang fp contract(off)
+#pragma unroll
+    for (int a = 0; a < 3; a++) gdir[a] = D[a * 3] * dRGB[0] + D[a * 3 + 1] * dRGB[1] + D[a * 3 + 2] * dRGB[2];
+}
+
+}
diff --git a/gaussian-mesh-splatting_amd/csrc/raster_backward.hip b/gaussian-mesh-splatting_amd/csrc/raster_backward.hip
--- a/gaussian-mesh-splatting_amd/csrc/raster_backward.hip
+++ b/gaussian-mesh-splatting_amd/csrc/raster_backward.hip
@@ -15,6 +15,7 @@
     int aa;
     const int *radii;
     const uint8_t *clamped;
+    const float *sh_ddir;
     float *accum;
     int rezero;
     float *dL_dmean2D, *dL_dopacity, *dL_dcolors;
@@ -26,155 +27,57 @@
 };
 
 template <int DEG>
-__device__ __forceinline__ void sh_backward_regs(float *r, float x, float y, float z, const float dRGB[3], float gdir[3])
-{
-#define GMS_SH_TERM(K, BV, BDX, BDY, BDZ)                                          \
-    {                                                                              \
-        const float bv = (BV), bx = (BDX), by = (BDY), bz = (BDZ);                 \
-        _Pragma("unroll") for (int c = 0; c < 3; c++) {                            \
-            const float w = r[(K) * 3 + c] * dRGB[c];                              \
-            gdir[0] += bx * w; gdir[1] += by * w; gdir[2] += bz * w;               \
-            r[(K) * 3 + c] = bv * dRGB[c];                                         \
-        }                                                                          \
-    }
-    GMS_SH_TERM(0, SH_C0, 0.f, 0.f, 0.f)
-    if (DEG > 0) {
-        GMS_SH_TERM(1, -SH_C1 * y, 0.f, -SH_C1, 0.f)
-        GMS_SH_TERM(2, SH_C1 * z, 0.f, 0.f, SH_C1)
-        GMS_SH_TERM(3, -SH_C1 * x, -SH_C1, 0.f, 0.f)
-    }
+__device__ __forceinline__ void sh_basis(float x, float y, float z, float *Y)
+{
+#pragma clang fp contract(on)
+    Y[0] = SH_C0;
+    if (DEG > 0) { Y[1] = -SH_C1 * y; Y[2] = SH_C1 * z; Y[3] = -SH_C1 * x; }
     if (DEG > 1) {
         const float xx = x * x, yy = y * y, zz = z * z;
-        GMS_SH_TERM(4, SH_C2[0] * x * y, SH_C2[0] * y, SH_C2[0] * x, 0.f)
-        GMS_SH_TERM(5, SH_C2[1] * y * z, 0.f, SH_C2[1] * z, SH_C2[1] * y)
-        GMS_SH_TERM(6, SH_C2[2] * (2.f * zz - xx - yy), -2.f * SH_C2[2] * x, -2.f * SH_C2[2] * y, 4.f * SH_C2[2] * z)
-        GMS_SH_TERM(7, SH_C2[3] * x * z, SH_C2[3] * z, 0.f, SH_C2[3] * x)
-        GMS_SH_TERM(8, SH_C2[4] * (xx - yy), 2.f * SH_C2[4] * x, -2.f * SH_C2[4] * y, 0.f)
+        Y[4] = SH_C2[0] * x * y; Y[5] = SH_C2[1] * y * z; Y[6] = SH_C2[2] * (2.f * zz - xx - yy);
+        Y[7] = SH_C2[3] * x * z; Y[8] = SH_C2[4] * (xx - yy);
     }
     if (DEG > 2) {
         const float xx = x * x, yy = y * y, zz = z * z;
-        GMS_SH_TERM(9, SH_C3[0] * y * (3.f * xx - yy), SH_C3[0] * 6.f * x * y, SH_C3[0] * (3.f * xx - 3.f * yy), 0.f)
-        GMS_SH_TERM(10, SH_C3[1] * x * y * z, SH_C3[1] * y * z, SH_C3[1] * x * z, SH_C3[1] * x * y)
-        GMS_SH_TERM(11, SH_C3[2] * y * (4.f * zz - xx - yy), SH_C3[2] * (-2.f * x * y), SH_C3[2] * (4.f * zz - xx - 3.f * yy), SH_C3[2] * 8.f * y * z)
-        GMS_SH_TERM(12, SH_C3[3] * z * (2.f * zz - 3.f * xx - 3.f * yy), SH_C3[3] * (-6.f * x * z), SH_C3[3] * (-6.f * y * z), SH_C3[3] * (6.f * zz - 3.f * xx - 3.f * yy))
-        GMS_SH_TERM(13, SH_C3[4] * x * (4.f * zz - xx - yy), SH_C3[4] * (4.f * zz - 3.f * xx - yy), SH_C3[4] * (-2.f * x * y), SH_C3[4] * 8.f * x * z)
-        GMS_SH_TERM(14, SH_C3[5] * z * (xx - yy), SH_C3[5] * 2.f * x * z, SH_C3[5] * (-2.f * y * z), SH_C3[5] * (xx - yy))
-        GMS_SH_TERM(15, SH_C3[6] * x * (xx - 3.f * yy), SH_C3[6] * (3.f * xx - 3.f * yy), SH_C3[6] * (-6.f * x * y), 0.f)
-    }
-#undef GMS_SH_TERM
-}
-
-template <int DEG>
-__device__ __forceinline__ void sh_backward(float *row_lds, float x, float y, float z, const float dRGB[3], float gdir[3])
-{
-    constexpr int NQ = ((DEG + 1) * (DEG + 1) * 3 + 3) / 4;
-    float r[NQ * 4];
-#pragma unroll
-    for (int q = 0; q < NQ; q++) {
-        const float4 v = *reinterpret_cast<const float4 *>(row_lds + q * 4);
-        r[4 * q] = v.x; r[4 * q + 1] = v.y; r[4 * q + 2] = v.z; r[4 * q + 3] = v.w;
-    }
-    sh_backward_regs<DEG>(r, x, y, z, dRGB, gdir);
-#pragma unroll
-    for (int k = (DEG + 1) * (DEG + 1) * 3; k < NQ * 4; k++) r[k] = 0.f;
-#pragma unroll
-    for (int q = 0; q < NQ; q++)
-        *reinterpret_cast<float4 *>(row_lds + q * 4) = make_float4(r[4 * q], r[4 * q + 1], r[4 * q + 2], r[4 * q + 3]);
-}
-
-template <int NQ>
-__device__ __forceinline__ void stage_sh_rows_b(const float *shs, int g0, int rows, int rowq, float *wl, int lane)
-{
-    const float4 *src = reinterpret_cast<const float4 *>(shs) + (size_t)g0 * rowq;
-    for (int idx = lane; idx < rows * NQ; idx += WAVE) {
-        const int r = idx / NQ, c = idx - r * NQ;
-        *reinterpret_cast<float4 *>(wl + r * 52 + c * 4) = src[(size_t)r * rowq + c];
-    }
-}
+        Y[9] = SH_C3[0] * y * (3.f * xx - yy); Y[10] = SH_C3[1] * x * y * z; Y[11] = SH_C3[2] * y * (4.f * zz - xx - yy);
+        Y[12] = SH_C3[3] * z * (2.f * zz - 3.f * xx - 3.f * yy); Y[13] = SH_C3[4] * x * (4.f * zz - xx - yy);
+        Y[14] = SH_C3[5] * z * (xx - yy); Y[15] = SH_C3[6] * x * (xx - 3.f * yy);
+    }
+}
+
+template <int DEG, typename PUT>
+__device__ __forceinline__ void sh_grad_row(bool vis, float x, float y, float z, const float dRGB[3], PUT put)
+{
+    constexpr int NB = (DEG + 1) * (DEG + 1);
+    float Y[16];
+    sh_basis<DEG>(x, y, z, Y);
+#pragma unroll
+    for (int k = 0; k < NB; k++) Y[k] = vis ? Y[k] : 0.f;
+#pragma unroll
+    for (int k = 0; k < 16; k++)
+#pragma unroll
+        for (int c = 0; c < 3; c++) put(k * 3 + c, k < NB ? Y[k < NB ? k : 0] * dRGB[c] : 0.f);
+}
+
+constexpr int BWD_RESTF = 45;
+constexpr int BWD_WAVE_FLOATS = WAVE * SH_PITCH_B;
+static_assert(BWD_WAVE_FLOATS >= WAVE * BWD_RESTF + WAVE * 3, "the split image fits the wave's LDS");
 
 template <bool MESH>
-__global__ void __launch_bounds__(BLOCK) preprocess_bwd_kernel(PreBwdArgs a, int pre_bwd_linear)
-{
-    __shared__ __attribute__((aligned(16))) float sh_lds[4 * WAVE * SH_PITCH_B];
+__global__ void __launch_bounds__(BLOCK) preprocess_bwd_kernel(PreBwdArgs a, int dst_vec)
+{
+#pragma clang fp contract(on)
+    __shared__ __attribute__((aligned(16))) float sh_lds[4 * BWD_WAVE_FLOATS];
     const int tid = threadIdx.x, lane = tid & 63, wave = tid >> 6;
     const int i = blockIdx.x * BLOCK + tid;
     const bool valid = i < a.P;
     const bool vis = valid && a.radii[i] > 0;
-    float *wl = sh_lds + wave * (WAVE * SH_PITCH_B);
+    float *wl = sh_lds + wave * BWD_WAVE_FLOATS;
     const int rowf = a.M * 3;
     const bool use_sh = a.shs != nullptr;
-    const bool vec_ok = use_sh && (rowf % 4 == 0) && (rowf <= 48);
-    const int nb = (a.D + 1) * (a.D + 1);
     const int g0 = blockIdx.x * BLOCK + wave * WAVE;
     const int rows = min(WAVE, a.P - g0);
-
     const bool split = a.shs_rest != nullptr;
-    constexpr int RESTF = 45;
-    const bool linear = use_sh && split && a.D == 3 && pre_bwd_linear;
-    float *const lin_dc = wl + WAVE * RESTF;
-    if (linear) {
-        if (__any(vis)) {
-            const int rr = max(rows, 0);
-            const float *sp = a.shs_rest + (size_t)g0 * RESTF;
-            const int nfl = rr * RESTF, nd = rr * 3;
-#pragma unroll
-            for (int j = 0; j < 12; j++) {
-                const int e4 = (lane + WAVE * j) * 4;
-                if (e4 + 3 < nfl)
-                    __builtin_amdgcn_global_load_lds((const __attribute__((address_space(1))) void *)(sp + e4),
-                                                     (__attribute__((address_space(3))) void *)(wl + WAVE * 4 * j), 16, 0, 0);
-            }
-            if (lane * 4 + 3 < nd)
-                __builtin_amdgcn_global_load_lds((const __attribute__((address_space(1))) void *)(a.shs + (size_t)g0 * 3 + lane * 4),
-                                                 (__attribute__((address_space(3))) void *)lin_dc, 16, 0, 0);
-            if (rr < WAVE) {
-                for (int e = (nfl & ~3) + lane; e < nfl; e += WAVE) wl[e] = sp[e];
-                for (int e = (nd & ~3) + lane; e < nd; e += WAVE) lin_dc[e] = a.shs[(size_t)g0 * 3 + e];
-            }
-            __builtin_amdgcn_s_waitcnt(0x0f70);
-        }
-        wave_sync();
-    } else if (use_sh && split) {
-        if (__any(vis)) {
-            for (int e = lane; e < rows * 3; e += WAVE) wl[(e / 3) * SH_PITCH_B + (e % 3)] = a.shs[(size_t)g0 * 3 + e];
-            const int need = nb * 3 - 3;
-            if (need == RESTF) {
-                const float *sp = a.shs_rest + (size_t)g0 * RESTF;
-                const int nfl = rows * RESTF;
-                for (int e4 = lane * 4; e4 < nfl; e4 += WAVE * 4) {
-                    float v4[4];
-                    if (e4 + 3 < nfl) { const float4 v = *reinterpret_cast<const float4 *>(sp + e4); v4[0] = v.x; v4[1] = v.y; v4[2] = v.z; v4[3] = v.w; }
-                    else { for (int t = 0; t < 4; t++) v4[t] = e4 + t < nfl ? sp[e4 + t] : 0.f; }
-#pragma unroll
-                    for (int t = 0; t < 4; t++) {
-                        const int e = e4 + t;
-                        if (e < nfl) wl[(e / RESTF) * SH_PITCH_B + 3 + (e % RESTF)] = v4[t];
-                    }
-                }
-            } else {
-                for (int e = lane; e < rows * need; e += WAVE) {
-                    const int r = e / need, c = e - r * need;
-                    wl[r * SH_PITCH_B + 3 + c] = a.shs_rest[((size_t)g0 + r) * RESTF + c];
-                }
-            }
-        }
-        wave_sync();
-    } else if (use_sh) {
-        if (vec_ok) {
-            if (__any(vis)) {
-                const int rowq = rowf / 4;
-                switch (a.D) {
-                case 0: stage_sh_rows_b<1>(a.shs, g0, rows, rowq, wl, lane); break;
-                case 1: stage_sh_rows_b<3>(a.shs, g0, rows, rowq, wl, lane); break;
-                case 2: stage_sh_rows_b<7>(a.shs, g0, rows, rowq, wl, lane); break;
-                default: stage_sh_rows_b<12>(a.shs, g0, rows, rowq, wl, lane); break;
-                }
-            }
-        } else if (vis) {
-            for (int k = 0; k < nb * 3; k++) wl[lane * SH_PITCH_B + k] = a.shs[(size_t)i * rowf + k];
-        }
-        wave_sync();
-    }
 
     float dmean[3] = {0.f, 0.f, 0.f};
     float dcov[6] = {0.f, 0.f, 0.f, 0.f, 0.f, 0.f};
@@ -195,10 +98,18 @@
     const float acc_col[3] = {gb.z, gb.w, gc4.x};
     const float acc_id = gc4.y;
     float dop = 0.f;
-    float *row = wl + lane * SH_PITCH_B;
-
+    float px = 0.f, py = 0.f, pz = 0.f;
+    float dirx = 0.f, diry = 0.f, dirz = 0.f, dir_inv = 0.f;
     if (vis) {
-        const float px = a.means3D[3 * (size_t)i], py = a.means3D[3 * (size_t)i + 1], pz = a.means3D[3 * (size_t)i + 2];
+        px = a.means3D[3 * (size_t)i]; py = a.means3D[3 * (size_t)i + 1]; pz = a.means3D[3 * (size_t)i + 2];
+        if (use_sh) {
+            const float ddx = px - a.campos[0], ddy = py - a.campos[1], ddz = pz - a.campos[2];
+            dir_inv = 1.f / sqrtf(ddx * ddx + ddy * ddy + ddz * ddz);
+            dirx = ddx * dir_inv; diry = ddy * dir_inv; dirz = ddz * dir_inv;
+            const unsigned cl = a.clamped[i];
+#pragma unroll
+            for (int c = 0; c < 3; c++) dcol_sh[c] = ((cl >> c) & 1u) ? 0.f : acc_col[c];
+        }
         const float *V = a.view, *Mx = a.proj;
         float vx, vy, vz;
         view_transform(V, px, py, pz, vx, vy, vz);
@@ -277,34 +188,11 @@
             dmean[r] += (Mx[4 * r + 0] * mw - Mx[4 * r + 3] * mul1) * gmx + (Mx[4 * r + 1] * mw - Mx[4 * r + 3] * mul2) * gmy;
 
         if (use_sh) {
-            const float ddx = px - a.campos[0], ddy = py - a.campos[1], ddz = pz - a.campos[2];
-            const float inv = 1.f / sqrtf(ddx * ddx + ddy * ddy + ddz * ddz);
-            const float x = ddx * inv, y = ddy * inv, z = ddz * inv;
-            const unsigned cl = a.clamped[i];
-            float dRGB[3];
-#pragma unroll
-            for (int c = 0; c < 3; c++) { dRGB[c] = ((cl >> c) & 1u) ? 0.f : acc_col[c]; dcol_sh[c] = dRGB[c]; }
-            float gdir[3] = {0.f, 0.f, 0.f};
-            if (linear) {
-                float r[48];
-#pragma unroll
-                for (int c = 0; c < 3; c++) r[c] = lin_dc[lane * 3 + c];
-#pragma unroll
-                for (int m = 0; m < RESTF; m++) r[3 + m] = wl[lane * RESTF + m];
-                sh_backward_regs<3>(r, x, y, z, dRGB, gdir);
-                if (!a.dL_dcolor_sh) {
-#pragma unroll
-                    for (int c = 0; c < 3; c++) lin_dc[lane * 3 + c] = r[c];
-#pragma unroll
-                    for (int m = 0; m < RESTF; m++) wl[lane * RESTF + m] = r[3 + m];
-                }
-            } else
-            switch (a.D) {
-            case 0: sh_backward<0>(row, x, y, z, dRGB, gdir); break;
-            case 1: sh_backward<1>(row, x, y, z, dRGB, gdir); break;
-            case 2: sh_backward<2>(row, x, y, z, dRGB, gdir); break;
-            default: sh_backward<3>(row, x, y, z, dRGB, gdir); break;
-            }
+            const float x = dirx, y = diry, z = dirz, inv = dir_inv;
+            float D[9], gdir[3];
+#pragma unroll
+            for (int j = 0; j < 9; j++) D[j] = a.sh_ddir[(size_t)i * GeomState::SH_DDIR + j];
+            sh_dir_grad(D, dcol_sh, gdir);
             const float dd = x * gdir[0] + y * gdir[1] + z * gdir[2];
             dmean[0] += (gdir[0] - x * dd) * inv;
             dmean[1] += (gdir[1] - y * dd) * inv;
@@ -344,68 +232,7 @@
         }
     }
 
-    if (use_sh && a.dL_dcolor_sh) {
-    } else if (linear) {
-        if (!vis) {
-#pragma unroll
-            for (int c = 0; c < 3; c++) lin_dc[lane * 3 + c] = 0.f;
-#pragma unroll
-            for (int m = 0; m < RESTF; m++) wl[lane * RESTF + m] = 0.f;
-        }
-        wave_sync();
-        if (rows > 0) {
-            const int nfl = rows * RESTF, nd = rows * 3;
-            float *dp = a.dL_dsh_rest + (size_t)g0 * RESTF, *dd = a.dL_dsh + (size_t)g0 * 3;
-#pragma unroll
-            for (int j = 0; j < 12; j++) {
-                const int e4 = (lane + WAVE * j) * 4;
-                if (e4 + 3 < nfl) {
-                    typedef float v4f __attribute__((ext_vector_type(4)));
-                    __builtin_nontemporal_store(*reinterpret_cast<const v4f *>(wl + e4), reinterpret_cast<v4f *>(dp + e4));
-                }
-                else for (int t = 0; t < 4; t++) if (e4 + t < nfl) dp[e4 + t] = wl[e4 + t];
-            }
-            if (lane * 4 + 3 < nd) *reinterpret_cast<float4 *>(dd + lane * 4) = *reinterpret_cast<const float4 *>(lin_dc + lane * 4);
-            else for (int t = 0; t < 4; t++) if (lane * 4 + t < nd) dd[lane * 4 + t] = lin_dc[lane * 4 + t];
-        }
-    } else if (use_sh && split) {
-        for (int q = vis ? (nb * 3 + 3) / 4 : 0; q < 12; q++)
-            *reinterpret_cast<float4 *>(row + q * 4) = make_float4(0.f, 0.f, 0.f, 0.f);
-        wave_sync();
-        if (rows > 0) {
-            for (int e = lane; e < rows * 3; e += WAVE) a.dL_dsh[(size_t)g0 * 3 + e] = wl[(e / 3) * SH_PITCH_B + (e % 3)];
-            float *dp = a.dL_dsh_rest + (size_t)g0 * RESTF;
-            const int nfl = rows * RESTF;
-            for (int e4 = lane * 4; e4 < nfl; e4 += WAVE * 4) {
-                float v4[4];
-#pragma unroll
-                for (int t = 0; t < 4; t++) {
-                    const int e = e4 + t;
-                    v4[t] = e < nfl ? wl[(e / RESTF) * SH_PITCH_B + 3 + (e % RESTF)] : 0.f;
-                }
-                if (e4 + 3 < nfl) *reinterpret_cast<float4 *>(dp + e4) = make_float4(v4[0], v4[1], v4[2], v4[3]);
-                else for (int t = 0; t < 4; t++) if (e4 + t < nfl) dp[e4 + t] = v4[t];
-            }
-        }
-    } else if (use_sh) {
-        const int used = vis ? nb * 3 : 0;
-        if (vec_ok) {
-            const int rowq = rowf / 4;
-            for (int q = vis ? (nb * 3 + 3) / 4 : 0; q < rowq; q++)
-                *reinterpret_cast<float4 *>(row + q * 4) = make_float4(0.f, 0.f, 0.f, 0.f);
-            wave_sync();
-            if (rows > 0) {
-                float4 *dst = reinterpret_cast<float4 *>(a.dL_dsh + (size_t)g0 * rowf);
-                for (int idx = lane; idx < rows * rowq; idx += WAVE) {
-                    int r = idx / rowq, c = idx - r * rowq;
-                    dst[(size_t)r * rowq + c] = *reinterpret_cast<const float4 *>(wl + r * SH_PITCH_B + c * 4);
-                }
-            }
-        } else if (valid) {
-            for (int k = 0; k < rowf; k++) a.dL_dsh[(size_t)i * rowf + k] = k < used ? row[k] : 0.f;
-        }
-    }
-    if (!valid) return;
+    if (valid) {
     if (MESH) {
         const float gs[3] = {dscale[0], dscale[1], dscale[2]}, gq[4] = {drot[0], drot[1], drot[2], drot[3]};
         splat_backward_from_registers(a.mesh, (int64_t)i, dmean, gs, gq, dop, a.mesh_dvertices, a.mesh_dalpha, a.mesh_dscale, a.mesh_dopacity);
@@ -418,7 +245,7 @@
         a.dL_dcolor_sh[3 * (size_t)a.P] = a.campos[0]; a.dL_dcolor_sh[3 * (size_t)a.P + 1] = a.campos[1]; a.dL_dcolor_sh[3 * (size_t)a.P + 2] = a.campos[2];
     }
     if (a.dL_dcolor_sh) { a.dL_dcolor_sh[3 * (size_t)i] = dcol_sh[0]; a.dL_dcolor_sh[3 * (size_t)i + 1] = dcol_sh[1]; a.dL_dcolor_sh[3 * (size_t)i + 2] = dcol_sh[2]; }
-    if (MESH) return;
+    if (!MESH) {
     a.dL_dmeans3D[3 * (size_t)i] = dmean[0]; a.dL_dmeans3D[3 * (size_t)i + 1] = dmean[1]; a.dL_dmeans3D[3 * (size_t)i + 2] = dmean[2];
     if (a.cov3Dp) {
         if (a.dL_dcov3D)
@@ -427,6 +254,63 @@
     } else {
         a.dL_dscales[3 * (size_t)i] = dscale[0]; a.dL_dscales[3 * (size_t)i + 1] = dscale[1]; a.dL_dscales[3 * (size_t)i + 2] = dscale[2];
         *reinterpret_cast<float4 *>(a.dL_drots + 4 * (size_t)i) = make_float4(drot[0], drot[1], drot[2], drot[3]);
+    }
+    }
+    }
+    if (use_sh && !a.dL_dcolor_sh && rows > 0) {
+        float rdx = 0.f, rdy = 0.f, rdz = 0.f;
+        if (vis) {
+            const float ddx = a.means3D[3 * (size_t)i] - a.campos[0], ddy = a.means3D[3 * (size_t)i + 1] - a.campos[1], ddz = a.means3D[3 * (size_t)i + 2] - a.campos[2];
+            const float dinv = 1.f / sqrtf(ddx * ddx + ddy * ddy + ddz * ddz);
+            rdx = ddx * dinv; rdy = ddy * dinv; rdz = ddz * dinv;
+        }
+        float *const dcw = wl + WAVE * BWD_RESTF;
+        auto write_row = [&](auto put) {
+            switch (a.D) {
+            case 0: sh_grad_row<0>(vis, rdx, rdy, rdz, dcol_sh, put); break;
+            case 1: sh_grad_row<1>(vis, rdx, rdy, rdz, dcol_sh, put); break;
+            case 2: sh_grad_row<2>(vis, rdx, rdy, rdz, dcol_sh, put); break;
+            default: sh_grad_row<3>(vis, rdx, rdy, rdz, dcol_sh, put); break;
+            }
+        };
+        if (split) {
+            float *const d0 = dcw + lane * 3, *const d1 = wl + lane * BWD_RESTF - 3;
+            write_row([&](int e, float v) { (e < 3 ? d0 : d1)[e] = v; });
+        } else {
+            float *const d0 = wl + lane * SH_PITCH_B;
+            const int lim = min(rowf, 48);
+            write_row([&](int e, float v) { if (e < lim) d0[e] = v; });
+        }
+        wave_sync();
+        if (split) {
+            const int nfl = rows * BWD_RESTF, nd = rows * 3;
+            float *dp = a.dL_dsh_rest + (size_t)g0 * BWD_RESTF, *dd = a.dL_dsh + (size_t)g0 * 3;
+            if (dst_vec) {
+                typedef float v4f __attribute__((ext_vector_type(4)));
+#pragma unroll
+                for (int j = 0; j < 12; j++) {
+                    const int e4 = (lane + WAVE * j) * 4;
+                    if (e4 + 3 < nfl) __builtin_nontemporal_store(*reinterpret_cast<const v4f *>(wl + e4), reinterpret_cast<v4f *>(dp + e4));
+                }
+                const int e = (nfl & ~3) + lane;
+                if (e < nfl) dp[e] = wl[e];
+                if (lane * 4 + 3 < nd) *reinterpret_cast<float4 *>(dd + lane * 4) = *reinterpret_cast<const float4 *>(dcw + lane * 4);
+                const int ed = (nd & ~3) + lane;
+                if (ed < nd) dd[ed] = dcw[ed];
+            } else {
+                for (int e = lane; e < nfl; e += WAVE) dp[e] = wl[e];
+                for (int e = lane; e < nd; e += WAVE) dd[e] = dcw[e];
+            }
+        } else if (rowf == 48) {
+            float4 *dst = reinterpret_cast<float4 *>(a.dL_dsh + (size_t)g0 * 48);
+            for (int idx = lane; idx < rows * 12; idx += WAVE) {
+                const int r = idx / 12, c = idx - r * 12;
+                dst[idx] = *reinterpret_cast<const float4 *>(wl + r * SH_PITCH_B + c * 4);
+            }
+        } else if (valid) {
+            const float *row = wl + lane * SH_PITCH_B;
+            for (int k = 0; k < rowf; k++) a.dL_dsh[(size_t)i * rowf + k] = k < 48 ? row[k] : 0.f;
+        }
     }
 }
 
@@ -476,24 +360,6 @@
     float *dL_dsh_rest;
     int accumulate;
 };
-
-template <int DEG>
-__device__ __forceinline__ void sh_basis(float x, float y, float z, float *Y)
-{
-    Y[0] = SH_C0;
-    if (DEG > 0) { Y[1] = -SH_C1 * y; Y[2] = SH_C1 * z; Y[3] = -SH_C1 * x; }
-    if (DEG > 1) {
-        const float xx = x * x, yy = y * y, zz = z * z;
-        Y[4] = SH_C2[0] * x * y; Y[5] = SH_C2[1] * y * z; Y[6] = SH_C2[2] * (2.f * zz - xx - yy);
-        Y[7] = SH_C2[3] * x * z; Y[8] = SH_C2[4] * (xx - yy);
-    }
-    if (DEG > 2) {
-        const float xx = x * x, yy = y * y, zz = z * z;
-        Y[9] = SH_C3[0] * y * (3.f * xx - yy); Y[10] = SH_C3[1] * x * y * z; Y[11] = SH_C3[2] * y * (4.f * zz - xx - yy);
-        Y[12] = SH_C3[3] * z * (2.f * zz - 3.f * xx - 3.f * yy); Y[13] = SH_C3[4] * x * (4.f * zz - xx - yy);
-        Y[14] = SH_C3[5] * z * (xx - yy); Y[15] = SH_C3[6] * x * (xx - 3.f * yy);
-    }
-}
 
 template <int DEG>
 __global__ void __launch_bounds__(BLOCK) sh_grad_expand_kernel(ShExpandArgs a)
@@ -618,16 +484,15 @@
     p.means3D = A->means3D; p.shs = A->shs; p.shs_rest = A->shs_rest; p.colors = A->colors_precomp; p.opac = A->opacities; p.scales = A->scales;
     p.rots = A->rotations; p.cov3Dp = A->cov3D_precomp; p.view = A->viewmatrix; p.proj = A->projmatrix; p.campos = A->campos;
     p.mod = A->scale_modifier; p.scale_grad_mod = upstream_scale_mod_grad() ? 1.f : A->scale_modifier; p.tanx = A->tan_fovx; p.tany = A->tan_fovy; p.aa = A->antialiasing; p.radii = A->radii;
-    p.clamped = geom.clamped; p.accum = A->grad_accum; p.rezero = fault_mode() == 3 ? 0 : A->grad_accum_rezero; p.dL_dmean2D = A->dL_dmeans2D;
+    p.clamped = geom.clamped; p.sh_ddir = geom.sh_ddir; p.accum = A->grad_accum; p.rezero = fault_mode() == 3 ? 0 : A->grad_accum_rezero; p.dL_dmean2D = A->dL_dmeans2D;
     p.dL_dcolors = A->colors_precomp ? A->dL_dcolors : nullptr; p.dL_dcolor_sh = (A->shs && A->sh_factor_mode) ? A->dL_dcolors : nullptr; p.campos_row = A->factor_campos_row; p.dL_dopacity = A->dL_dopacity; p.dL_dmeans3D = A->dL_dmeans3D;
     p.dL_dcov3D = A->dL_dcov3D; p.dL_dsh = A->dL_dsh; p.dL_dsh_rest = A->dL_dsh_rest; p.dL_dscales = A->dL_dscales; p.dL_drots = A->dL_drotations;
-    const int lin_ok = A->shs && A->shs_rest && A->D == 3 && (((uintptr_t)A->shs) & 15u) == 0 && (((uintptr_t)A->shs_rest) & 15u) == 0 &&
-                       (A->sh_factor_mode || ((((uintptr_t)A->dL_dsh) & 15u) == 0 && (((uintptr_t)A->dL_dsh_rest) & 15u) == 0));
+    const int dst_vec = A->shs_rest && !A->sh_factor_mode && (((uintptr_t)A->dL_dsh) & 15u) == 0 && (((uintptr_t)A->dL_dsh_rest) & 15u) == 0;
     if (mesh) {
         p.mesh = *mesh; p.mesh_dvertices = A->mesh_dL_dvertices; p.mesh_dalpha = A->mesh_dL_dalpha; p.mesh_dscale = A->mesh_dL_dscale; p.mesh_dopacity = A->mesh_dL_d_opacity;
-        GMS_LAUNCH(GMS_K_PREPROCESS_BWD, stream, preprocess_bwd_kernel<true><<<(unsigned)((P + BLOCK - 1) / BLOCK), BLOCK, 0, stream>>>(p, lin_ok));
+        GMS_LAUNCH(GMS_K_PREPROCESS_BWD, stream, preprocess_bwd_kernel<true><<<(unsigned)((P + BLOCK - 1) / BLOCK), BLOCK, 0, stream>>>(p, dst_vec));
     } else {
-        GMS_LAUNCH(GMS_K_PREPROCESS_BWD, stream, preprocess_bwd_kernel<false><<<(unsigned)((P + BLOCK - 1) / BLOCK), BLOCK, 0, stream>>>(p, lin_ok));
+        GMS_LAUNCH(GMS_K_PREPROCESS_BWD, stream, preprocess_bwd_kernel<false><<<(unsigned)((P + BLOCK - 1) / BLOCK), BLOCK, 0, stream>>>(p, dst_vec));
     }
     GMS_KERNEL_CHECK(A->debug, stream, "preprocess_bwd");
     if (fault_mode() == 4 && A->dL_dscales)
diff --git a/gaussian-mesh-splatting_amd/csrc/raster_forward.hip b/gaussian-mesh-splatting_amd/csrc/raster_forward.hip
--- a/gaussian-mesh-splatting_amd/csrc/raster_forward.hip
+++ b/gaussian-mesh-splatting_amd/csrc/raster_forward.hip
@@ -44,30 +44,6 @@
     float *k0_xyz, *k0_scale, *k0_rot, *k0_opac;
 };
 
-template <int DEG>
-__device__ __forceinline__ float sh_eval_channel(const float *row, int c, float x, float y, float z)
-{
-#pragma clang fp contract(off)
-    float res = SH_C0 * row[0 * 3 + c];
-    if (DEG > 0) {
-        res = res - SH_C1 * y * row[1 * 3 + c] + SH_C1 * z * row[2 * 3 + c] - SH_C1 * x * row[3 * 3 + c];
-        if (DEG > 1) {
-            float xx = x * x, yy = y * y, zz = z * z, xy = x * y, yz = y * z, xz = x * z;
-            res = res + SH_C2[0] * xy * row[4 * 3 + c] + SH_C2[1] * yz * row[5 * 3 + c] +
-                  SH_C2[2] * (2.f * zz - xx - yy) * row[6 * 3 + c] + SH_C2[3] * xz * row[7 * 3 + c] +
-                  SH_C2[4] * (xx - yy) * row[8 * 3 + c];
-            if (DEG > 2) {
-                res = res + SH_C3[0] * y * (3.f * xx - yy) * row[9 * 3 + c] + SH_C3[1] * xy * z * row[10 * 3 + c] +
-                      SH_C3[2] * y * (4.f * zz - xx - yy) * row[11 * 3 + c] +
-                      SH_C3[3] * z * (2.f * zz - 3.f * xx - 3.f * yy) * row[12 * 3 + c] +
-                      SH_C3[4] * x * (4.f * zz - xx - yy) * row[13 * 3 + c] + SH_C3[5] * z * (xx - yy) * row[14 * 3 + c] +
-                      SH_C3[6] * x * (xx - 3.f * yy) * row[15 * 3 + c];
-            }
-        }
-    }
-    return res;
-}
-
 template <int NQ>
 __device__ __forceinline__ void stage_sh_rows(const float *shs, int g0, int rows, int rowq, float *wl, int lane)
 {
@@ -79,7 +55,7 @@
 }
 
 template <int DEG>
-__device__ __forceinline__ void sh_colour(const float *row_lds, float x, float y, float z, float rgb[3], unsigned &clampbits)
+__device__ __forceinline__ void sh_colour(const float *row_lds, float x, float y, float z, float rgb[3], unsigned &clampbits, float ddir[9])
 {
     constexpr int NQ = ((DEG + 1) * (DEG + 1) * 3 + 3) / 4;
     float r[NQ * 4];
@@ -88,12 +64,21 @@
         const float4 v = *reinterpret_cast<const float4 *>(row_lds + q * 4);
         r[4 * q] = v.x; r[4 * q + 1] = v.y; r[4 * q + 2] = v.z; r[4 * q + 3] = v.w;
     }
+    float res[3];
+    sh_eval_with_dir_jacobian<DEG>([&](int k, int c) { return r[k * 3 + c]; }, x, y, z, res, ddir);
 #pragma unroll
     for (int c = 0; c < 3; c++) {
-        float v = sh_eval_channel<DEG>(r, c, x, y, z) + 0.5f;
+        float v = res[c] + 0.5f;
         if (v < 0.f) { clampbits |= 1u << c; v = 0.f; }
         rgb[c] = v;
     }
+}
+
+__device__ __forceinline__ void store_sh_ddir(float *sh_ddir, int i, const float ddir[9])
+{
+    float *d = sh_ddir + (size_t)i * GeomState::SH_DDIR;
+#pragma unroll
+    for (int j = 0; j < 9; j++) d[j] = ddir[j];
 }
 
 template <int SHDEG, bool SPLIT, bool DMA = false, bool K0 = false, bool PTS = false>
@@ -286,17 +271,17 @@
             __builtin_amdgcn_s_waitcnt(0x0f70);
             wave_sync();
             if (vis && (lane >> 5) == half) {
-                float r[48];
-#pragma unroll
-                for (int c = 0; c < 3; c++) r[c] = wl[DMA_REST_FLOATS + lane * 3 + c];
-#pragma unroll
-                for (int m = 0; m < RESTF; m++) r[3 + m] = wl[(lane - r0) * RESTF + m];
+                const float *dcrow = wl + DMA_REST_FLOATS + lane * 3;
+                const float *rrow = wl + (lane - r0) * RESTF - 3;
+                float res[3], ddir[9];
+                sh_eval_with_dir_jacobian<SHDEG>([&](int k, int c) { return k == 0 ? dcrow[c] : rrow[k * 3 + c]; }, dxc, dyc, dzc, res, ddir);
 #pragma unroll
                 for (int c = 0; c < 3; c++) {
-                    float v = sh_eval_channel<SHDEG>(r, c, dxc, dyc, dzc) + 0.5f;
+                    float v = res[c] + 0.5f;
                     if (v < 0.f) { clampbits |= 1u << c; v = 0.f; }
                     rgb[c] = v;
                 }
+                store_sh_ddir(a.geom.sh_ddir, i, ddir);
             }
         }
     } else if (SHDEG >= 0) {
@@ -328,7 +313,9 @@
         if (vis) {
             float dx = px - a.campos[0], dy = py - a.campos[1], dz = pz - a.campos[2];
             float inv = 1.f / sqrtf(dx * dx + dy * dy + dz * dz);
-            sh_colour<(SHDEG >= 0 ? SHDEG : 0)>(wl + lane * SH_PITCH, dx * inv, dy * inv, dz * inv, rgb, clampbits);
+            float ddir[9];
+            sh_colour<(SHDEG >= 0 ? SHDEG : 0)>(wl + lane * SH_PITCH, dx * inv, dy * inv, dz * inv, rgb, clampbits, ddir);
+            store_sh_ddir(a.geom.sh_ddir, i, ddir);
         }
     } else if (a.shs) {
         const int nb = (a.D + 1) * (a.D + 1);
@@ -355,12 +342,14 @@
             float inv = 1.f / sqrtf(dx * dx + dy * dy + dz * dz);
             float x = dx * inv, y = dy * inv, z = dz * inv;
             const float *row = wl + lane * SH_PITCH;
+            float ddir[9];
             switch (a.D) {
-            case 0: sh_colour<0>(row, x, y, z, rgb, clampbits); break;
-            case 1: sh_colour<1>(row, x, y, z, rgb, clampbits); break;
-            case 2: sh_colour<2>(row, x, y, z, rgb, clampbits); break;
-            default: sh_colour<3>(row, x, y, z, rgb, clampbits); break;
-            }
+            case 0: sh_colour<0>(row, x, y, z, rgb, clampbits, ddir); break;
+            case 1: sh_colour<1>(row, x, y, z, rgb, clampbits, ddir); break;
+            case 2: sh_colour<2>(row, x, y, z, rgb, clampbits, ddir); break;
+            default: sh_colour<3>(row, x, y, z, rgb, clampbits, ddir); break;
+            }
+            store_sh_ddir(a.geom.sh_ddir, i, ddir);
         }
     } else if (vis) {
         rgb[0] = a.colors[3 * (size_t)i]; rgb[1] = a.colors[3 * (size_t)i + 1]; rgb[2] = a.colors[3 * (size_t)i + 2];
diff --git a/gaussian-mesh-splatting_amd/csrc/torch_binding.cpp b/gaussian-mesh-splatting_amd/csrc/torch_binding.cpp
--- a/gaussian-mesh-splatting_amd/csrc/torch_binding.cpp
+++ b/gaussian-mesh-splatting_amd/csrc/torch_binding.cpp
@@ -43,11 +43,15 @@
 }
 
 struct Slot { Tensor t; c10::Device dev; bool failed; };
+std::atomic<int> g_scratch_fill{-1};
+void set_scratch_fill(int64_t byte) { g_scratch_fill = (byte >= 0 && byte <= 255) ? (int)byte : -1; }
 void *alloc_cb(void *ctx, size_t bytes)
 {
     Slot *s = static_cast<Slot *>(ctx);
     try {
         s->t = torch::empty({(int64_t)(bytes > 0 ? bytes : 1)}, torch::TensorOptions().dtype(torch::kUInt8).device(s->dev));
+        const int fill = g_scratch_fill.load();
+        if (fill >= 0) s->t.fill_(fill);
         return s->t.data_ptr();
     } catch (...) {
         s->failed = true;
@@ -1229,6 +1233,7 @@
     m.def("render_mesh", &render_mesh, "differentiable frame straight from a mesh: [image, radii, invdepth, xyz, scaling_act, rotation_unit, opacity_act]", nogil());
     m.def("l1_ssim", &l1_ssim, "differentiable w_l1 * L1 + w_ssim * SSIM + bias; returns (value [0-dim], [l1, ssim])", nogil());
     m.def("adam_step", &adam_step, nogil());
+    m.def("set_scratch_fill", &set_scratch_fill, "fill every scratch buffer with this byte before the library writes into it; -1: off (diagnostics only)");
     m.def("set_keep_buffers", &set_keep_buffers, "keep references to the last forward's scratch tensors (diagnostics only)");
     m.def("clear_accum", &clear_accum);
     m.def("set_sh_factor_mode", &set_sh_factor_mode, "factorised SH gradient: backward calls queue [P+1,3] factors instead of writing dL/dsh");
diff --git a/gaussian-mesh-splatting_amd/diff_gaussian_rasterization/__init__.py b/gaussian-mesh-splatting_amd/diff_gaussian_rasterization/__init__.py
--- a/gaussian-mesh-splatting_amd/diff_gaussian_rasterization/__init__.py
+++ b/gaussian-mesh-splatting_amd/diff_gaussian_rasterization/__init__.py
@@ -146,6 +146,16 @@
             _last_stats.pop(k, None)
 
 
+_scratch_fill = None
+
+
+def set_scratch_fill(byte: Optional[int]) -> None:
+    global _scratch_fill
+    _scratch_fill = None if byte is None else int(byte) & 0xFF
+    if _C is not None:
+        _C.set_scratch_fill(-1 if _scratch_fill is None else _scratch_fill)
+
+
 def raw_buffers() -> dict:
     d = _C.last_stats() if _C is not None else _last_stats
     return {k: d.get(k) for k in ("geom", "binning", "image")}
@@ -186,6 +196,8 @@
             def cb(_ctx, nbytes):
                 try:
                     t = torch.empty(max(int(nbytes), 1), dtype=torch.uint8, device=self.device)
+                    if _scratch_fill is not None:
+                        t.fill_(_scratch_fill)
                     self.tensors[name] = t
                     return t.data_ptr()
                 except Exception as e:
```

Result: faster. 3034, median of 6 (+1.1%).
